# nirschl-lab/stain2stain

Measured on AMD Instinct MI355X. Metric: paired 256x256 stain tiles/sec (full CFM optimisation step), higher is better.
Workload: dtype bf16

## Files before the change

include/stain2stain_hip.h:

```cpp
#ifndef STAIN2STAIN_HIP_H
#define STAIN2STAIN_HIP_H

#ifdef __cplusplus
extern "C" {
#endif

#define S2S_OK 0
#define S2S_ERR_SHAPE (-1)
#define S2S_ERR_ALIGN (-2)
#define S2S_ERR_DTYPE (-3)
#define S2S_ERR_LAUNCH (-4)
#define S2S_ERR_NULL (-5)

#define S2S_BF16 0
#define S2S_F32 1

int s2s_conv3x3_stat_blocks(int dtype, int B, int H, int W, int Cout);
int s2s_conv3x3_nhwc(int dtype, const void* x0, int ld0, int c0, const void* x1, int ld1, int c1,
                     const void* w_packed, const float* bias, void* y, int ldy, float* stat_part,
                     const float* ep_scale, const float* ep_shift, int relu, int B, int H, int W, int Cout,
                     void* stream);

int s2s_conv3x3_ksplit(int dtype, int B, int H, int W, int Cout, int cin);
int s2s_conv3x3_nhwc_k(int dtype, const void* x0, int ld0, int c0, const void* x1, int ld1, int c1,
                       const void* w_packed, const float* bias, void* y, int ldy, float* stat_part,
                       const float* ep_scale, const float* ep_shift, int relu, float* kwork, int B, int H, int W,
                       int Cout, void* stream);
int s2s_conv3x3_stat_rows(int dtype, int B, int H, int W, int Cout, int c0, int c1, int ld0, int ld1, int has_bias);
int s2s_conv3x3_staged(int dtype, int B, int H, int W, int Cout, int c0, int c1, int ld0, int ld1, int ldy, int stats);
int s2s_conv3x3_family(int dtype, int B, int H, int W, int Cout, int c0, int c1, int ld0, int ld1, int ldy, int has_bias,
                       int has_affine, int stats, int stat_rows, int kwork);
int s2s_conv3x3_nhwc_s(int dtype, const void* x0, int ld0, int c0, const void* x1, int ld1, int c1, const void* w_packed,
                       const float* bias, void* y, int ldy, float* stat_part, int stat_rows, const float* ep_scale,
                       const float* ep_shift, int relu, float* kwork, int B, int H, int W, int Cout, void* stream);
int s2s_debug_conv_clock(long* out_host, int n);

int s2s_conv3x3_wgrad_splits(int dtype, int B, int H, int W, int Cin, int Cout);
int s2s_conv3x3_wgrad_nhwc(int dtype, const void* dy, int lddy, int Cout, const void* x0, int ld0, int c0,
                           const void* x1, int ld1, int c1, float* part, float* grad_oihw, int accumulate,
                           int B, int H, int W, void* stream);
int s2s_conv3x3_wgrad_phase(int dtype, const void* dy, int lddy, int Cout, const void* x0, int ld0, int c0,
                            const void* x1, int ld1, int c1, float* part, float* grad_oihw, int accumulate,
                            int B, int H, int W, int phases, void* stream);

int s2s_stem_stat_blocks(int B, int H, int W);
int s2s_stem_conv3x3_fwd(int dtype, const float* x_nchw, const float* w_oihw, const float* bias, void* y, int ldy,
                         float* stat_part, int B, int H, int W, int Cin, int Cout, void* stream);
int s2s_stem_wgrad_blocks(int B, int H, int W);
int s2s_stem_conv3x3_wgrad(int dtype, const void* dy, int lddy, const float* x_nchw, float* part, float* dw_oihw,
                           float* dbias, int accumulate, int B, int H, int W, int Cin, int Cout, void* stream);
int s2s_head_conv1x1_fwd(int dtype, const void* x, int ldx, const float* w, const float* bias, float* y_nchw, int B,
                         int H, int W, int C, int Cout, void* stream);
int s2s_head_wgrad_blocks(int B, int H, int W);
int s2s_head_conv1x1_bwd(int dtype, const float* dy_nchw, const void* x, int ldx, const float* w, void* dx, int lddx,
                         float* part, float* dw, float* dbias, int accumulate, int B, int H, int W, int C, int Cout,
                         void* stream);

int s2s_head_loss_blocks(int B, int H, int W);
int s2s_head_loss_fused(int dtype, const void* x, int ldx, const float* w, const float* bias, const float* u_nchw,
                        float* v_nchw, void* dx, int lddx, float grad_scale, float* part, double* lpart, float* dw,
                        float* dbias, float* loss, int accumulate, int B, int H, int W, int C, int Cout, void* stream);

int s2s_tail_blocks(int B, int H, int W);
int s2s_tail_fwd_loss(int dtype, const void* raw, int ldx, const float* scale, const float* shift, const float* mean,
                      const float* invstd, const float* w, const float* bias, const float* u_nchw, float* v_nchw,
                      float* g_nchw, float grad_scale, float* part, double* lpart, float* bnwork, float* dw,
                      float* dbias, float* loss, float* dgamma, float* dbeta, float* conv_dbias, int accumulate, int B,
                      int H, int W, int C, int Cout, void* stream);
int s2s_tail_bwd_apply(int dtype, const void* raw, int ldx, const float* g_nchw, const float* w, const float* scale,
                       const float* shift, const float* mean, const float* invstd, const float* gamma,
                       const float* bnwork, void* dx, int lddx, int B, int H, int W, int C, int Cout, void* stream);

int s2s_bn_finalize(const float* part, int nblk, int C, long count, const float* gamma, const float* beta,
                    float* running_mean, float* running_var, long* num_batches_tracked, float momentum, float eps,
                    float* mean, float* invstd, float* scale, float* shift, void* stream);
int s2s_bn_finalize_b(const float* part, int nblk, int C, long count, const float* gamma, const float* beta,
                      float* running_mean, float* running_var, long* num_batches_tracked, float momentum, float eps,
                      float* mean, float* invstd, float* scale, float* shift, const float* conv_bias, void* stream);
int s2s_bn_eval_prepare(int C, const float* gamma, const float* beta, const float* running_mean,
                        const float* running_var, float eps, float* scale, float* shift, void* stream);
int s2s_bn_relu_apply(int dtype, const void* x, int ldx, const float* scale, const float* shift, void* y, int ldy,
                      void* pool, int ldp, int B, int H, int W, int C, void* stream);
int s2s_maxpool2(int dtype, const void* x, int ldx, void* pool, int ldp, int B, int H, int W, int C, void* stream);
int s2s_bn_bwd_blocks(int B, int H, int W, int C);
int s2s_bn_relu_bwd(int dtype, const void* g1, int ldg1, const void* gp, int ldgp, const float* scale,
                    const float* shift, const void* x, int ldx, const float* mean, const float* invstd, const float* gamma, float* dgamma,
                    float* dbeta, float* dbias_conv, int accumulate, void* dx, int lddx, float* work, int B, int H,
                    int W, int C, void* stream);
int s2s_bn_partial_sums(const float* part, int nblk, int C, float* sums, void* stream);
int s2s_bn_relu_bwd_phase(int dtype, const void* g1, int ldg1, const void* gp, int ldgp, const float* scale,
                          const float* shift, const void* x, int ldx, const float* mean, const float* invstd,
                          const float* gamma, float* dgamma, float* dbeta, float* dbias_conv, int accumulate, void* dx,
                          int lddx, float* work, int B, int H, int W, int C, long count_total, int phases, void* stream);

int s2s_upsample2x_bilinear_ac_fwd(int dtype, const void* x, int ldx, const float* bias_nc, void* y, int ldy, int B,
                                   int Hin, int Win, int Hout, int Wout, int C, void* stream);
int s2s_upsample2x_bilinear_ac_fwd_ref(int dtype, const void* x, int ldx, const float* bias_nc, void* y, int ldy, int B,
                                       int Hin, int Win, int Hout, int Wout, int C, void* stream);
int s2s_upsample2x_fwd_family(int ldx, int ldy, int B, int Hin, int Win, int Hout, int Wout, int C, int reference);
int s2s_upsample2x_bilinear_ac_bwd(int dtype, const void* dy, int lddy, void* dx, int lddx, int B, int Hin, int Win,
                                   int Hout, int Wout, int C, void* stream);
int s2s_upsample2x_bilinear_ac_bwd_ref(int dtype, const void* dy, int lddy, void* dx, int lddx, int B, int Hin,
                                       int Win, int Hout, int Wout, int C, void* stream);
int s2s_upsample2x_bwd_family(int lddy, int lddx, int B, int Hin, int Win, int Hout, int Wout, int C, int reference);
int s2s_pixel_sum(int dtype, const void* x, int ldx, float* out_nc, int B, int HW, int C, int accumulate,
                  void* stream);

int s2s_time_embedding(const float* t, float* out, int B, int dim, void* stream);
int s2s_linear_fwd(const float* x, const float* w, const float* bias, float* y, int B, int K, int N, void* stream);
int s2s_linear_bwd(const float* dy, const float* x, const float* w, float* dx, float* dw, float* db, int accumulate,
                   int B, int K, int N, void* stream);
int s2s_silu_fwd(const float* h, float* a, int n, void* stream);
int s2s_silu_bwd(const float* h, const float* da, float* dh, int n, void* stream);
int s2s_cfm_sample(const float* x0, const float* x1, const float* t, const float* eps, float sigma, float* xt,
                   float* ut, int B, long per_sample, void* stream);
int s2s_mse_loss(const float* v, const float* u, float* dv, float grad_scale, float* loss, double* work, long count,
                 void* stream);
int s2s_ode_error_norm(const float* e, const float* y0, const float* y1, float atol, float rtol, float* out,
                       double* work, long n, void* stream);
int s2s_axpy(float* x, const float* y, float a, long n, void* stream);
int s2s_dp_partials(long n);
int s2s_dp_init(int phase, const float* y, const float* k1, const float* fa, double* state, double* part, float* out,
                float* t_out, int* status, float atol, float rtol, int B, long n, void* stream);
int s2s_dp_stage(int i, const float* y, const float* k1, const float* k2, const float* k3, const float* k4,
                 const float* k5, const float* k6, const double* state, float* out, float* t_out, int B, long n,
                 void* stream);
int s2s_dp_error(const float* k1, const float* k2, const float* k3, const float* k4, const float* k5, const float* k6,
                 const float* k7, const float* y, const float* y_new, const double* state, double* part, float atol,
                 float rtol, int B, long n, void* stream);
int s2s_dp_control(double* state, const double* part, int* status, int max_steps, int B, long n, void* stream);
int s2s_dp_commit(float* y, const float* y_new, float* k1, const float* k7, const double* state, int B, long n,
                  void* stream);
int s2s_rk_stage(const float* x, const float* k1, const float* k2, const float* k3, float c1, float c2, float c3, int nk,
                 float* out, float* t_out, const float* table, const int* counter, int stages, int stage, int table_len,
                 int B, long n, void* stream);
int s2s_rk_combine(float* x, const float* k1, const float* k2, const float* k3, const float* k4, float c1, float c2,
                   float c3, float c4, int nk, int* counter, int B, long n, void* stream);
int s2s_fill_f32(float* x, float v, long n, void* stream);
int s2s_euler_tick(float* t, int n, const float* table, int* counter, void* stream);

int s2s_adam_step(float* p, const float* g, float* m, float* v, long n, int step, float lr, float beta1, float beta2,
                  float eps, float weight_decay, float grad_scale, void* stream);
int s2s_adam_step_dev(float* p, const float* g, float* m, float* v, long n, const float* hyper, void* stream);
long s2s_adam_multi_blocks(long n);
int s2s_adam_multi(const void* desc, int ntensors, long total, int step, float lr, float beta1, float beta2, float eps,
                   float weight_decay, float grad_scale, void* stream);
int s2s_adam_ema_step(float* p, const float* g, float* m, float* v, float* ema, long n, int step, float lr, float beta1,
                      float beta2, float eps, float weight_decay, float grad_scale, float ema_weight, void* stream);
int s2s_adam_ema_step_dev(float* p, const float* g, float* m, float* v, float* ema, long n, const float* hyper,
                          const float* ema_weight, void* stream);
long s2s_ema_multi_blocks(long n);
int s2s_ema_multi(const void* desc, int ntensors, long total, const float* weight, void* stream);
long s2s_pack_conv3x3_fwd_elems(int Cout, int Cin);
long s2s_pack_conv3x3_dgrad_elems(int Cout, int Cin);
int s2s_pack_conv3x3(int dtype, const float* w_oihw, void* w_fwd, void* w_dgrad, int Cout, int Cin, void* stream);
int s2s_pack_conv3x3_batched(int dtype, const void* desc, int nlayers, long total, void* stream);
int s2s_nchw_to_nhwc(int dtype, const float* x_nchw, void* y, int ldy, int B, int C, int H, int W, void* stream);
int s2s_nhwc_to_nchw(int dtype, const void* x, int ldx, float* y_nchw, int accumulate, int B, int C, int H, int W,
                     void* stream);

int s2s_paired_crop_flip_normalize(const void* src_u8, const void* tgt_u8, const int* params, float* out_src,
                                   float* out_tgt, int B, int Hs, int Ws, int S, void* stream);
int s2s_pil_resize_bilinear_normalize(const void* src_u8, void* tmp_u8, const int* bounds_h, const int* kk_h,
                                      int ksize_h, const int* bounds_v, const int* kk_v, int ksize_v, void* out_u8,
                                      float* out_f, int B, int Hs, int Ws, int Ho, int Wo, void* stream);

int s2s_region_gather(const void* img_u8, long pitch, int H, int W, int band_top, int band_h, const int* origins,
                      float* out, int B, int T, void* stream);
int s2s_region_blend(const float* tiles, int c0, const float* tiles1, int c1, const int* origins, int n, int T,
                     int overlap, float* acc, int band_rows, int H, int W, int r0, int r1, void* stream);
int s2s_region_finalize(float* acc, int band_rows, int W, int C, int r0, int r1, void* out_u8, long pitch_u8,
                        float* out_f, long pitch_f, int out_top, void* stream);

int s2s_region_tissue_count(const void* img_u8, long pitch, int H, int W, int band_top, int band_h, const int* origins,
                            int n, int T, int white, int black, int* counts, void* stream);
int s2s_region_skip_weight(const int* origins, int n, int T, int overlap, float* ws, int band_rows, int H, int W,
                           int r0, int r1, void* stream);
int s2s_region_finalize_mixed(float* acc, float* ws, int band_rows, int W, int C, int r0, int r1, const void* src_u8,
                              long src_pitch, int src_top, void* out_u8, long pitch_u8, float* out_f, long pitch_f,
                              int out_top, void* stream);

int s2s_seg_loss(const float* z, const float* g, float* dz, float* out, double* work, long n, float smooth,
                 float dice_weight, float grad_scale, void* stream);
int s2s_seg_loss_multiclass(const float* z, const long* target, float* dz, float* out, double* work, long B, long HW,
                            int C, int ignore_index, float smooth, float dice_weight, float grad_scale, void* stream);

int s2s_seg_eval_binary(const float* z, const float* g, float* out, long* counts, double* work, long n, float smooth,
                        float dice_weight, void* stream);
int s2s_seg_eval_multiclass(const float* z, const long* target, float* out, long* counts, double* work, long B,
                            long HW, int C, int ignore_index, float smooth, float dice_weight, void* stream);
int s2s_head_mse_eval_blocks(int B, int H, int W, int C);
int s2s_head_mse_eval(int dtype, const void* x, int ldx, const float* w, const float* bias, const float* u_nchw,
                      float* loss, double* lpart, int B, int H, int W, int C, int Cout, void* stream);

int s2s_image_quality_blocks(int H, int W, int win);
int s2s_image_quality_f32(const float* a, const float* b, int B, int C, int H, int W, int quantize, int win,
                          const float* taps, float k1, float k2, double* part, void* stream);
int s2s_image_quality_u8(const void* a, long pitch_a, long img_a, const void* b, long pitch_b, long img_b, int B,
                         int band_top, int band_h, int H, int W, int by0, int nby, int win, const float* taps, float k1,
                         float k2, double* part, void* stream);
int s2s_image_quality_finalize(const double* part, int B, int C, int H, int W, int win, float range, float* out,
                               void* stream);

int s2s_stain_quant_chunks(int cell_h, int cell_w);
int s2s_stain_quant_u8(const void* a, long pitch_a, long img_a, const void* b, long pitch_b, long img_b, int paired,
                       int B, int band_top, int band_h, int H, int W, int cell_h, int cell_w, int g0, int ng,
                       const float* od_table, const float* unmix, int white, int black, int stain, double* part,
                       void* stream);
int s2s_stain_quant_f32(const float* a, const float* b, int paired, int B, int H, int W, const float* od_table,
                        const float* unmix, int white, int black, int stain, double* part, void* stream);
int s2s_stain_quant_finalize(const double* part, long owners, int nchunk, int paired, long* counts, double* sums,
                             float* out, void* stream);
int s2s_stain_separate(const void* img, int is_f32, long pitch, long img_stride, int B, int H, int W,
                       const float* od_table, const float* unmix, float* out, void* stream);
int s2s_stain_mask_u8(const void* img, long pitch, long img_stride, int B, int band_top, int band_h, int H, int W,
                      const float* od_table, const float* unmix, int white, int black, int stain, void* mask,
                      long mask_pitch, long mask_stride, long* tissue, void* stream);
int s2s_stain_mask_f32(const float* img, int B, int H, int W, const float* od_table, const float* unmix, int white,
                       int black, int stain, void* mask, long mask_pitch, long mask_stride, long* tissue, void* stream);

long s2s_stain_moments_slots(int B, int H, int W);
int s2s_stain_moments_u8(const void* img, long pitch, long img_stride, int B, int band_top, int band_h, int H, int W,
                         const int* q_table, int u_beta, int black, long* part, void* stream);
int s2s_stain_moments_finalize(const long* part, long nslots, long* out, void* stream);
int s2s_stain_angle_hist_u8(const void* img, long pitch, long img_stride, int B, int band_top, int band_h, int H, int W,
                            const float* od_table, const float* plane, int u_beta, int black, int reset, long* hist,
                            void* stream);
int s2s_stain_conc_hist_u8(const void* img, long pitch, long img_stride, int B, int band_top, int band_h, int H, int W,
                           const float* od_table, const float* unmix, int u_beta, int black, int reset, long* hist,
                           void* stream);
int s2s_stain_normalize_u8(const void* img, long pitch, long img_stride, int B, int H, int W, const float* od_table,
                           const float* coef, void* out, long out_pitch, long out_img, int out_f32, void* stream);

long s2s_objects_words(int B, int H, int W);
long s2s_objects_hit_words(int B, int H, int W);
int s2s_objects_label(const void* mask, long pitch, long img_stride, int fg_bits, int B, int H, int W, int connectivity,
                      int min_area, int max_objects, int* scratch, int* labels, int* count, long* kept_pixels,
                      int* largest, long* size_hist, int* tab_area, int* tab_bbox, long* tab_sums, void* stream);
int s2s_objects_centroid(const int* count, const int* tab_area, const long* tab_sums, int B, int max_objects,
                         float* centroid, void* stream);
int s2s_objects_hits(const int* labels_pred, const int* labels_target, int B, int H, int W, int* scratch, int* hits,
                     void* stream);
int s2s_objects_scores(const int* count_pred, const int* count_target, const int* hits, int B, float* out,
                       int* abs_err, void* stream);
int s2s_objects_density(const long* kept_pixels, const long* tissue, const int* count, int B,
                        const double* mm2_per_pixel, float* burden, double* per_mm2, void* stream);

int s2s_paired_augment(const void* src_u8, long src_pitch, long src_img, const void* tgt_u8, long tgt_pitch,
                       long tgt_img, const void* mask_u8, long mask_pitch, long mask_img, int B, int Hs, int Ws, int S,
                       const int* params, int param_cols, const float* src_map, const float* tgt_map,
                       const float* od_table, int white, float* out_src, float* out_tgt, void* out_mask, int mask_kind,
                       void* out_src_u8, void* out_tgt_u8, void* stream);
int s2s_stain_augment_u8(const void* img, long pitch, long img_stride, int B, int H, int W, const float* maps,
                         const float* od_table, int white, void* out, long out_pitch, long out_img, int out_f32,
                         void* stream);

int s2s_structure_map_u8(const void* img, long pitch, long img_stride, int B, int H, int W, const int* q_table,
                         const int* w, int ds, void* out, void* stream);
int s2s_register_sums(const void* a, const void* b, int B, int h, int w, int R, const int* center, long* tsum,
                      long* sums, void* stream);
int s2s_register_pick(const long* tsum, const long* sums, const int* center, int B, int R, int ds, int* shift,
                      double* score, int* valid, void* stream);
int s2s_shift_tiles_u8(const void* img, long pitch, long img_stride, int B, int H, int W, int C, const int* shift,
                       int fill, void* out, long out_pitch, long out_img, void* stream);

int s2s_weighted_mse(const float* v, const float* u, const float* mask, float* dv, float* out, double* work, long B,
                     int C, long HW, float roi_lambda, float grad_scale, void* stream);
int s2s_charbonnier_roi(const float* pred, const float* truth, const float* mask, float* out, double* work, long B,
                        int C, long HW, float eps_charb, float eps_area, void* stream);
int s2s_class_embed_add(const float* temb, const float* table, const long* y, float* out, int B, int dim,
                        void* stream);
int s2s_class_embed_bwd(const float* dout, const long* y, float* dtable, int accumulate, int B, int dim,
                        int num_classes, void* stream);

int s2s_instnorm_blocks(int B, int H, int W, int C);
int s2s_instnorm_lrelu_fwd(int dtype, const void* x, int ldx, const float* gamma, const float* beta, void* y, int ldy,
                           float* work, float* stats, int B, int H, int W, int C, float eps, float slope,
                           void* stream);
int s2s_instnorm_lrelu_bwd(int dtype, const void* g, int ldg, const void* x, int ldx, const float* stats, void* dx,
                           int lddx, float* dgamma, float* dbeta, int accumulate, float* work, int B, int H, int W,
                           int C, float eps, float slope, void* stream);

int s2s_conv2x2_stat_blocks(int B, int H, int W, int Cout);
int s2s_conv2x2_nhwc(int dtype, const void* x, int ldx, int cin, const void* w_packed, const float* bias, void* y,
                     int ldy, float* stat_part, int B, int H, int W, int Cout, int pad, void* stream);
int s2s_space_to_depth_pad1(int dtype, const void* x, int ldx, void* xs, int ldxs, int inverse, int B, int H, int W,
                            int C, void* stream);
int s2s_channel_sum_blocks(long npix, int C);
int s2s_channel_sum(int dtype, const void* x, int ldx, float* work, float* out, long npix, int C, int accumulate,
                    void* stream);
int s2s_pack_conv4x4(const float* w_oihw, void* wf, void* wd, int Cout, int Cin, int stride, void* stream);
int s2s_conv4x4s1_nhwc(int dtype, const void* x, int ldx, int cin, const void* w_packed, const float* bias, void* y,
                       int ldy, float* stat_part, int B, int H, int W, int Cout, int pad, void* stream);
int s2s_conv4x4s1_wgrad_splits(int B, int H, int W, int Cin, int Cout);
int s2s_conv4x4s1_wgrad_nhwc(int dtype, const void* dy, int lddy, int Cout, const void* x, int ldx, int cin,
                             float* part, float* grad16, int accumulate, int B, int H, int W, void* stream);
int s2s_conv2x2_wgrad_splits(int B, int H, int W, int Cin, int Cout);
int s2s_conv2x2_wgrad_nhwc(int dtype, const void* dy, int lddy, int Cout, const void* x, int ldx, int cin, float* part,
                           float* grad2, int accumulate, int B, int H, int W, void* stream);

int s2s_convkxk_stat_blocks(int dtype, int B, int H, int W, int Cout, int ks);
int s2s_convkxk_nhwc(int dtype, const void* x, int ldx, int cin, const void* w_packed, const float* bias, int bias_mod,
                     void* y, int ldy, void* y2, int ldy2, int act, float act_slope, float* stat_part, float* kwork, int B,
                     int H, int W, int Cout, int ks, int pad, void* stream);
int s2s_convkxk_ksplit(int dtype, int B, int H, int W, int Cout, int cin, int ks);
int s2s_convkxk_wgrad_splits(int dtype, int B, int H, int W, int Cin, int Cout, int ks);
int s2s_convkxk_wgrad_nhwc(int dtype, const void* dy, int lddy, int Cout, const void* x, int ldx, int cin, float* part,
                           float* grad, int layout, int accumulate, int B, int H, int W, int ks, int x_plain, void* stream);
int s2s_conv4x4s2_ksplit(int B, int H, int W, int Cout, int Cin);
int s2s_conv4x4s2_plan(int B, int H, int W, int Cout, int Cin);
int s2s_conv4x4s2_nhwc(int dtype, const void* x, int ldx, int Cin, const void* wf, const float* bias, void* y, int ldy,
                       void* y2, int ldy2, int act, float act_slope, float* kwork, int B, int H, int W, int Cout,
                       void* stream);
int s2s_convt4x4s2_ksplit(int B, int h, int w, int C, int Cin);
int s2s_convt4x4s2_plan(int B, int h, int w, int C, int Cin);
int s2s_convt4x4s2_nhwc(int dtype, const void* x, int ldx, int Cin, const void* wd, const float* bias, void* y, int ldy,
                        float* kwork, int B, int h, int w, int C, void* stream);
int s2s_convsm_ok(int dtype, int mode, int B, int h, int w, int Cin, int Cout);
int s2s_convsm_nhwc(int dtype, int mode, const void* x, int ldx, int Cin, const void* w_packed, const float* bias, int epi,
                    int act, float slope, float eps, void* raw, int ldraw, void* y, int ldy, void* y2, int ldy2,
                    float* stats, const float* stats_in, const void* z, int ldz, const void* g2, int ldg2, int bwd_c0,
                    int B, int h, int w, int Cout, void* stream);
int s2s_instnorm_lrelu_fwd2(int dtype, const void* x, int ldx, const float* gamma, const float* beta, void* y, int ldy,
                            void* y2, int ldy2, float* work, float* stats, int B, int H, int W, int C, float eps,
                            float slope, void* stream);
int s2s_instnorm_lrelu_bwd2(int dtype, const void* g, int ldg, const void* g2, int ldg2, const void* x, int ldx,
                            const float* stats, void* dx, int lddx, float* dgamma, float* dbeta, int accumulate,
                            float* work, int B, int H, int W, int C, float eps, float slope, void* stream);
int s2s_instnorm_split_ok(int dtype, int H, int W, int C);
int s2s_instnorm_lrelu_fwd_split(int dtype, const float* slabs, int S, const float* bias, void* raw, int ldraw, void* y,
                                 int ldy, void* y2, int ldy2, float* stats, int B, int H, int W, int C, float eps,
                                 float slope, void* stream);
int s2s_instnorm_lrelu_bwd_split(int dtype, const float* gslabs, int S, const void* g2, int ldg2, const void* x, int ldx,
                                 const float* stats, void* dx, int lddx, int B, int H, int W, int C, float slope,
                                 void* stream);
int s2s_pack_conv4x4_t(int dtype, const float* w_oihw, void* wf, void* wd, int Cout, int Cin, int stride, void* stream);
long s2s_pack_conv4x4_blocks(int Cout, int Cin, int stride);
int s2s_pack_conv4x4_batched(int dtype, const void* desc, int nlayers, long total, void* stream);
int s2s_p2p_pack_input(int dtype, const float* a_nchw, int ca, const float* b_nchw, int cb, void* out, int ldo, int B,
                       int H, int W, void* stream);
int s2s_p2p_unpack(int dtype, const void* in, int ldi, int c0, int C, float* out_nchw, int B, int H, int W, void* stream);
int s2s_p2p_tanh_l1_blocks(int B, int H, int W);
int s2s_p2p_tanh_l1_fwd(int dtype, const void* h, int ldh, const float* src_nchw, const float* tgt_nchw, void* d_in,
                        int ldd, float* fake_nchw, float* l1_out, void* work, int B, int H, int W, int C, void* stream);
int s2s_p2p_tanh_l1_bwd(int dtype, const void* h, int ldh, const float* tgt_nchw, const void* gd, int ldg, float l1_scale,
                        void* dh, int lddh, int B, int H, int W, int C, void* stream);
int s2s_p2p_bce_logits(int dtype, const void* z, int ldz, int n_real, float w_real, float w_fake, void* dz, int lddz,
                       float* out2, int N, int HW, void* stream);
int s2s_p2p_bce_blocks(int N, int HW);
int s2s_p2p_bce_logits_w(int dtype, const void* z, int ldz, int n_real, float w_real, float w_fake, void* dz, int lddz,
                         float* out2, double* work, int N, int HW, void* stream);
int s2s_p2p_act_bwd_blocks(long npix, int C);
int s2s_p2p_act_bwd(int dtype, const void* g, int ldg, const void* g2, int ldg2, const void* a, int lda, float slope,
// ... 15 lines not shown
```

stain2stain_amd/csrc/conv_edge.hip:

```cpp
#include "common.h"

namespace {

constexpr int STEM_MAX_CIN = 8;

typedef __attribute__((address_space(3))) s16x4 lds_s16x4;

__device__ __forceinline__ bf16x8 tr_frag8(const char* p) {
  s16x4 lo = __builtin_amdgcn_ds_read_tr16_b64_v4i16((lds_s16x4*)(p));
  s16x4 hi = __builtin_amdgcn_ds_read_tr16_b64_v4i16((lds_s16x4*)(p + 4 * 64));
  bf16x4 l4 = __builtin_bit_cast(bf16x4, lo), h4 = __builtin_bit_cast(bf16x4, hi);
  bf16x8 r;
#pragma unroll
  for (int i = 0; i < 4; ++i) { r[i] = l4[i]; r[4 + i] = h4[i]; }
  return r;
}

template <int NIMG>
__device__ __forceinline__ void split_store(char* base, int img_stride, int off, const float* v8) {
  bf16x8 h, m, l;
#pragma unroll
  for (int i = 0; i < 8; ++i) {
    h[i] = (bf16_t)v8[i];
    const float r1 = v8[i] - (float)h[i];
    m[i] = (bf16_t)r1;
    l[i] = (bf16_t)(r1 - (float)m[i]);
  }
  *reinterpret_cast<bf16x8*>(base + off) = h;
  if (NIMG == 3) {
    *reinterpret_cast<bf16x8*>(base + img_stride + off) = m;
    *reinterpret_cast<bf16x8*>(base + 2 * img_stride + off) = l;
  }
}

template <typename T>
__global__ __launch_bounds__(256) void stem_wgrad_kernel(const T* __restrict__ dy, int lddy,
                                                         const float* __restrict__ x, float* __restrict__ part,
                                                         int B, int H, int W, int Cin, int Cout, int tilesY,
                                                         int tilesX) {
  constexpr int NIMG = sizeof(T) == 4 ? 3 : 1;
  constexpr int NPX = 256;
  constexpr int DY_IMG = 2 * NPX * 64;
  constexpr int P_IMG = NPX * 64;
  extern __shared__ __attribute__((aligned(16))) char smem[];
  char* const ldsDY = smem;
  char* const ldsP = smem + NIMG * DY_IMG;
  float* const xl = reinterpret_cast<float*>(ldsP + NIMG * P_IMG);
  const int tid = threadIdx.x, lane = tid & 63, wave = tid >> 6;
  const int wco = wave & 1, whalf = wave >> 1;
  const int co0 = blockIdx.y * 64;
  const int c0 = blockIdx.z * 3;
  const int nc = (Cin - c0) < 3 ? (Cin - c0) : 3, K = nc * 9;
  const int g = lane >> 4, q = (lane & 15) >> 2, pq = lane & 3;
  const int frag_off = ((g >> 1) * 8 + q) * 64 + ((g & 1) * 16 + pq * 4) * 2;
  const int ntiles = B * tilesY * tilesX;
  f32x16 acc;
#pragma unroll
  for (int j = 0; j < 16; ++j) acc[j] = 0.f;
  for (int tile = blockIdx.x; tile < ntiles; tile += gridDim.x) {
    int bt = tile;
    const int tx = bt % tilesX; bt /= tilesX;
    const int ty = bt % tilesY;
    const int n = bt / tilesY;
    const int y0 = ty * 16, x0 = tx * 16;
    __syncthreads();
    for (int i = tid; i < nc * 324; i += 256) {
      const int ci = i / 324, r = i - ci * 324, hy = r / 18, hx = r - hy * 18;
      const int gy = y0 - 1 + hy, gx = x0 - 1 + hx;
      xl[i] = (gy >= 0 && gy < H && gx >= 0 && gx < W) ? x[(((long)n * Cin + c0 + ci) * H + gy) * W + gx] : 0.f;
    }
#pragma unroll
    for (int it = 0; it < 8; ++it) {
      const int idx = tid + it * 256;
      const int px = idx >> 3, pc = idx & 7;
      const int gy = y0 + (px >> 4), gx = x0 + (px & 15), co = co0 + pc * 8;
      float v8[8];
#pragma unroll
      for (int k = 0; k < 8; ++k) v8[k] = 0.f;
      if (gy < H && gx < W && co < Cout) {
        const f32x8 v = load8(dy + (((long)n * H + gy) * W + gx) * lddy + co);
#pragma unroll
        for (int k = 0; k < 8; ++k) v8[k] = v.v[k];
      }
      split_store<NIMG>(ldsDY, DY_IMG, (pc >> 2) * (NPX * 64) + px * 64 + (pc & 3) * 16, v8);
    }
    __syncthreads();
    {
      const int py = tid >> 4, px = tid & 15;
      const bool inside = (y0 + py < H) && (x0 + px < W);
#pragma unroll
      for (int c4 = 0; c4 < 4; ++c4) {
        float v8[8];
#pragma unroll
        for (int k = 0; k < 8; ++k) {
          const int kk = c4 * 8 + k;
          float v = 0.f;
          if (kk < K) {
            const int ci = kk / 9, t = kk - ci * 9;
            v = xl[ci * 324 + (py + t / 3) * 18 + px + t % 3];
          } else if (kk == K && c0 == 0) {
            v = inside ? 1.f : 0.f;
          }
          v8[k] = v;
        }
        split_store<NIMG>(ldsP, P_IMG, tid * 64 + c4 * 16, v8);
      }
    }
    __syncthreads();
    const char* A0 = ldsDY + wco * (NPX * 64) + frag_off;
    const char* B0 = ldsP + frag_off;
#pragma unroll
    for (int ks = 0; ks < 8; ++ks) {
      const int m0 = (whalf * 8 + ks) * 16;
      const bf16x8 ah = tr_frag8(A0 + m0 * 64);
      const bf16x8 bh = tr_frag8(B0 + m0 * 64);
      if constexpr (NIMG == 3) {
        const bf16x8 am = tr_frag8(A0 + DY_IMG + m0 * 64), al = tr_frag8(A0 + 2 * DY_IMG + m0 * 64);
        const bf16x8 bm = tr_frag8(B0 + P_IMG + m0 * 64), bl = tr_frag8(B0 + 2 * P_IMG + m0 * 64);
        acc = __builtin_amdgcn_mfma_f32_32x32x16_bf16(am, bm, acc, 0, 0, 0);
        acc = __builtin_amdgcn_mfma_f32_32x32x16_bf16(al, bh, acc, 0, 0, 0);
        acc = __builtin_amdgcn_mfma_f32_32x32x16_bf16(ah, bl, acc, 0, 0, 0);
        acc = __builtin_amdgcn_mfma_f32_32x32x16_bf16(am, bh, acc, 0, 0, 0);
        acc = __builtin_amdgcn_mfma_f32_32x32x16_bf16(ah, bm, acc, 0, 0, 0);
      }
      acc = __builtin_amdgcn_mfma_f32_32x32x16_bf16(ah, bh, acc, 0, 0, 0);
    }
  }
  const int kcol = lane & 31, h = lane >> 5;
#pragma unroll
  for (int j = 0; j < 16; ++j) {
    const int co = co0 + wco * 32 + (j & 3) + 8 * (j >> 2) + 4 * h;
    if (co < Cout)
      part[((((long)blockIdx.z * gridDim.x + blockIdx.x) * 2 + whalf) * Cout + co) * 32 + kcol] = acc[j];
  }
}

__global__ __launch_bounds__(1024) void stem_wgrad_reduce_kernel(const float* part, int nslab, int Cout, int Cin, float* dw, float* db,
                                         int accumulate) {
  __shared__ double red[32][33];
  const int c0 = blockIdx.y * 3;
  const int K = ((Cin - c0) < 3 ? (Cin - c0) : 3) * 9;
  const int co = blockIdx.x, k = threadIdx.x & 31, sg = threadIdx.x >> 5;
  part += (long)blockIdx.y * nslab * Cout * 32;
  double s = 0.0, s1 = 0.0;
  int b = sg;
  for (; b + 32 < nslab; b += 64) {
    s += (double)part[((long)b * Cout + co) * 32 + k];
    s1 += (double)part[((long)(b + 32) * Cout + co) * 32 + k];
  }
  for (; b < nslab; b += 32) s += (double)part[((long)b * Cout + co) * 32 + k];
  s += s1;
  red[sg][k] = s;
  __syncthreads();
  if (sg == 0) {
    for (int j = 1; j < 32; ++j) s += red[j][k];
    if (k < K) {
      float* dst = dw + co * Cin * 9 + c0 * 9 + k;
      *dst = accumulate ? *dst + (float)s : (float)s;
    } else if (k == K && c0 == 0 && db) {
      db[co] = accumulate ? db[co] + (float)s : (float)s;
    }
  }
}

constexpr int HEAD_MAX_COUT = 4;
constexpr int HEAD_WIDE_COUT = 8;

template <typename T, int MO>
__global__ void head_fwd_kernel(const T* __restrict__ x, int ldx, const float* __restrict__ w,
                                const float* __restrict__ bias, float* __restrict__ y, long npix, int HW, int C,
                                int Cout) {
  extern __shared__ __attribute__((aligned(16))) char smem[];
  float* wl = reinterpret_cast<float*>(smem);
  for (int i = threadIdx.x; i < Cout * C; i += blockDim.x) wl[i] = w[i];
  __syncthreads();
  for (long p = (long)blockIdx.x * blockDim.x + threadIdx.x; p < npix; p += (long)gridDim.x * blockDim.x) {
    float acc[MO];
#pragma unroll
    for (int o = 0; o < MO; ++o) acc[o] = 0.f;
    for (int c8 = 0; c8 < C; c8 += 8) {
      const f32x8 v = load8(x + p * ldx + c8);
#pragma unroll
      for (int o = 0; o < MO; ++o)
        if (o < Cout)
#pragma unroll
          for (int k = 0; k < 8; ++k) acc[o] = fmaf(v.v[k], wl[o * C + c8 + k], acc[o]);
    }
    const long n = p / HW, q = p - n * HW;
#pragma unroll
    for (int o = 0; o < MO; ++o)
      if (o < Cout) y[(n * Cout + o) * HW + q] = acc[o] + (bias ? bias[o] : 0.f);
  }
}

template <typename T, int MO>
__global__ void head_bwd_data_kernel(const float* __restrict__ dy, const float* __restrict__ w, T* __restrict__ dx,
                                     int lddx, long npix, int HW, int C, int Cout) {
  extern __shared__ __attribute__((aligned(16))) char smem[];
  float* wl = reinterpret_cast<float*>(smem);
  for (int i = threadIdx.x; i < Cout * C; i += blockDim.x) wl[i] = w[i];
  __syncthreads();
  for (long p = (long)blockIdx.x * blockDim.x + threadIdx.x; p < npix; p += (long)gridDim.x * blockDim.x) {
    const long n = p / HW, q = p - n * HW;
    float g[MO];
#pragma unroll
    for (int o = 0; o < MO; ++o) g[o] = o < Cout ? dy[(n * Cout + o) * HW + q] : 0.f;
    for (int c8 = 0; c8 < C; c8 += 8) {
      f32x8 v;
#pragma unroll
      for (int k = 0; k < 8; ++k) {
        float a = 0.f;
#pragma unroll
        for (int o = 0; o < MO; ++o)
          if (o < Cout) a = fmaf(g[o], wl[o * C + c8 + k], a);
        v.v[k] = a;
      }
      store8(dx + p * lddx + c8, v);
    }
  }
}

template <typename T, int MO>
__global__ __launch_bounds__(256) void head_wgrad_kernel(const float* __restrict__ dy, const T* __restrict__ x,
                                                         int ldx, float* __restrict__ part, long npix, int HW, int C,
                                                         int Cout) {
  extern __shared__ __attribute__((aligned(16))) char smem[];
  float* xl = reinterpret_cast<float*>(smem);
  float* gl = xl + 64 * (C + 1);
  const int nout = Cout * (C + 1);
  float acc[8];
#pragma unroll
  for (int i = 0; i < 8; ++i) acc[i] = 0.f;
  for (long p0 = (long)blockIdx.x * 64; p0 < npix; p0 += (long)gridDim.x * 64) {
    __syncthreads();
    for (int i = threadIdx.x; i < 64 * C; i += 256) {
      const int pp = i / C, c = i - pp * C;
      xl[pp * (C + 1) + c] = (p0 + pp < npix) ? to_f32(x[(p0 + pp) * ldx + c]) : 0.f;
    }
    for (int i = threadIdx.x; i < 64 * MO; i += 256) {
      const int pp = i / MO, o = i - pp * MO;
      float v = 0.f;
      if (o < Cout && p0 + pp < npix) {
        const long p = p0 + pp, n = p / HW, q = p - n * HW;
        v = dy[(n * Cout + o) * HW + q];
      }
      gl[i] = v;
    }
    __syncthreads();
#pragma unroll
    for (int i = 0; i < 8; ++i) {
      const int id = threadIdx.x + i * 256;
      if (id < nout) {
        const int o = id / (C + 1), c = id - o * (C + 1);
        float a = acc[i];
        if (c < C) for (int pp = 0; pp < 64; ++pp) a = fmaf(gl[pp * MO + o], xl[pp * (C + 1) + c], a);
        else for (int pp = 0; pp < 64; ++pp) a += gl[pp * MO + o];
        acc[i] = a;
      }
    }
  }
#pragma unroll
  for (int i = 0; i < 8; ++i) {
    const int id = threadIdx.x + i * 256;
    if (id < nout) part[(long)blockIdx.x * nout + id] = acc[i];
  }
}

__global__ __launch_bounds__(256) void head_wgrad_reduce_kernel(const float* part, int nblk, int Cout, int C, float* dw, float* db,
                                         int accumulate) {
  __shared__ double red[32][9];
  const int nout = Cout * (C + 1);
  const int ol = threadIdx.x & 7, sg = threadIdx.x >> 3;
  const int i = blockIdx.x * 8 + ol;
  double s = 0.0;
  if (i < nout) {
    double s1 = 0.0;
    int b = sg;
    for (; b + 32 < nblk; b += 64) { s += (double)part[(long)b * nout + i]; s1 += (double)part[(long)(b + 32) * nout + i]; }
    for (; b < nblk; b += 32) s += (double)part[(long)b * nout + i];
    s += s1;
  }
  red[sg][ol] = s;
  __syncthreads();
  if (sg == 0 && i < nout) {
    for (int j = 1; j < 32; ++j) s += red[j][ol];
    const int o = i / (C + 1), c = i - o * (C + 1);
    if (c == C && !db) return;
    float* dst = (c < C) ? dw + o * C + c : db + o;
    *dst = accumulate ? *dst + (float)s : (float)s;
  }
}

template <typename T>
__global__ __launch_bounds__(256) void head_loss_fused_kernel(const T* __restrict__ x, int ldx,
                                                              const float* __restrict__ w, const float* __restrict__ bias,
                                                              const float* __restrict__ u, float* __restrict__ v_out,
                                                              T* __restrict__ dx, int lddx, float coef,
                                                              float* __restrict__ part, double* __restrict__ lpart,
                                                              long npix, int HW, int C, int Cout) {
  extern __shared__ __attribute__((aligned(16))) char smem[];
  float* wl = reinterpret_cast<float*>(smem);
  float* gl = wl + HEAD_MAX_COUT * C;
  bf16_t* al = reinterpret_cast<bf16_t*>(gl + 256 * HEAD_MAX_COUT);
  __shared__ double lred[256];
  const int AS = C + 8;
  for (int i = threadIdx.x; i < Cout * C; i += 256) wl[i] = w[i];
  const int nout = Cout * (C + 1);
  float acc[4];
#pragma unroll
  for (int i = 0; i < 4; ++i) acc[i] = 0.f;
  double lsum = 0.0;
  __syncthreads();
  for (long p0 = (long)blockIdx.x * 256; p0 < npix; p0 += (long)gridDim.x * 256) {
    const long p = p0 + threadIdx.x;
    const bool ok = p < npix;
    float g[HEAD_MAX_COUT];
#pragma unroll
    for (int o = 0; o < HEAD_MAX_COUT; ++o) g[o] = 0.f;
    if (ok) {
      float vv[HEAD_MAX_COUT];
#pragma unroll
      for (int o = 0; o < HEAD_MAX_COUT; ++o) vv[o] = 0.f;
      for (int c8 = 0; c8 < C; c8 += 8) {
        const f32x8 a = load8(x + p * ldx + c8);
        bf16x8 ab;
#pragma unroll
        for (int k = 0; k < 8; ++k) ab[k] = (bf16_t)a.v[k];
        *reinterpret_cast<bf16x8*>(al + threadIdx.x * AS + c8) = ab;
#pragma unroll
        for (int o = 0; o < HEAD_MAX_COUT; ++o)
          if (o < Cout)
#pragma unroll
            for (int k = 0; k < 8; ++k) vv[o] = fmaf(a.v[k], wl[o * C + c8 + k], vv[o]);
      }
      const long n = p / HW, q = p - n * HW;
#pragma unroll
      for (int o = 0; o < HEAD_MAX_COUT; ++o)
        if (o < Cout) {
          const float vo = vv[o] + (bias ? bias[o] : 0.f);
          const long idx = (n * Cout + o) * HW + q;
          if (v_out) v_out[idx] = vo;
          const float d = vo - u[idx];
          lsum += (double)(d * d);
          g[o] = coef * d;
        }
      for (int c8 = 0; c8 < C; c8 += 8) {
        f32x8 da;
#pragma unroll
        for (int k = 0; k < 8; ++k) {
          float s = 0.f;
#pragma unroll
          for (int o = 0; o < HEAD_MAX_COUT; ++o)
            if (o < Cout) s = fmaf(g[o], wl[o * C + c8 + k], s);
          da.v[k] = s;
        }
        store8(dx + p * lddx + c8, da);
      }
    } else {
      for (int c8 = 0; c8 < C; c8 += 8) {
        bf16x8 z;
#pragma unroll
        for (int k = 0; k < 8; ++k) z[k] = (bf16_t)0.f;
        *reinterpret_cast<bf16x8*>(al + threadIdx.x * AS + c8) = z;
      }
    }
#pragma unroll
    for (int o = 0; o < HEAD_MAX_COUT; ++o) gl[threadIdx.x * HEAD_MAX_COUT + o] = g[o];
    __syncthreads();
#pragma unroll
    for (int i = 0; i < 4; ++i) {
      const int id = threadIdx.x + i * 256;
      if (id < nout) {
        const int o = id / (C + 1), c = id - o * (C + 1);
        float a = acc[i];
        if (c < C) for (int pp = 0; pp < 256; ++pp) a = fmaf(gl[pp * HEAD_MAX_COUT + o], (float)al[pp * AS + c], a);
        else for (int pp = 0; pp < 256; ++pp) a += gl[pp * HEAD_MAX_COUT + o];
        acc[i] = a;
      }
    }
    __syncthreads();
  }
#pragma unroll
  for (int i = 0; i < 4; ++i) {
    const int id = threadIdx.x + i * 256;
    if (id < nout) part[(long)blockIdx.x * nout + id] = acc[i];
  }
  lred[threadIdx.x] = lsum;
  __syncthreads();
  for (int o = 128; o > 0; o >>= 1) {
    if (threadIdx.x < o) lred[threadIdx.x] += lred[threadIdx.x + o];
    __syncthreads();
  }
  if (threadIdx.x == 0) lpart[blockIdx.x] = lred[0];
}

template <typename T, int PCB>
__global__ __launch_bounds__(256) void head_loss_lanes_kernel(const T* __restrict__ x, int ldx,
                                                              const float* __restrict__ w,
                                                              const float* __restrict__ bias,
                                                              const float* __restrict__ u, float* __restrict__ v_out,
                                                              T* __restrict__ dx, int lddx, float coef,
                                                              float* __restrict__ part, double* __restrict__ lpart,
                                                              long npix, int HW, int Cout) {
  constexpr int C = PCB * 8, PPB = 256 / PCB, MO = HEAD_MAX_COUT;
  __shared__ float fold[256][MO * 8 + 1];
  __shared__ float dbf[PPB][MO];
  __shared__ double lred[256];
  const int tid = threadIdx.x, pc = tid & (PCB - 1), slot = tid / PCB;
  const int lane = tid & 63, grp0 = lane & ~(PCB - 1);
  float wr[MO][8], bo[MO];
#pragma unroll
  for (int o = 0; o < MO; ++o) {
    bo[o] = (o < Cout && bias) ? bias[o] : 0.f;
#pragma unroll
    for (int k = 0; k < 8; ++k) wr[o][k] = o < Cout ? w[o * C + pc * 8 + k] : 0.f;
  }
  float dwacc[MO][8], dbacc[MO];
#pragma unroll
  for (int o = 0; o < MO; ++o) {
    dbacc[o] = 0.f;
#pragma unroll
    for (int k = 0; k < 8; ++k) dwacc[o][k] = 0.f;
  }
  double lsum = 0.0;
  const int np = (int)npix, stride = (int)gridDim.x * PPB;
  f32x8 a_next;
  {
    const int pf = (int)blockIdx.x * PPB + slot;
#pragma unroll
    for (int k = 0; k < 8; ++k) a_next.v[k] = 0.f;
    if (pf < np) a_next = load8(x + (long)pf * ldx + pc * 8);
  }
  for (int p0 = (int)blockIdx.x * PPB; p0 < np; p0 += stride) {
    const int p = p0 + slot;
    const bool ok = p < np;
    const f32x8 a = a_next;
    {
// ... 104 lines not shown
#pragma unroll
    for (int k = 0; k < 8; ++k) a_next.v[k] = 0.f;
    if (pf < np) a_next = load8(x + (long)pf * ldx + pc * 8);
  }
  for (int p0 = (int)blockIdx.x * PPB; p0 < np; p0 += stride) {
    const int p = p0 + slot;
    const bool ok = p < np;
    const f32x8 a = a_next;
    {
      const int pn = p + stride;
#pragma unroll
      for (int k = 0; k < 8; ++k) a_next.v[k] = 0.f;
      if (p0 + stride < np && pn < np) a_next = load8(x + (long)pn * ldx + pc * 8);
    }
    const int n = p / HW, q = p - n * HW;
    if (FWD) {
#pragma unroll
      for (int o = 0; o < MO; ++o) {
        float t = 0.f;
#pragma unroll
        for (int k = 0; k < 8; ++k) t = fmaf(a.v[k], wr[o][k], t);
#pragma unroll
        for (int m = 1; m < PCB; m <<= 1) t += __shfl_xor(t, m, 64);
        if (ok && o < Cout && (o & (PCB - 1)) == pc) v_out[((long)n * Cout + o) * HW + q] = t + bo[o];
      }
    } else {
      float gm[MO], g[MO];
#pragma unroll
      for (int o = 0; o < MO; ++o) {
        gm[o] = 0.f;
        if (ok && o < Cout && (o & (PCB - 1)) == pc) gm[o] = dy[((long)n * Cout + o) * HW + q];
      }
#pragma unroll
      for (int o = 0; o < MO; ++o) g[o] = __shfl(gm[o], grp0 + (o & (PCB - 1)), 64);
      if (ok) {
        f32x8 da;
#pragma unroll
        for (int k = 0; k < 8; ++k) {
          float t = 0.f;
#pragma unroll
          for (int o = 0; o < MO; ++o) t = fmaf(g[o], wr[o][k], t);
          da.v[k] = t;
        }
        store8(dx + (long)p * lddx + pc * 8, da);
      }
#pragma unroll
      for (int o = 0; o < MO; ++o) {
        if (pc == 0) dbacc[o] += g[o];
#pragma unroll
        for (int k = 0; k < 8; ++k) dwacc[o][k] = fmaf(g[o], a.v[k], dwacc[o][k]);
      }
    }
  }
  if (FWD) return;
#pragma unroll
  for (int o = 0; o < MO; ++o) {
#pragma unroll
    for (int k = 0; k < 8; ++k) fold[tid][o * 8 + k] = dwacc[o][k];
    if (pc == 0) dbf[slot][o] = dbacc[o];
  }
  __syncthreads();
  const int nout = Cout * (C + 1);
  for (int id = tid; id < nout; id += 256) {
    const int o = id / (C + 1), c = id - o * (C + 1);
    float t = 0.f;
    if (c < C) {
      const int cp = c >> 3, k = c & 7;
      for (int sl = 0; sl < PPB; ++sl) t += fold[sl * PCB + cp][o * 8 + k];
    } else {
      for (int sl = 0; sl < PPB; ++sl) t += dbf[sl][o];
    }
    part[(long)blockIdx.x * nout + id] = t;
  }
}

template <typename T, bool FWD>
bool launch_head_lanes(const void* x, int ldx, const float* w, const float* bias, const float* dy, float* v, void* dx,
                       int lddx, float* part, int nb, long npix, int HW, int C, int Cout, hipStream_t s) {
  if (Cout > HEAD_MAX_COUT || (C % 8) || npix >= (1L << 31) - (1L << 20)) return false;
#define S2S_HLN(PP)                                                                                                  \
  hipLaunchKernelGGL((head_lanes_kernel<T, PP, FWD>), dim3(nb), dim3(256), 0, s, (const T*)x, ldx, w, bias, dy, v,   \
                     (T*)dx, lddx, part, npix, HW, Cout);                                                            \
  return true;
  switch (C / 8) {
    case 1: S2S_HLN(1) case 2: S2S_HLN(2) case 4: S2S_HLN(4) case 8: S2S_HLN(8) case 16: S2S_HLN(16) case 32: S2S_HLN(32)
    case 64: S2S_HLN(64) default: return false;
  }
#undef S2S_HLN
}

template <int CTRL>
__device__ __forceinline__ float dpp_f32(float v) {
  return __builtin_bit_cast(float, __builtin_amdgcn_update_dpp(0, __builtin_bit_cast(int, v), CTRL, 0xf, 0xf, true));
}
template <int PCB>
__device__ __forceinline__ float group_sum(float t) {
  if (PCB >= 2) t += dpp_f32<0xB1>(t);
  if (PCB >= 4) t += dpp_f32<0x4E>(t);
  if (PCB >= 8) t += dpp_f32<0x141>(t);
  if (PCB >= 16) t += dpp_f32<0x140>(t);
#pragma unroll
  for (int m = 16; m < PCB; m <<= 1) t += __shfl_xor(t, m, 64);
  return t;
}

__device__ __forceinline__ bf16x8 tail_ld(const bf16_t* p) { return *reinterpret_cast<const bf16x8*>(p); }
__device__ __forceinline__ f32x8 tail_ld(const float* p) { return load8(p); }
__device__ __forceinline__ float tail_at(const bf16x8& v, int k) { return (float)v[k]; }
__device__ __forceinline__ float tail_at(const f32x8& v, int k) { return v.v[k]; }

template <typename T, int PCB, int MO>
__global__ __launch_bounds__(256) void tail_fwd_loss_kernel(const T* __restrict__ raw, int ldx,
                                                            const float* __restrict__ scale, const float* __restrict__ shift,
                                                            const float* __restrict__ w, const float* __restrict__ bias,
                                                            const float* __restrict__ u, float* __restrict__ v_out,
                                                            float* __restrict__ g_out, float coef,
                                                            float* __restrict__ part, double* __restrict__ lpart,
                                                            long npix, int HW, int Cout) {
  constexpr int C = PCB * 8, PPB = 256 / PCB;
  __shared__ float fold[256][MO * 8 + 1];
  __shared__ float dbf[PPB][MO];
  __shared__ double lred[256];
  const int tid = threadIdx.x, pc = tid & (PCB - 1), slot = tid / PCB;
  float wr[MO][8], bo[MO];
#pragma unroll
  for (int o = 0; o < MO; ++o) {
    bo[o] = (o < Cout && bias) ? bias[o] : 0.f;
#pragma unroll
    for (int k = 0; k < 8; ++k) wr[o][k] = o < Cout ? w[o * C + pc * 8 + k] : 0.f;
  }
  float sc[8], sh[8];
#pragma unroll
  for (int k = 0; k < 8; ++k) { sc[k] = scale[pc * 8 + k]; sh[k] = shift[pc * 8 + k]; }
  float dwacc[MO][8], dbacc[MO];
#pragma unroll
  for (int o = 0; o < MO; ++o) {
    dbacc[o] = 0.f;
#pragma unroll
    for (int k = 0; k < 8; ++k) dwacc[o][k] = 0.f;
  }
  double lsum = 0.0;
  const int np = (int)npix, stride = (int)gridDim.x * PPB;
  struct Stage {
    decltype(tail_ld((const T*)nullptr)) r;
    float u[MO];
    long i;
  };
  auto fetch = [&](Stage& st, int pf) {
    pf = pf < np ? pf : np - 1;
    st.r = tail_ld(raw + (long)pf * ldx + pc * 8);
    const int n = pf / HW, q = pf - n * HW;
    st.i = (long)n * Cout * HW + q;
#pragma unroll
    for (int o = 0; o < MO; ++o) st.u[o] = u[st.i + (long)(o < Cout ? o : Cout - 1) * HW];
  };
  Stage sa, sb;
  fetch(sa, (int)blockIdx.x * PPB + slot);
  fetch(sb, (int)blockIdx.x * PPB + slot + stride);
  auto step = [&](Stage& st, int p0) {
    const int p = p0 + slot;
    const bool ok = p < np;
    f32x8 r;
#pragma unroll
    for (int k = 0; k < 8; ++k) r.v[k] = tail_at(st.r, k);
    float cu[MO];
#pragma unroll
    for (int o = 0; o < MO; ++o) cu[o] = st.u[o];
    const long i0 = st.i;
    fetch(st, p + 2 * stride);
    float a[8];
#pragma unroll
    for (int k = 0; k < 8; ++k)
      a[k] = to_f32(from_f32<T>(fmaxf(fmaf(r.v[k], sc[k], sh[k]), 0.f)));
    float vv[MO];
#pragma unroll
    for (int o = 0; o < MO; ++o) {
      float t = 0.f;
#pragma unroll
      for (int k = 0; k < 8; ++k) t = fmaf(a[k], wr[o][k], t);
      vv[o] = group_sum<PCB>(t) + bo[o];
    }
    float g[MO];
#pragma unroll
    for (int o = 0; o < MO; ++o) {
      const float d = vv[o] - cu[o];
      g[o] = (ok && o < Cout) ? coef * d : 0.f;
      if (ok && o < Cout && (o & (PCB - 1)) == pc) {
        const long idx = i0 + (long)o * HW;
        if (v_out) v_out[idx] = vv[o];
        lsum += (double)(d * d);
        g_out[idx] = g[o];
      }
    }
#pragma unroll
    for (int o = 0; o < MO; ++o) {
      if (pc == 0) dbacc[o] += g[o];
#pragma unroll
      for (int k = 0; k < 8; ++k) dwacc[o][k] = fmaf(g[o], a[k], dwacc[o][k]);
    }
  };
  for (int p0 = (int)blockIdx.x * PPB; p0 < np; p0 += 2 * stride) {
    step(sa, p0);
    if (p0 + stride < np) step(sb, p0 + stride);
  }
#pragma unroll
  for (int o = 0; o < MO; ++o) {
#pragma unroll
    for (int k = 0; k < 8; ++k) fold[tid][o * 8 + k] = dwacc[o][k];
    if (pc == 0) dbf[slot][o] = dbacc[o];
  }
  lred[tid] = lsum;
  __syncthreads();
  const int nout = Cout * (C + 1);
  for (int id = tid; id < nout; id += 256) {
    const int o = id / (C + 1), c = id - o * (C + 1);
    float t = 0.f;
    if (c < C) {
      const int cp = c >> 3, k = c & 7;
      for (int sl = 0; sl < PPB; ++sl) t += fold[sl * PCB + cp][o * 8 + k];
    } else {
      for (int sl = 0; sl < PPB; ++sl) t += dbf[sl][o];
    }
    part[(long)blockIdx.x * nout + id] = t;
  }
  for (int o = 128; o > 0; o >>= 1) {
    if (tid < o) lred[tid] += lred[tid + o];
    __syncthreads();
  }
  if (tid == 0) lpart[blockIdx.x] = lred[0];
}

template <typename T, int PCB, int MO>
__global__ __launch_bounds__(256) void tail_bwd_apply_kernel(const T* __restrict__ raw, int ldx,
                                                             const float* __restrict__ g_nchw, const float* __restrict__ w,
                                                             const float* __restrict__ scale, const float* __restrict__ shift,
                                                             const float* __restrict__ mean, const float* __restrict__ invstd,
                                                             const float* __restrict__ gamma, const float* __restrict__ c1,
                                                             const float* __restrict__ c2, T* __restrict__ dx, int lddx,
                                                             long npix, int HW, int Cout) {
  constexpr int C = PCB * 8, PPB = 256 / PCB;
  const int tid = threadIdx.x, pc = tid & (PCB - 1), slot = tid / PCB;
  float wr[MO][8];
#pragma unroll
  for (int o = 0; o < MO; ++o)
#pragma unroll
    for (int k = 0; k < 8; ++k) wr[o][k] = o < Cout ? w[o * C + pc * 8 + k] : 0.f;
  float ga[8], k1[8], k2[8], mu[8], is[8], sc[8], sh[8];
#pragma unroll
  for (int k = 0; k < 8; ++k) {
    const int c = pc * 8 + k;
    mu[k] = mean[c]; is[k] = invstd[c]; sc[k] = scale[c]; sh[k] = shift[c];
    ga[k] = gamma[c] * is[k]; k1[k] = c1[c]; k2[k] = c2[c];
  }
  const int np = (int)npix, stride = (int)gridDim.x * PPB;
  const int first = (int)blockIdx.x * PPB + slot;
  const int nit = first < np ? (np - first + stride - 1) / stride : 0;
  f32x8 r_next;
  float g_next[MO];
  auto fetch = [&](int p) {
    r_next = load8(raw + (long)p * ldx + pc * 8);
    const int n = p / HW, q = p - n * HW;
#pragma unroll
    for (int o = 0; o < MO; ++o) g_next[o] = o < Cout ? g_nchw[((long)n * Cout + o) * HW + q] : 0.f;
  };
  if (nit > 0) fetch(first + (nit - 1) * stride);
  for (int it = nit - 1; it >= 0; --it) {
    const int p = first + it * stride;
    const f32x8 r = r_next;
    float g[MO];
#pragma unroll
    for (int o = 0; o < MO; ++o) g[o] = g_next[o];
    if (it > 0) fetch(p - stride);
    f32x8 out;
#pragma unroll
    for (int k = 0; k < 8; ++k) {
      float t = 0.f;
#pragma unroll
      for (int o = 0; o < MO; ++o) t = fmaf(g[o], wr[o][k], t);
      const float da = to_f32(from_f32<T>(t));
      const float dz = fmaf(r.v[k], sc[k], sh[k]) > 0.f ? da : 0.f;
      out.v[k] = ga[k] * (dz - k1[k] - ((r.v[k] - mu[k]) * is[k]) * k2[k]);
    }
    store8(dx + (long)p * lddx + pc * 8, out);
  }
}

__global__ __launch_bounds__(256) void loss_finalize_kernel(const double* part, int n, double inv_count, float* loss) {
  __shared__ double red[256];
  double s = 0.0;
  for (int i = threadIdx.x; i < n; i += 256) s += part[i];
  red[threadIdx.x] = s;
  __syncthreads();
  for (int o = 128; o > 0; o >>= 1) {
    if (threadIdx.x < o) red[threadIdx.x] += red[threadIdx.x + o];
    __syncthreads();
  }
  if (threadIdx.x == 0) *loss = (float)(red[0] * inv_count);
}

}

int s2s_internal_stem_fwd(int dtype, const float* x_nchw, const float* w_oihw, const float* bias, void* y, int ldy,
                          float* stat_part, int B, int H, int W, int Cin, int Cout, hipStream_t s);

extern "C" int s2s_stem_stat_blocks(int B, int H, int W) {
  if (B <= 0 || H <= 0 || W <= 0) return S2S_ERR_SHAPE;
  return B * cdiv(H, 16) * cdiv(W, 16);
}

extern "C" int s2s_stem_conv3x3_fwd(int dtype, const float* x_nchw, const float* w_oihw, const float* bias, void* y,
                                    int ldy, float* stat_part, int B, int H, int W, int Cin, int Cout, void* stream) {
  if (!x_nchw || !w_oihw || !y) return S2S_ERR_NULL;
  if (B <= 0 || H <= 0 || W <= 0 || Cin <= 0 || Cin > 6 || Cout <= 0 || (Cout % 8) || (ldy % 8))
    return S2S_ERR_SHAPE;
  return s2s_internal_stem_fwd(dtype, x_nchw, w_oihw, bias, y, ldy, stat_part, B, H, W, Cin, Cout,
                               (hipStream_t)stream);
}

extern "C" int s2s_stem_wgrad_blocks(int B, int H, int W) {
  if (B <= 0 || H <= 0 || W <= 0) return S2S_ERR_SHAPE;
  const int nt = B * cdiv(H, 16) * cdiv(W, 16);
  constexpr int cap = 512;
  return nt < cap ? nt : cap;
}

extern "C" int s2s_stem_conv3x3_wgrad(int dtype, const void* dy, int lddy, const float* x_nchw, float* part,
                                      float* dw_oihw, float* dbias, int accumulate, int B, int H, int W, int Cin,
                                      int Cout, void* stream) {
  if (!dy || !x_nchw || !part || !dw_oihw) return S2S_ERR_NULL;
  if (B <= 0 || H <= 0 || W <= 0 || Cin <= 0 || Cin > 6 || Cout <= 0 || (Cout % 8) || (lddy % 8))
    return S2S_ERR_SHAPE;
  const int nb = s2s_stem_wgrad_blocks(B, H, W);
  hipStream_t s = (hipStream_t)stream;
  dim3 grid(nb, cdiv(Cout, 64), cdiv(Cin, 3));
  if (dtype == S2S_BF16) {
    const int lds = 1 * (2 * 256 * 64 + 256 * 64) + 3 * 324 * 4;
    hipLaunchKernelGGL(stem_wgrad_kernel<bf16_t>, grid, dim3(256), lds, s, (const bf16_t*)dy, lddy, x_nchw, part, B,
                       H, W, Cin, Cout, cdiv(H, 16), cdiv(W, 16));
  } else if (dtype == S2S_F32) {
    const int lds = 3 * (2 * 256 * 64 + 256 * 64) + 3 * 324 * 4;
    static unsigned long long attr_devs = 0;
    if (int rc = s2s_allow_dyn_lds(reinterpret_cast<const void*>(stem_wgrad_kernel<float>), lds, &attr_devs)) return rc;
    hipLaunchKernelGGL(stem_wgrad_kernel<float>, grid, dim3(256), lds, s, (const float*)dy, lddy, x_nchw, part, B, H,
                       W, Cin, Cout, cdiv(H, 16), cdiv(W, 16));
  } else return S2S_ERR_DTYPE;
  hipLaunchKernelGGL(stem_wgrad_reduce_kernel, dim3(Cout, cdiv(Cin, 3)), dim3(1024), 0, s, part, 2 * nb, Cout, Cin, dw_oihw, dbias,
                     accumulate);
  S2S_LAUNCH_CHECK();
  return S2S_OK;
}

extern "C" int s2s_head_conv1x1_fwd(int dtype, const void* x, int ldx, const float* w, const float* bias,
                                    float* y_nchw, int B, int H, int W, int C, int Cout, void* stream) {
  if (!x || !w || !y_nchw) return S2S_ERR_NULL;
  if (B <= 0 || H <= 0 || W <= 0 || C <= 0 || (C % 8) || (ldx % 8) || Cout <= 0 || Cout > HEAD_WIDE_COUT)
    return S2S_ERR_SHAPE;
  const long npix = (long)B * H * W;
  long grid = (npix + 255) / 256;
  if (grid > 4096) grid = 4096;
  hipStream_t s = (hipStream_t)stream;
  if (dtype != S2S_BF16 && dtype != S2S_F32) return S2S_ERR_DTYPE;
  {
    const int nbl = (int)(((npix + 255) / 256) < 2048 ? ((npix + 255) / 256) : 2048);
    const bool done = dtype == S2S_BF16
        ? launch_head_lanes<bf16_t, true>(x, ldx, w, bias, nullptr, y_nchw, nullptr, 8, nullptr, nbl, npix, H * W, C, Cout, s)
        : launch_head_lanes<float, true>(x, ldx, w, bias, nullptr, y_nchw, nullptr, 8, nullptr, nbl, npix, H * W, C, Cout, s);
    if (done) { S2S_LAUNCH_CHECK(); return S2S_OK; }
  }
#define S2S_HEAD_FWD(TT, MO)                                                                                        \
  hipLaunchKernelGGL((head_fwd_kernel<TT, MO>), dim3((int)grid), dim3(256), Cout * C * 4, s, (const TT*)x, ldx, w, \
                     bias, y_nchw, npix, H * W, C, Cout)
  if (dtype == S2S_BF16) { if (Cout <= 4) S2S_HEAD_FWD(bf16_t, 4); else S2S_HEAD_FWD(bf16_t, 8); }
  else if (dtype == S2S_F32) { if (Cout <= 4) S2S_HEAD_FWD(float, 4); else S2S_HEAD_FWD(float, 8); }
  else return S2S_ERR_DTYPE;
#undef S2S_HEAD_FWD
  S2S_LAUNCH_CHECK();
  return S2S_OK;
}

extern "C" int s2s_head_wgrad_blocks(int B, int H, int W) {
  if (B <= 0 || H <= 0 || W <= 0) return S2S_ERR_SHAPE;
  const long nb = ((long)B * H * W + 63) / 64;
  return (int)(nb < 512 ? nb : 512);
}

extern "C" int s2s_head_conv1x1_bwd(int dtype, const float* dy_nchw, const void* x, int ldx, const float* w, void* dx,
                                    int lddx, float* part, float* dw, float* dbias, int accumulate, int B, int H, int W,
                                    int C, int Cout, void* stream) {
  if (!dy_nchw || !x || !w || !dx || !part || !dw) return S2S_ERR_NULL;
  if (B <= 0 || H <= 0 || W <= 0 || C <= 0 || (C % 8) || (ldx % 8) || (lddx % 8) || Cout <= 0 || Cout > HEAD_WIDE_COUT)
    return S2S_ERR_SHAPE;
  if (Cout * (C + 1) > 2048) return S2S_ERR_SHAPE;
  const long npix = (long)B * H * W;
  long grid = (npix + 255) / 256;
  if (grid > 4096) grid = 4096;
  const int nb = s2s_head_wgrad_blocks(B, H, W);
  const int mo = Cout <= 4 ? 4 : 8;
  const int lds = (64 * (C + 1) + 64 * mo) * 4;
  hipStream_t s = (hipStream_t)stream;
  if (dtype != S2S_BF16 && dtype != S2S_F32) return S2S_ERR_DTYPE;
  {
    const bool done = dtype == S2S_BF16
        ? launch_head_lanes<bf16_t, false>(x, ldx, w, nullptr, dy_nchw, nullptr, dx, lddx, part, nb, npix, H * W, C, Cout, s)
        : launch_head_lanes<float, false>(x, ldx, w, nullptr, dy_nchw, nullptr, dx, lddx, part, nb, npix, H * W, C, Cout, s);
    if (done) {
      hipLaunchKernelGGL(head_wgrad_reduce_kernel, dim3(cdiv(Cout * (C + 1), 8)), dim3(256), 0, s, part, nb, Cout, C,
                         dw, dbias, accumulate);
      S2S_LAUNCH_CHECK();
      return S2S_OK;
    }
  }
#define S2S_HEAD_BWD(TT, MO)                                                                                       \
  hipLaunchKernelGGL((head_bwd_data_kernel<TT, MO>), dim3((int)grid), dim3(256), Cout * C * 4, s, dy_nchw, w,      \
                     (TT*)dx, lddx, npix, H * W, C, Cout);                                                         \
  hipLaunchKernelGGL((head_wgrad_kernel<TT, MO>), dim3(nb), dim3(256), lds, s, dy_nchw, (const TT*)x, ldx, part,   \
                     npix, H * W, C, Cout);
  if (dtype == S2S_BF16) { if (mo == 4) { S2S_HEAD_BWD(bf16_t, 4) } else { S2S_HEAD_BWD(bf16_t, 8) } }
  else if (dtype == S2S_F32) { if (mo == 4) { S2S_HEAD_BWD(float, 4) } else { S2S_HEAD_BWD(float, 8) } }
  else return S2S_ERR_DTYPE;
#undef S2S_HEAD_BWD
  hipLaunchKernelGGL(head_wgrad_reduce_kernel, dim3(cdiv(Cout * (C + 1), 8)), dim3(256), 0, s, part, nb, Cout, C,
                     dw, dbias, accumulate);
  S2S_LAUNCH_CHECK();
  return S2S_OK;
}

extern "C" int s2s_head_loss_blocks(int B, int H, int W) {
  if (B <= 0 || H <= 0 || W <= 0) return S2S_ERR_SHAPE;
  const long nb = ((long)B * H * W + 255) / 256;
  return (int)(nb < 1024 ? nb : 1024);
}

extern "C" int s2s_head_loss_fused(int dtype, const void* x, int ldx, const float* w, const float* bias,
                                   const float* u_nchw, float* v_nchw, void* dx, int lddx, float grad_scale,
                                   float* part, double* lpart, float* dw, float* dbias, float* loss, int accumulate,
                                   int B, int H, int W, int C, int Cout, void* stream) {
  if (!x || !w || !u_nchw || !dx || !part || !lpart || !dw || !loss) return S2S_ERR_NULL;
  if (B <= 0 || H <= 0 || W <= 0 || C <= 0 || (C % 8) || (ldx % 8) || (lddx % 8) || Cout <= 0 || Cout > HEAD_MAX_COUT)
    return S2S_ERR_SHAPE;
  if (Cout * (C + 1) > 1024) return S2S_ERR_SHAPE;
  const long npix = (long)B * H * W;
  if (npix >= (1L << 31) - (1L << 20)) return S2S_ERR_SHAPE;
  const double count = (double)npix * Cout;
  const int nb = s2s_head_loss_blocks(B, H, W);
  const int lds = (HEAD_MAX_COUT * C + 256 * HEAD_MAX_COUT) * 4 + 256 * (C + 8) * 2;
  if (lds > 60 * 1024) return S2S_ERR_SHAPE;
  hipStream_t s = (hipStream_t)stream;
  const float coef = (float)(2.0 * (double)grad_scale / count);
  if (dtype != S2S_BF16 && dtype != S2S_F32) return S2S_ERR_DTYPE;
  const int pcb = C / 8;
  bool done = false;
#define S2S_HL(TT, PP)                                                                                              \
  hipLaunchKernelGGL((head_loss_lanes_kernel<TT, PP>), dim3(nb), dim3(256), 0, s, (const TT*)x, ldx, w, bias, u_nchw, \
                     v_nchw, (TT*)dx, lddx, coef, part, lpart, npix, H * W, Cout);                                 \
  done = true;
#define S2S_HL_T(TT)                                                                                    \
  switch (pcb) {                                                                                        \
    case 1: { S2S_HL(TT, 1) } break;  case 2: { S2S_HL(TT, 2) } break;  case 4: { S2S_HL(TT, 4) } break;    \
    case 8: { S2S_HL(TT, 8) } break;  case 16: { S2S_HL(TT, 16) } break; case 32: { S2S_HL(TT, 32) } break;  \
    case 64: { S2S_HL(TT, 64) } break; default: break;                                                  \
  }
  if (dtype == S2S_BF16) { S2S_HL_T(bf16_t) } else { S2S_HL_T(float) }
#undef S2S_HL_T
#undef S2S_HL
  if (!done) {
    if (dtype == S2S_BF16)
      hipLaunchKernelGGL(head_loss_fused_kernel<bf16_t>, dim3(nb), dim3(256), lds, s, (const bf16_t*)x, ldx, w, bias,
                         u_nchw, v_nchw, (bf16_t*)dx, lddx, coef, part, lpart, npix, H * W, C, Cout);
    else
      hipLaunchKernelGGL(head_loss_fused_kernel<float>, dim3(nb), dim3(256), lds, s, (const float*)x, ldx, w, bias,
                         u_nchw, v_nchw, (float*)dx, lddx, coef, part, lpart, npix, H * W, C, Cout);
  }
  hipLaunchKernelGGL(head_wgrad_reduce_kernel, dim3(cdiv(Cout * (C + 1), 8)), dim3(256), 0, s, part, nb, Cout, C,
                     dw, dbias, accumulate);
  hipLaunchKernelGGL(loss_finalize_kernel, dim3(1), dim3(256), 0, s, lpart, nb, 1.0 / count, loss);
  S2S_LAUNCH_CHECK();
  return S2S_OK;
}

int s2s_internal_tail_bn_sums(int dtype, const void* raw, int ldx, const float* g_nchw, const float* w, const float* scale,
                              const float* shift, const float* mean, const float* invstd, float* work, float* dgamma,
                              float* dbeta, float* zero_out, int accumulate, int B, int H, int W, int C, int Cout,
                              hipStream_t s);
extern "C" int s2s_bn_bwd_blocks(int B, int H, int W, int C);

namespace {
inline bool tail_shape_ok(int B, int H, int W, int C, int Cout, int ldx) {
  if (B <= 0 || H <= 0 || W <= 0 || C < 8 || (C % 8) || (ldx % 8) || Cout <= 0 || Cout > HEAD_MAX_COUT) return false;
  const int pcb = C / 8;
  if (pcb > 64 || (pcb & (pcb - 1))) return false;
  return (long)B * H * W < (1L << 31) - (1L << 20);
}
}

extern "C" int s2s_tail_blocks(int B, int H, int W) { return s2s_head_loss_blocks(B, H, W); }

extern "C" int s2s_tail_fwd_loss(int dtype, const void* raw, int ldx, const float* scale, const float* shift,
                                 const float* mean, const float* invstd, const float* w, const float* bias,
                                 const float* u_nchw, float* v_nchw, float* g_nchw, float grad_scale, float* part,
                                 double* lpart, float* bnwork, float* dw, float* dbias, float* loss, float* dgamma,
                                 float* dbeta, float* conv_dbias, int accumulate, int B, int H, int W, int C, int Cout,
                                 void* stream) {
  if (!raw || !scale || !shift || !mean || !invstd || !w || !u_nchw || !g_nchw || !part || !lpart || !bnwork || !dw ||
      !loss || !dgamma || !dbeta)
    return S2S_ERR_NULL;
  if (!tail_shape_ok(B, H, W, C, Cout, ldx)) return S2S_ERR_SHAPE;
  if (dtype != S2S_BF16 && dtype != S2S_F32) return S2S_ERR_DTYPE;
  const long npix = (long)B * H * W;
  const double count = (double)npix * Cout;
  const int nb = s2s_tail_blocks(B, H, W);
  hipStream_t s = (hipStream_t)stream;
  const float coef = (float)(2.0 * (double)grad_scale / count);
#define S2S_TA(TT, PP)                                                                                               \
  if (Cout <= 3)                                                                                                     \
    hipLaunchKernelGGL((tail_fwd_loss_kernel<TT, PP, 3>), dim3(nb), dim3(256), 0, s, (const TT*)raw, ldx, scale,     \
                       shift, w, bias, u_nchw, v_nchw, g_nchw, coef, part, lpart, npix, H * W, Cout);                \
  else                                                                                                               \
  hipLaunchKernelGGL((tail_fwd_loss_kernel<TT, PP, HEAD_MAX_COUT>), dim3(nb), dim3(256), 0, s, (const TT*)raw, ldx, scale, shift,   \
                     w, bias, u_nchw, v_nchw, g_nchw, coef, part, lpart, npix, H * W, Cout);
#define S2S_TA_T(TT)                                                                                    \
  switch (C / 8) {                                                                                      \
    case 1: { S2S_TA(TT, 1) } break;  case 2: { S2S_TA(TT, 2) } break;  case 4: { S2S_TA(TT, 4) } break;    \
    case 8: { S2S_TA(TT, 8) } break;  case 16: { S2S_TA(TT, 16) } break; case 32: { S2S_TA(TT, 32) } break;  \
    default: { S2S_TA(TT, 64) } break;                                                                  \
  }
  if (dtype == S2S_BF16) { S2S_TA_T(bf16_t) } else { S2S_TA_T(float) }
#undef S2S_TA_T
#undef S2S_TA
  hipLaunchKernelGGL(head_wgrad_reduce_kernel, dim3(cdiv(Cout * (C + 1), 8)), dim3(256), 0, s, part, nb, Cout, C,
                     dw, dbias, accumulate);
  hipLaunchKernelGGL(loss_finalize_kernel, dim3(1), dim3(256), 0, s, lpart, nb, 1.0 / count, loss);
  if (int rc = s2s_internal_tail_bn_sums(dtype, raw, ldx, g_nchw, w, scale, shift, mean, invstd, bnwork, dgamma, dbeta,
                                         (conv_dbias && !accumulate) ? conv_dbias : nullptr, accumulate, B, H, W, C,
                                         Cout, s))
    return rc;
  S2S_LAUNCH_CHECK();
  return S2S_OK;
}

extern "C" int s2s_tail_bwd_apply(int dtype, const void* raw, int ldx, const float* g_nchw, const float* w,
                                  const float* scale, const float* shift, const float* mean, const float* invstd,
                                  const float* gamma, const float* bnwork, void* dx, int lddx, int B, int H, int W,
                                  int C, int Cout, void* stream) {
  if (!raw || !g_nchw || !w || !scale || !shift || !mean || !invstd || !gamma || !bnwork || !dx) return S2S_ERR_NULL;
  if (!tail_shape_ok(B, H, W, C, Cout, ldx) || (lddx % 8) || lddx < C) return S2S_ERR_SHAPE;
  if (dtype != S2S_BF16 && dtype != S2S_F32) return S2S_ERR_DTYPE;
  const long npix = (long)B * H * W;
  const int nb = s2s_tail_blocks(B, H, W);
  const float* const c1 = bnwork + (long)2 * C * s2s_bn_bwd_blocks(B, H, W, C);
  hipStream_t s = (hipStream_t)stream;
#define S2S_TB(TT, PP)                                                                                              \
  if (Cout <= 3)                                                                                                    \
    hipLaunchKernelGGL((tail_bwd_apply_kernel<TT, PP, 3>), dim3(nb), dim3(256), 0, s, (const TT*)raw, ldx, g_nchw,  \
                       w, scale, shift, mean, invstd, gamma, c1, c1 + C, (TT*)dx, lddx, npix, H * W, Cout);         \
  else                                                                                                              \
  hipLaunchKernelGGL((tail_bwd_apply_kernel<TT, PP, HEAD_MAX_COUT>), dim3(nb), dim3(256), 0, s, (const TT*)raw, ldx, g_nchw, w,    \
                     scale, shift, mean, invstd, gamma, c1, c1 + C, (TT*)dx, lddx, npix, H * W, Cout);
#define S2S_TB_T(TT)                                                                                    \
  switch (C / 8) {                                                                                      \
    case 1: { S2S_TB(TT, 1) } break;  case 2: { S2S_TB(TT, 2) } break;  case 4: { S2S_TB(TT, 4) } break;    \
    case 8: { S2S_TB(TT, 8) } break;  case 16: { S2S_TB(TT, 16) } break; case 32: { S2S_TB(TT, 32) } break;  \
    default: { S2S_TB(TT, 64) } break;                                                                  \
  }
  if (dtype == S2S_BF16) { S2S_TB_T(bf16_t) } else { S2S_TB_T(float) }
#undef S2S_TB_T
#undef S2S_TB
  S2S_LAUNCH_CHECK();
  return S2S_OK;
}
```

stain2stain_amd/csrc/norm_act.hip:

```cpp
#include "common.h"
#include <type_traits>

namespace {

constexpr int RED_ROWS = 8;

constexpr int PRE_R = 16;
__global__ __launch_bounds__(1024) void prereduce_rows_kernel(float* __restrict__ part, int nrows, int ncols) {
  __shared__ double s1[32][33];
  const int cl = threadIdx.x & 31, rg = threadIdx.x >> 5;
  const int c = blockIdx.x * 32 + cl, r = blockIdx.y;
  double a = 0.0;
  if (c < ncols)
    for (int i = r + PRE_R * rg; i < nrows; i += PRE_R * 32) a += (double)part[(long)i * ncols + c];
  s1[rg][cl] = a;
  __syncthreads();
  if (rg == 0 && c < ncols) {
    for (int k = 1; k < 32; ++k) a += s1[k][cl];
    part[(long)r * ncols + c] = (float)a;
  }
}

inline int prereduce(float* part, int nrows, int ncols, hipStream_t s) {
  if (nrows <= 4 * PRE_R) return nrows;
// ... 342 lines not shown
        }
        o0[k] = from_f32<T>(v[0]); o1[k] = from_f32<T>(v[1]); o2[k] = from_f32<T>(v[2]); o3[k] = from_f32<T>(v[3]);
        __builtin_amdgcn_sched_barrier(0);
      }
      T* const d00 = dx + (((long)n * H + wy * 2) * W + wx * 2) * lddx + c8;
      vstore8(d00, o0);
      if (wg.ok(1)) vstore8(d00 + lddx, o1);
      if (wg.ok(2)) vstore8(d00 + (long)W * lddx, o2);
      if (wg.ok(3)) vstore8(d00 + (long)(W + 1) * lddx, o3);
    }
  }
  if (dxsum_part) {
    __shared__ float red[2304];
    const int rowlen = PCB * 8 + 1;
#pragma unroll
    for (int k = 0; k < 8; ++k) red[wl * rowlen + pc * 8 + k] = s[k];
    __syncthreads();
    for (int cl = threadIdx.x; cl < PCB * 8; cl += 256) {
      float t = 0.f;
      for (int r = 0; r < WL; ++r) t += red[r * rowlen + cl];
      const int c = blockIdx.x * PCB * 8 + cl;
      if (c < C) dxsum_part[(long)blockIdx.y * C + c] = t;
    }
  }
}

template <typename T>
__global__ __launch_bounds__(256) void bn_relu_bwd_reduce_flat_kernel(const T* __restrict__ g1, int ldg1, const float* __restrict__ scale, const float* __restrict__ shift,
                                               const T* __restrict__ x, int ldx, const float* mean, const float* invstd,
                                               float* part, long npix, int C) {
  const int PCB = pcb_of(C), WL = 256 / PCB;
  const int pc = threadIdx.x & (PCB - 1), wl = threadIdx.x / PCB;
  const int c8 = (blockIdx.x * PCB + pc) * 8;
  using Acc = typename std::conditional<std::is_same<T, float>::value, double, float>::type;
  Acc s1[8], s2[8];
#pragma unroll
  for (int k = 0; k < 8; ++k) { s1[k] = 0; s2[k] = 0; }
  if (c8 < C) {
    float mu[8], is[8], sc[8], sh[8];
#pragma unroll
    for (int k = 0; k < 8; ++k) { mu[k] = mean[c8 + k]; is[k] = invstd[c8 + k]; sc[k] = scale[c8 + k]; sh[k] = shift[c8 + k]; }
    for (long p = (long)blockIdx.y * WL + wl; p < npix; p += (long)gridDim.y * WL) {
      const f32x8 g = load8(g1 + p * ldg1 + c8);
      const f32x8 b = load8(x + p * ldx + c8);
#pragma unroll
      for (int k = 0; k < 8; ++k) {
        const float dz = fmaf(b.v[k], sc[k], sh[k]) > 0.f ? g.v[k] : 0.f;
        s1[k] += (Acc)dz;
        s2[k] += (Acc)(dz * ((b.v[k] - mu[k]) * is[k]));
      }
    }
  }
  __shared__ Acc red[2][2304];
  const int rowlen = PCB * 8 + 1;
#pragma unroll
  for (int k = 0; k < 8; ++k) { red[0][wl * rowlen + pc * 8 + k] = s1[k]; red[1][wl * rowlen + pc * 8 + k] = s2[k]; }
  __syncthreads();
  for (int i = threadIdx.x; i < 2 * PCB * 8; i += 256) {
    const int which = i / (PCB * 8), cl = i - which * (PCB * 8);
    Acc s = 0;
    for (int r = 0; r < WL; ++r) s += red[which][r * rowlen + cl];
    const int c = blockIdx.x * PCB * 8 + cl;
    if (c < C) part[((long)which * C + c) * gridDim.y + blockIdx.y] = (float)s;
  }
}

template <typename T>
__global__ __launch_bounds__(256) void bn_relu_bwd_reduce_tail_kernel(const float* __restrict__ g_nchw, const float* __restrict__ w, int Cout, int HW,
                                               const float* __restrict__ scale, const float* __restrict__ shift,
                                               const T* __restrict__ x, int ldx, const float* mean, const float* invstd,
                                               float* part, long npix, int C) {
  const int PCB = pcb_of(C), WL = 256 / PCB;
  const int pc = threadIdx.x & (PCB - 1), wl = threadIdx.x / PCB;
  const int c8 = (blockIdx.x * PCB + pc) * 8;
  using Acc = typename std::conditional<std::is_same<T, float>::value, double, float>::type;
  Acc s1[8], s2[8];
#pragma unroll
  for (int k = 0; k < 8; ++k) { s1[k] = 0; s2[k] = 0; }
  if (c8 < C) {
    float mu[8], is[8], sc[8], sh[8], wr[4][8];
#pragma unroll
    for (int k = 0; k < 8; ++k) { mu[k] = mean[c8 + k]; is[k] = invstd[c8 + k]; sc[k] = scale[c8 + k]; sh[k] = shift[c8 + k]; }
#pragma unroll
    for (int o = 0; o < 4; ++o)
#pragma unroll
      for (int k = 0; k < 8; ++k) wr[o][k] = o < Cout ? w[o * C + c8 + k] : 0.f;
    for (long p = (long)blockIdx.y * WL + wl; p < npix; p += (long)gridDim.y * WL) {
      const int pi = (int)p, n = pi / HW, q = pi - n * HW;
      float gv[4];
#pragma unroll
      for (int o = 0; o < 4; ++o) {
        const float t = g_nchw[((long)n * Cout + (o < Cout ? o : Cout - 1)) * HW + q];
        gv[o] = o < Cout ? t : 0.f;
      }
      const f32x8 b = load8(x + p * ldx + c8);
#pragma unroll
      for (int k = 0; k < 8; ++k) {
        float t = 0.f;
#pragma unroll
        for (int o = 0; o < 4; ++o) t = fmaf(gv[o], wr[o][k], t);
        const float gk = to_f32(from_f32<T>(t));
        const float dz = fmaf(b.v[k], sc[k], sh[k]) > 0.f ? gk : 0.f;
        s1[k] += (Acc)dz;
        s2[k] += (Acc)(dz * ((b.v[k] - mu[k]) * is[k]));
      }
    }
  }
  __shared__ Acc red[2][2304];
  const int rowlen = PCB * 8 + 1;
#pragma unroll
  for (int k = 0; k < 8; ++k) { red[0][wl * rowlen + pc * 8 + k] = s1[k]; red[1][wl * rowlen + pc * 8 + k] = s2[k]; }
  __syncthreads();
  for (int i = threadIdx.x; i < 2 * PCB * 8; i += 256) {
    const int which = i / (PCB * 8), cl = i - which * (PCB * 8);
    Acc s = 0;
    for (int r = 0; r < WL; ++r) s += red[which][r * rowlen + cl];
    const int c = blockIdx.x * PCB * 8 + cl;
    if (c < C) part[((long)which * C + c) * gridDim.y + blockIdx.y] = (float)s;
  }
}

template <typename T>
__global__ __launch_bounds__(256) void bn_relu_bwd_apply_flat_kernel(const T* __restrict__ g1, int ldg1, const float* __restrict__ scale, const float* __restrict__ shift,
                                              const T* __restrict__ x, int ldx, const float* mean, const float* invstd,
                                              const float* gamma, const float* c1, const float* c2, T* __restrict__ dx,
                                              int lddx, float* dxsum_part, long npix, int C, int rev) {
  const int PCB = pcb_of(C), WL = 256 / PCB;
  const int pc = threadIdx.x & (PCB - 1), wl = threadIdx.x / PCB;
  const int c8 = (blockIdx.x * PCB + pc) * 8;
  float s[8];
#pragma unroll
  for (int k = 0; k < 8; ++k) s[k] = 0.f;
  if (c8 < C) {
    float ga[8], k1[8], k2[8], mu[8], is[8], sc[8], sh[8];
#pragma unroll
    for (int k = 0; k < 8; ++k) {
      mu[k] = mean[c8 + k]; is[k] = invstd[c8 + k]; sc[k] = scale[c8 + k]; sh[k] = shift[c8 + k];
      ga[k] = gamma[c8 + k] * is[k]; k1[k] = c1[c8 + k]; k2[k] = c2[c8 + k];
    }
    const long p0 = (long)blockIdx.y * WL + wl, pstep = (long)gridDim.y * WL;
    const long nit = p0 < npix ? (npix - p0 + pstep - 1) / pstep : 0;
    for (long it = 0; it < nit; ++it) {
      const long p = p0 + (rev ? nit - 1 - it : it) * pstep;
      const f32x8 g = load8(g1 + p * ldg1 + c8);
      const f32x8 b = load8(x + p * ldx + c8);
      f32x8 o;
#pragma unroll
      for (int k = 0; k < 8; ++k) {
        const float dz = fmaf(b.v[k], sc[k], sh[k]) > 0.f ? g.v[k] : 0.f;
        o.v[k] = ga[k] * (dz - k1[k] - ((b.v[k] - mu[k]) * is[k]) * k2[k]);
        s[k] += o.v[k];
      }
      store8(dx + p * lddx + c8, o);
    }
  }
  if (dxsum_part) {
    __shared__ float red[2304];
    const int rowlen = PCB * 8 + 1;
#pragma unroll
    for (int k = 0; k < 8; ++k) red[wl * rowlen + pc * 8 + k] = s[k];
    __syncthreads();
    for (int cl = threadIdx.x; cl < PCB * 8; cl += 256) {
      float t = 0.f;
      for (int r = 0; r < WL; ++r) t += red[r * rowlen + cl];
      const int c = blockIdx.x * PCB * 8 + cl;
      if (c < C) dxsum_part[(long)blockIdx.y * C + c] = t;
    }
  }
}

__global__ __launch_bounds__(1024) void colsum_finalize_kernel(const float* part, int nblk, int C, float* out, int accumulate) {
  __shared__ double s1[32][33];
  const int cl = threadIdx.x & 31, rg = threadIdx.x >> 5;
  const int c = blockIdx.x * 32 + cl;
  double a = 0.0;
  if (c < C)
    for (int i = rg; i < nblk; i += 32) a += (double)part[(long)i * C + c];
  s1[rg][cl] = a;
  __syncthreads();
  if (rg == 0 && c < C) {
    for (int k = 1; k < 32; ++k) a += s1[k][cl];
    out[c] = accumulate ? out[c] + (float)a : (float)a;
  }
}

inline int ew_grid(long total) {
  long b = (total + 255) / 256;
  if (b > 2048 * 4) b = 2048 * 4;
  if (b < 1) b = 1;
  return (int)b;
}

inline int host_pcb(int C) {
  int p = 1;
  while (p < 32 && p * 8 < C) p <<= 1;
  return p;
}

inline int red_blocks(int B, int H, int W, int C) {
  const long nwin = (long)B * ((H + 1) / 2) * ((W + 1) / 2);
  const int pcb = host_pcb(C), wl = 256 / pcb;
  long want = 1536 / cdiv(C / 8, pcb);
  if (want < 1) want = 1;
  long nb = (nwin + wl - 1) / wl;
  if (nb > want) nb = want;
  if (nb < 1) nb = 1;
  return (int)nb;
}

}

extern "C" int s2s_bn_finalize_b(const float* part, int nblk, int C, long count, const float* gamma,
                                 const float* beta, float* running_mean, float* running_var, long* num_batches,
                                 float momentum, float eps, float* mean, float* invstd, float* scale, float* shift,
                                 const float* conv_bias, void* stream) {
  if (!part || !gamma || !beta || !mean || !invstd || !scale || !shift) return S2S_ERR_NULL;
  if (nblk <= 0 || C <= 0 || count <= 0) return S2S_ERR_SHAPE;
  if (finalize_tpc(nblk) == 256)
    hipLaunchKernelGGL(bn_finalize_kernel<256>, dim3(C), dim3(256), 0, (hipStream_t)stream, part, nblk, C,
                       (double)count, gamma, beta, running_mean, running_var, num_batches, momentum, eps, mean,
                       invstd, scale, shift, conv_bias);
  else
    hipLaunchKernelGGL(bn_finalize_kernel<64>, dim3(cdiv(C, 4)), dim3(256), 0, (hipStream_t)stream, part, nblk, C,
                       (double)count, gamma, beta, running_mean, running_var, num_batches, momentum, eps, mean,
                       invstd, scale, shift, conv_bias);
  S2S_LAUNCH_CHECK();
  return S2S_OK;
}

extern "C" int s2s_bn_finalize(const float* part, int nblk, int C, long count, const float* gamma,
                               const float* beta, float* running_mean, float* running_var, long* num_batches,
                               float momentum, float eps, float* mean, float* invstd, float* scale, float* shift,
                               void* stream) {
  return s2s_bn_finalize_b(part, nblk, C, count, gamma, beta, running_mean, running_var, num_batches, momentum, eps, mean,
                           invstd, scale, shift, nullptr, stream);
}

extern "C" int s2s_bn_partial_sums(const float* part, int nblk, int C, float* sums, void* stream) {
  if (!part || !sums) return S2S_ERR_NULL;
  if (nblk <= 0 || C <= 0) return S2S_ERR_SHAPE;
  if (finalize_tpc(nblk) == 256)
    hipLaunchKernelGGL(bn_partial_sums_kernel<256>, dim3(C), dim3(256), 0, (hipStream_t)stream, part, nblk, C, sums);
  else
    hipLaunchKernelGGL(bn_partial_sums_kernel<64>, dim3(cdiv(C, 4)), dim3(256), 0, (hipStream_t)stream, part, nblk, C, sums);
  S2S_LAUNCH_CHECK();
  return S2S_OK;
}

extern "C" int s2s_bn_eval_prepare(int C, const float* gamma, const float* beta, const float* rmean,
                                   const float* rvar, float eps, float* scale, float* shift, void* stream) {
  if (!gamma || !beta || !rmean || !rvar || !scale || !shift) return S2S_ERR_NULL;
  if (C <= 0) return S2S_ERR_SHAPE;
  hipLaunchKernelGGL(bn_eval_prepare_kernel, dim3(cdiv(C, 256)), dim3(256), 0, (hipStream_t)stream, C, gamma, beta,
                     rmean, rvar, eps, scale, shift);
  S2S_LAUNCH_CHECK();
  return S2S_OK;
}

extern "C" int s2s_bn_relu_apply(int dtype, const void* x, int ldx, const float* scale, const float* shift, void* y,
                                 int ldy, void* pool, int ldp, int B, int H, int W, int C, void* stream) {
  if (!x || !scale || !shift || !y) return S2S_ERR_NULL;
  if (B <= 0 || H <= 0 || W <= 0 || C <= 0 || (C % 8) || (ldx % 8) || (ldy % 8) || (pool && (ldp % 8)))
    return S2S_ERR_SHAPE;
  const long total = (long)B * ((H + 1) / 2) * ((W + 1) / 2) * (C / 8);
  hipStream_t s = (hipStream_t)stream;
  if (dtype == S2S_BF16)
    hipLaunchKernelGGL(bn_relu_apply_kernel<bf16_t>, dim3(ew_grid(total)), dim3(256), 0, s, (const bf16_t*)x, ldx,
                       scale, shift, (bf16_t*)y, ldy, (bf16_t*)pool, ldp, B, H, W, C);
  else if (dtype == S2S_F32)
    hipLaunchKernelGGL(bn_relu_apply_kernel<float>, dim3(ew_grid(total)), dim3(256), 0, s, (const float*)x, ldx,
                       scale, shift, (float*)y, ldy, (float*)pool, ldp, B, H, W, C);
  else return S2S_ERR_DTYPE;
  S2S_LAUNCH_CHECK();
  return S2S_OK;
}

extern "C" int s2s_maxpool2(int dtype, const void* x, int ldx, void* pool, int ldp, int B, int H, int W, int C,
                            void* stream) {
  if (!x || !pool) return S2S_ERR_NULL;
  if (B <= 0 || H < 2 || W < 2 || C <= 0 || (C % 8) || (ldx % 8) || (ldp % 8)) return S2S_ERR_SHAPE;
  const long total = (long)B * (H / 2) * (W / 2) * (C / 8);
  hipStream_t s = (hipStream_t)stream;
  if (dtype == S2S_BF16)
    hipLaunchKernelGGL(maxpool2_kernel<bf16_t>, dim3(ew_grid(total)), dim3(256), 0, s, (const bf16_t*)x, ldx,
                       (bf16_t*)pool, ldp, B, H, W, C);
  else if (dtype == S2S_F32)
    hipLaunchKernelGGL(maxpool2_kernel<float>, dim3(ew_grid(total)), dim3(256), 0, s, (const float*)x, ldx,
                       (float*)pool, ldp, B, H, W, C);
  else return S2S_ERR_DTYPE;
  S2S_LAUNCH_CHECK();
  return S2S_OK;
}

extern "C" int s2s_bn_bwd_blocks(int B, int H, int W, int C) {
  if (B <= 0 || H <= 0 || W <= 0 || C <= 0) return S2S_ERR_SHAPE;
  return red_blocks(B, H, W, C);
}

extern "C" int s2s_bn_relu_bwd_phase(int dtype, const void* g1, int ldg1, const void* gp, int ldgp, const float* scale,
                               const float* shift, const void* x, int ldx, const float* mean, const float* invstd, const float* gamma,
                               float* dgamma, float* dbeta, float* dbias_conv, int accumulate, void* dx, int lddx,
                               float* work, int B, int H, int W, int C, long count_total, int phases, void* stream) {
  if (phases < 1 || phases > 3 || count_total < (long)B * H * W) return S2S_ERR_SHAPE;
  if ((!g1 && !gp) || !scale || !shift || !x || !mean || !invstd || !gamma || !dgamma || !dbeta || !dx || !work) return S2S_ERR_NULL;
  if (B <= 0 || H <= 0 || W <= 0 || C <= 0 || (C % 8) || (ldx % 8) || (lddx % 8) ||
      (g1 && (ldg1 % 8)) || (gp && (ldgp % 8)))
    return S2S_ERR_SHAPE;
  if ((long)B * ((H + 1) / 2) * ((W + 1) / 2) >= (1L << 31) - (1 << 20)) return S2S_ERR_SHAPE;
  const int nb = red_blocks(B, H, W, C);
  float* part = work;
  float* part2 = work + (long)nb * 2 * C;
  float* c1 = part2 + (long)nb * 2 * C;
  float* c2 = c1 + C;
  const double count = (double)count_total;
  hipStream_t s = (hipStream_t)stream;
  float* const dbias_zero = (dbias_conv && !accumulate) ? dbias_conv : nullptr;
  dbias_conv = nullptr;
  dim3 grid(cdiv(C / 8, host_pcb(C)), nb);
  constexpr int bn_rev = 1;
#define S2S_BN_BWD(TT)                                                                                             \
  if (!(phases & 1)) {                                                                                             \
  } else if (gp) {                                                                                                 \
    hipLaunchKernelGGL(bn_relu_bwd_reduce_kernel<TT>, grid, dim3(256), 0, s, (const TT*)g1, ldg1, (const TT*)gp,   \
                       ldgp, scale, shift, (const TT*)x, ldx, mean, invstd, part, B, H, W, C);                \
  } else {                                                                                                         \
    hipLaunchKernelGGL(bn_relu_bwd_reduce_flat_kernel<TT>, grid, dim3(256), 0, s, (const TT*)g1, ldg1,             \
                       scale, shift, (const TT*)x, ldx, mean, invstd, part, (long)B * H * W, C);              \
  }                                                                                                                \
  if (!(phases & 1)) {                                                                                             \
  } else if (finalize_tpc(nb) == 256)                                                                              \
    hipLaunchKernelGGL(bn_bwd_finalize_kernel<256>, dim3(C), dim3(256), 0, s, part, nb, C, count, dgamma, dbeta,   \
                       accumulate, c1, c2, dbias_zero);                                                            \
  else                                                                                                             \
    hipLaunchKernelGGL(bn_bwd_finalize_kernel<64>, dim3(cdiv(C, 4)), dim3(256), 0, s, part, nb, C, count, dgamma,  \
                       dbeta, accumulate, c1, c2, dbias_zero);                                                     \
  if (!(phases & 2)) {                                                                                             \
  } else if (gp) {                                                                                                 \
    hipLaunchKernelGGL(bn_relu_bwd_apply_kernel<TT>, grid, dim3(256), 0, s, (const TT*)g1, ldg1, (const TT*)gp,    \
                       ldgp, scale, shift, (const TT*)x, ldx, mean, invstd, gamma, c1, c2, (TT*)dx, lddx,     \
                       dbias_conv ? part2 : nullptr, B, H, W, C);                                                  \
  } else {                                                                                                         \
    hipLaunchKernelGGL(bn_relu_bwd_apply_flat_kernel<TT>, grid, dim3(256), 0, s, (const TT*)g1, ldg1,              \
                       scale, shift, (const TT*)x, ldx, mean, invstd, gamma, c1, c2, (TT*)dx, lddx,           \
                       dbias_conv ? part2 : nullptr, (long)B * H * W, C, bn_rev);                                  \
  }
  if (dtype == S2S_BF16) { S2S_BN_BWD(bf16_t) }
  else if (dtype == S2S_F32) { S2S_BN_BWD(float) }
  else return S2S_ERR_DTYPE;
#undef S2S_BN_BWD
  if (dbias_conv && (phases & 2))
    hipLaunchKernelGGL(colsum_finalize_kernel, dim3(cdiv(C, 32)), dim3(1024), 0, s, part2, prereduce(part2, nb, C, s),
                       C, dbias_conv, accumulate);
  S2S_LAUNCH_CHECK();
  return S2S_OK;
}

int s2s_internal_tail_bn_sums(int dtype, const void* raw, int ldx, const float* g_nchw, const float* w, const float* scale,
                              const float* shift, const float* mean, const float* invstd, float* work, float* dgamma,
                              float* dbeta, float* zero_out, int accumulate, int B, int H, int W, int C, int Cout,
                              hipStream_t s) {
  const int nb = red_blocks(B, H, W, C);
  float* const c1 = work + (long)2 * C * nb;
  const long npix = (long)B * H * W;
  dim3 grid(cdiv(C / 8, host_pcb(C)), nb);
  if (dtype == S2S_BF16)
    hipLaunchKernelGGL(bn_relu_bwd_reduce_tail_kernel<bf16_t>, grid, dim3(256), 0, s, g_nchw, w, Cout, H * W, scale, shift,
                       (const bf16_t*)raw, ldx, mean, invstd, work, npix, C);
  else if (dtype == S2S_F32)
    hipLaunchKernelGGL(bn_relu_bwd_reduce_tail_kernel<float>, grid, dim3(256), 0, s, g_nchw, w, Cout, H * W, scale, shift,
                       (const float*)raw, ldx, mean, invstd, work, npix, C);
  else return S2S_ERR_DTYPE;
  if (finalize_tpc(nb) == 256)
    hipLaunchKernelGGL(bn_bwd_finalize_kernel<256>, dim3(C), dim3(256), 0, s, work, nb, C, (double)npix, dgamma, dbeta,
                       accumulate, c1, c1 + C, zero_out);
  else
    hipLaunchKernelGGL(bn_bwd_finalize_kernel<64>, dim3(cdiv(C, 4)), dim3(256), 0, s, work, nb, C, (double)npix, dgamma,
                       dbeta, accumulate, c1, c1 + C, zero_out);
  return S2S_OK;
}

extern "C" int s2s_bn_relu_bwd(int dtype, const void* g1, int ldg1, const void* gp, int ldgp, const float* scale,
                               const float* shift, const void* x, int ldx, const float* mean, const float* invstd, const float* gamma,
                               float* dgamma, float* dbeta, float* dbias_conv, int accumulate, void* dx, int lddx,
                               float* work, int B, int H, int W, int C, void* stream) {
  return s2s_bn_relu_bwd_phase(dtype, g1, ldg1, gp, ldgp, scale, shift, x, ldx, mean, invstd, gamma, dgamma, dbeta,
                               dbias_conv, accumulate, dx, lddx, work, B, H, W, C, (long)B * H * W, 3, stream);
}
```

stain2stain_amd/engine.py:

```python
from __future__ import annotations

from dataclasses import dataclass, field
from typing import Dict, List, Optional, Sequence, Tuple

import contextlib
import threading

import torch
import torch.distributed as dist

from . import ops

BN_EPS = 1e-5
BN_MOMENTUM = 0.1


class SyncBNExchange:

    def __init__(self, process_group=None):
        if not (dist.is_available() and dist.is_initialized()):
            raise RuntimeError("stain2stain_amd: SyncBatchNorm needs an initialised torch.distributed process group")
        self.pg = process_group
        self.world = dist.get_world_size(process_group)
        self._host = dist.get_backend(process_group) != "nccl"

    def __call__(self, t: torch.Tensor) -> None:
        if self._host and t.is_cuda:
            h = t.cpu()
            dist.all_reduce(h, op=dist.ReduceOp.SUM, group=self.pg)
            t.copy_(h)
        else:
            dist.all_reduce(t, op=dist.ReduceOp.SUM, group=self.pg)


sync_bn: Optional[SyncBNExchange] = None
_module_exchanges: Dict[int, SyncBNExchange] = {}


def _module_exchange(bn: torch.nn.Module) -> Optional[SyncBNExchange]:
    if not isinstance(bn, torch.nn.SyncBatchNorm) or not (dist.is_available() and dist.is_initialized()):
        return None
    pg = bn.process_group
    import os
    if dist.get_world_size(pg) < 2 and os.environ.get("S2S_FORCE_DDP") != "1":
        return None
    key = id(pg) if pg is not None else 0
    ex = _module_exchanges.get(key)
    if ex is None or ex.pg is not pg:
        ex = _module_exchanges[key] = SyncBNExchange(pg)
    return ex


@contextlib.contextmanager
def sync_batchnorm(exchange: Optional[SyncBNExchange]):
    global sync_bn
    prev, sync_bn = sync_bn, exchange
    try:
        yield
    finally:
        sync_bn = prev


mutation_epoch = [0]


class ConvBN:

    def __init__(self, prefix: str, i_conv: str, i_bn: str, seq: torch.nn.Sequential):
        self.prefix = prefix
        self.idx = (i_conv, i_bn)
        self._seq = seq
        self._pack: Dict[torch.dtype, Tuple] = {}
        self._pack_key: Dict[torch.dtype, Tuple] = {}
        self._eval_key, self._eval_ss = None, None

    @property
    def conv(self) -> torch.nn.Conv2d:
        return self._seq._modules[self.idx[0]]

    @property
    def bn(self) -> torch.nn.BatchNorm2d:
        return self._seq._modules[self.idx[1]]

    @property
    def cout(self) -> int:
        return self.conv.weight.shape[0]

    @property
    def cin(self) -> int:
        return self.conv.weight.shape[1]

    def packed(self, dtype: torch.dtype):
        w = self.conv.weight
        key = (w.data_ptr(), w._version, w.device)
        if self._pack_key.get(dtype) != key:
            old = self._pack.get(dtype)
            reuse = old if (old is not None and old[0].device == w.device) else None
            self._pack[dtype] = ops.pack_conv3x3(w.detach(), dtype, want_dgrad=True, out=reuse)
            self._pack_key[dtype] = key
        return self._pack[dtype]

    def invalidate(self) -> None:
        self._pack_key.clear()

    def eval_affine(self):
        bn = self.bn
        ts = (bn.weight, bn.bias, bn.running_mean, bn.running_var)
        key = (mutation_epoch[0],) + tuple((t.data_ptr(), t._version) for t in ts)
        if self._eval_key != key:
            self._eval_ss = ops.bn_eval_prepare(bn.weight.detach(), bn.bias.detach(), bn.running_mean,
                                                bn.running_var, bn.eps)
            self._eval_key = key
        return self._eval_ss

    def ensure_buffers(self, dtype: torch.dtype):
        old = self._pack.get(dtype)
        w = self.conv.weight
        if old is None or old[0].device != w.device:
            L = ops._L()
            wf = torch.empty((L.s2s_pack_conv3x3_fwd_elems(self.cout, self.cin),), dtype=dtype, device=w.device)
            wd = torch.empty((L.s2s_pack_conv3x3_dgrad_elems(self.cout, self.cin),), dtype=dtype, device=w.device)
            self._pack[dtype] = (wf, wd)
            self._pack_key.pop(dtype, None)
        return self._pack[dtype]

    def mark_packed(self, dtype: torch.dtype) -> None:
        w = self.conv.weight
        self._pack_key[dtype] = (w.data_ptr(), w._version, w.device)


def _pack_table(cbs: Sequence[ConvBN], dtype: torch.dtype) -> Tuple[torch.Tensor, int]:
    rows, start = [], 0
    for cb in cbs:
        wf, wd = cb.ensure_buffers(dtype)
        rows.append([cb.conv.weight.data_ptr(), wf.data_ptr(), wd.data_ptr(), cb.cout, cb.cin, start])
        start += ((cb.cout + 31) // 32) * ((cb.cin + 31) // 32)
    return torch.tensor(rows, dtype=torch.int64, device=cbs[0].conv.weight.device), start


class Conv3x3Packer:

    def __init__(self, blocks: Sequence[Tuple[ConvBN, ConvBN]], dtype: torch.dtype):
        stem = blocks[0][0]
        self.convs = [cb for pair in blocks for cb in pair
                      if cb is not stem or (dtype == torch.bfloat16 and cb.cin <= 8)]
        self.dtype = dtype
        self.desc, self.total = _pack_table(self.convs, dtype)
        self.repack()

    def repack(self) -> None:
        ops.pack_conv3x3_batched(self.desc, self.total, self.dtype)
        for cb in self.convs:
            cb.mark_packed(self.dtype)


_REPACK_DESC: Dict[tuple, Tuple[torch.Tensor, int]] = {}


def repack_stale(cbs: Sequence[ConvBN], dtype: torch.dtype) -> None:
    stale = []
    for cb in cbs:
        w = cb.conv.weight
        if not w.is_cuda:
            return
        if cb._pack_key.get(dtype) != (w.data_ptr(), w._version, w.device):
            stale.append(cb)
    if len(stale) < 2:
        return
    bufs = [cb.ensure_buffers(dtype) for cb in stale]
    key = (dtype,) + tuple((cb.conv.weight.data_ptr(), b[0].data_ptr(), b[1].data_ptr(), cb.cout, cb.cin)
                           for cb, b in zip(stale, bufs))
    hit = _REPACK_DESC.get(key)
    if hit is None:
        if len(_REPACK_DESC) > 64:
            _REPACK_DESC.clear()
        hit = _REPACK_DESC[key] = _pack_table(stale, dtype)
    ops.pack_conv3x3_batched(hit[0], hit[1], dtype)
    for cb in stale:
        cb.mark_packed(dtype)


@dataclass
class LayerCtx:
    x0: Optional[torch.Tensor]
    x1: Optional[torch.Tensor]
    raw: torch.Tensor
    act: Optional[torch.Tensor]
    stats: torch.Tensor
    count: Optional[int] = None
    sync: Optional["SyncBNExchange"] = None


@dataclass
class EncCtx:
    dtype: torch.dtype
    x_nchw: torch.Tensor
    layers: List[Tuple[LayerCtx, LayerCtx]] = field(default_factory=list)
    feats: List[torch.Tensor] = field(default_factory=list)


@dataclass
class DecCtx:
    dtype: torch.dtype
    t_emb: torch.Tensor
    h1: torch.Tensor = None
    a1: torch.Tensor = None
    h2: torch.Tensor = None
    lows: List[torch.Tensor] = field(default_factory=list)
    ups: List[torch.Tensor] = field(default_factory=list)
    skips: List[torch.Tensor] = field(default_factory=list)
    layers: List[Tuple[LayerCtx, LayerCtx]] = field(default_factory=list)
    v: torch.Tensor = None
    tail: Optional[Tuple[torch.Tensor, torch.Tensor]] = None


def _stem_as_conv(x_nchw: torch.Tensor, dtype: torch.dtype) -> bool:
    return dtype == torch.bfloat16 and x_nchw.shape[1] <= 8


def _stem_image(x_nchw: torch.Tensor, dtype: torch.dtype) -> torch.Tensor:
    B, _, H, W = x_nchw.shape
    return ops.p2p_pack_input(x_nchw, None, torch.empty((B, H, W, 8), dtype=dtype, device=x_nchw.device))


def _conv_bn_stats(cb: ConvBN, x0, x1, dtype, stem: bool = False):
    bn = cb.bn
    bias = cb.conv.bias.detach() if cb.conv.bias is not None else None
    late_bias = None
    if stem and _stem_as_conv(x0, dtype):
        raw, stat = ops.conv3x3(_stem_image(x0, dtype), None, cb.packed(dtype)[0], None, cb.cout, want_stats=True)
        late_bias = bias
    elif stem:
        raw, stat = ops.stem_fwd(x0, cb.conv.weight.detach(), bias, dtype, want_stats=True)
    elif dtype == torch.bfloat16 and bias is not None:
        raw, stat = ops.conv3x3(x0, x1, cb.packed(dtype)[0], None, cb.cout, want_stats=True)
        late_bias = bias
    else:
        raw, stat = ops.conv3x3(x0, x1, cb.packed(dtype)[0], bias, cb.cout, want_stats=True)
    count = raw.shape[0] * raw.shape[1] * raw.shape[2]
    sx = sync_bn if sync_bn is not None else _module_exchange(bn)
    if sx is not None:
        sums = ops.bn_partial_sums(stat)
        sx(sums)
        stat = sums.view(2, -1, 1)
        count *= sx.world
    if count <= 1:
        raise ValueError(f"Expected more than 1 value per channel when training, got input size "
                         f"{[raw.shape[0], raw.shape[3], raw.shape[1], raw.shape[2]]}")
    track = bn.track_running_stats and bn.running_mean is not None
    mutation_epoch[0] += 1
    st = ops.bn_finalize(stat, count, bn.weight.detach(), bn.bias.detach(),
                         bn.running_mean if track else None, bn.running_var if track else None,
                         bn.num_batches_tracked if track else None,
                         BN_MOMENTUM if bn.momentum is None else bn.momentum, bn.eps, conv_bias=late_bias)
    return raw, st, count, sx


def _conv_bn_relu(cb: ConvBN, x0, x1, dtype, training: bool, want_pool: bool = False, stem: bool = False):
    bias = cb.conv.bias.detach() if cb.conv.bias is not None else None
    if training:
        raw, st, count, sx = _conv_bn_stats(cb, x0, x1, dtype, stem)
        act, pooled = ops.bn_relu_apply(raw, st[2], st[3], want_pool=want_pool)
        return LayerCtx(x0, x1, raw, act, st, count if sx is not None else None, sx), act, pooled
    ss = cb.eval_affine()
    if stem and _stem_as_conv(x0, dtype):
        act, _ = ops.conv3x3(_stem_image(x0, dtype), None, cb.packed(dtype)[0], bias, cb.cout, scale=ss[0], shift=ss[1], relu=True)
        pooled = ops.maxpool2(act) if want_pool else None
    elif stem:
        raw, _ = ops.stem_fwd(x0, cb.conv.weight.detach(), bias, dtype, want_stats=False)
        act, pooled = ops.bn_relu_apply(raw, ss[0], ss[1], want_pool=want_pool)
    else:
        act, _ = ops.conv3x3(x0, x1, cb.packed(dtype)[0], bias, cb.cout, scale=ss[0], shift=ss[1], relu=True)
        pooled = ops.maxpool2(act) if want_pool else None
    return None, act, pooled


class _SideState(threading.local):
    stream: Optional[torch.cuda.Stream] = None
    keep: Optional[List[torch.Tensor]] = None


_side = _SideState()


@contextlib.contextmanager
def side_scope(stream: Optional[torch.cuda.Stream]):
    prev = _side.stream, _side.keep
    _side.stream, _side.keep = stream, []
    try:
        yield
    finally:
        try:
            join_side(stream)
        finally:
            _side.stream, _side.keep = prev


def current_side() -> Optional[torch.cuda.Stream]:
    return _side.stream


def run_on_side(fn, keep=()) -> None:
    side = _side.stream
    if side is None:
        fn()
        return
    ev = torch.cuda.Event()
    ev.record()
    with torch.cuda.stream(side):
        side.wait_event(ev)
        fn()
    _side.keep.extend(t for t in keep if t is not None)


def join_side(side: Optional[torch.cuda.Stream]) -> None:
    if side is not None:
        torch.cuda.current_stream().wait_stream(side)


def _g(grads: Dict[str, torch.Tensor], name: str) -> torch.Tensor:
    try:
        return grads[name]
    except KeyError as e:
        raise RuntimeError(f"stain2stain_amd: no gradient buffer for parameter {name!r}") from e


def _conv_bn_relu_bwd(cb: ConvBN, lc: LayerCtx, g1, gp, grads, accumulate: bool, need_dx: bool, stem: bool = False):
    p = cb.prefix
    i_conv, i_bn = cb.idx
    dgamma = _g(grads, f"{p}.{i_bn}.weight")
    dbeta = _g(grads, f"{p}.{i_bn}.bias")
    dbias = _g(grads, f"{p}.{i_conv}.bias") if cb.conv.bias is not None else None
    draw = ops.bn_relu_bwd(g1, gp, lc.raw, lc.stats, cb.bn.weight.detach(), dgamma, dbeta, dbias, accumulate,
                           exchange=lc.sync, count_total=lc.count)
    dw = _g(grads, f"{p}.{i_conv}.weight")
    if stem:
        run_on_side(lambda: ops.stem_wgrad(draw, lc.x0, dw, None, accumulate), (draw,))
        return None
    run_on_side(lambda: ops.conv3x3_wgrad(draw, lc.x0, lc.x1, dw, accumulate), (draw,))
    if not need_dx:
        return None
    dx, _ = ops.conv3x3(draw, None, cb.packed(draw.dtype)[1], None, cb.cin)
    return dx


def _conv_bn_tail(cb: ConvBN, x0, dtype):
    raw, st, count, sx = _conv_bn_stats(cb, x0, None, dtype)
    if sx is not None:
        act, _ = ops.bn_relu_apply(raw, st[2], st[3])
        return LayerCtx(x0, None, raw, act, st, count, sx), act
    return LayerCtx(x0, None, raw, None, st), None


def decoder_tail_loss(dec, ctx: DecCtx, u_nchw: torch.Tensor, grads: Dict[str, torch.Tensor], want_v: bool = False,
                      accumulate: bool = False):
    cb = dec.up_blocks[-1][1]
    lc = ctx.layers[-1][1]
    p = cb.prefix
    i_conv, i_bn = cb.idx
    loss, g, v, work = ops.tail_fwd_loss(
        lc.raw, lc.stats, dec.outc.weight.detach(), dec.outc.bias.detach() if dec.outc.bias is not None else None,
        u_nchw, _g(grads, "outc.weight"), _g(grads, "outc.bias") if dec.outc.bias is not None else None,
        _g(grads, f"{p}.{i_bn}.weight"), _g(grads, f"{p}.{i_bn}.bias"),
        _g(grads, f"{p}.{i_conv}.bias") if cb.conv.bias is not None else None, want_v=want_v, accumulate=accumulate)
    ctx.tail = (g, work)
    ctx.v = v
    return loss, v


def _conv_bn_tail_bwd(dec, cb: ConvBN, lc: LayerCtx, tail, grads, accumulate: bool):
    g, work = tail
    draw = ops.tail_bwd_apply(lc.raw, lc.stats, dec.outc.weight.detach(), g, cb.bn.weight.detach(), work)
    dw = _g(grads, f"{cb.prefix}.{cb.idx[0]}.weight")
    run_on_side(lambda: ops.conv3x3_wgrad(draw, lc.x0, lc.x1, dw, accumulate), (draw,))
    dx, _ = ops.conv3x3(draw, None, cb.packed(draw.dtype)[1], None, cb.cin)
    return dx


def encoder_forward(blocks: Sequence[Tuple[ConvBN, ConvBN]], x_nchw: torch.Tensor, dtype: torch.dtype,
                    training: bool) -> EncCtx:
    ctx = EncCtx(dtype, x_nchw)
    nlev = len(blocks)
    repack_stale([cb for l, pair in enumerate(blocks) for j, cb in enumerate(pair)
                  if (l, j) != (0, 0) or _stem_as_conv(x_nchw, dtype)], dtype)
    inp = x_nchw
    for l, (c1, c2) in enumerate(blocks):
        lc1, a1, _ = _conv_bn_relu(c1, inp, None, dtype, training, stem=(l == 0))
        lc2, a2, pooled = _conv_bn_relu(c2, a1, None, dtype, training, want_pool=(l + 1 < nlev))
        ctx.layers.append((lc1, lc2))
        ctx.feats.append(a2)
        inp = pooled
    return ctx


def encoder_backward(blocks: Sequence[Tuple[ConvBN, ConvBN]], ctx: EncCtx, dfeats: Sequence[Optional[torch.Tensor]],
                     grads: Dict[str, torch.Tensor], accumulate: bool = False, on_group_done=None) -> None:
    gpool = None
    nlev = len(blocks)
    for l in range(len(blocks) - 1, -1, -1):
        c1, c2 = blocks[l]
        lc1, lc2 = ctx.layers[l]
        g1 = dfeats[l]
        if g1 is None and gpool is None:
            raise RuntimeError("stain2stain_amd: encoder level without any incoming gradient")
        ga1 = _conv_bn_relu_bwd(c2, lc2, g1, gpool, grads, accumulate, need_dx=True)
        if on_group_done is not None:
            on_group_done()
        gpool = _conv_bn_relu_bwd(c1, lc1, ga1, None, grads, accumulate, need_dx=(l > 0), stem=(l == 0))
        if on_group_done is not None:
            on_group_done()


def decoder_forward(dec, bottleneck: torch.Tensor, skips: Sequence[torch.Tensor], t_emb: torch.Tensor,
                    dtype: torch.dtype, training: bool, with_head: bool = True, fuse_tail: bool = False) -> DecCtx:
    fuse_tail = (fuse_tail and training and not with_head and len(dec.up_blocks) > 0
                 and ops.tail_fusable(dec.up_blocks[-1][1].cout, dec.outc.weight.shape[0]))
    ctx = DecCtx(dtype, t_emb)
    repack_stale([cb for pair in dec.up_blocks for cb in pair], dtype)
    tbias = None
    if getattr(dec, "time_mlp", None) is not None:
        l0, l2 = dec.time_mlp[0], dec.time_mlp[2]
        ctx.h1 = ops.linear_fwd(t_emb, l0.weight.detach(), l0.bias.detach())
        ctx.a1 = ops.silu_fwd(ctx.h1)
        ctx.h2 = ops.linear_fwd(ctx.a1, l2.weight.detach(), l2.bias.detach())
        tbias = ops.linear_fwd(ctx.h2, dec.time_proj.weight.detach(), dec.time_proj.bias.detach())
    x = bottleneck
    for i, ((c1, c2), skip) in enumerate(zip(dec.up_blocks, skips)):
        B, Hs, Ws, _ = skip.shape
        up = torch.empty((B, Hs, Ws, x.shape[3]), dtype=dtype, device=x.device)
        ops.upsample2x_fwd(x, up, tbias if i == 0 else None)
        lc1, a1, _ = _conv_bn_relu(c1, skip, up, dtype, training)
        if fuse_tail and i == len(dec.up_blocks) - 1:
            lc2, a2 = _conv_bn_tail(c2, a1, dtype)
        else:
            lc2, a2, _ = _conv_bn_relu(c2, a1, None, dtype, training)
        ctx.lows.append(x); ctx.ups.append(up); ctx.skips.append(skip); ctx.layers.append((lc1, lc2))
        x = a2
    ctx.lows.append(x)
    if not with_head:
        return ctx
    ctx.v = ops.head_fwd(x, dec.outc.weight.detach(), dec.outc.bias.detach() if dec.outc.bias is not None else None)
    return ctx


def decoder_backward(dec, ctx: DecCtx, dv: Optional[torch.Tensor], grads: Dict[str, torch.Tensor],
                     accumulate: bool = False, need_dt_emb: bool = False, on_group_done=None,
                     g_head: Optional[torch.Tensor] = None):
    if ctx.tail is not None:
        g = None
    elif g_head is not None:
        g = g_head
    else:
        g = ops.head_bwd(dv, ctx.lows[-1], dec.outc.weight.detach(), _g(grads, "outc.weight"),
                         _g(grads, "outc.bias") if dec.outc.bias is not None else None, accumulate)
    if on_group_done is not None:
        on_group_done()
    nup = len(ctx.layers)
    dskips: List[torch.Tensor] = [None] * len(ctx.layers)
    for i in range(len(ctx.layers) - 1, -1, -1):
        c1, c2 = dec.up_blocks[i]
        lc1, lc2 = ctx.layers[i]
        if ctx.tail is not None and i == nup - 1:
            ga1 = _conv_bn_tail_bwd(dec, c2, lc2, ctx.tail, grads, accumulate)
        else:
            ga1 = _conv_bn_relu_bwd(c2, lc2, g, None, grads, accumulate, need_dx=True)
        if on_group_done is not None:
            on_group_done()
        dcat = _conv_bn_relu_bwd(c1, lc1, ga1, None, grads, accumulate, need_dx=True)
        cs = ctx.skips[i].shape[3]
        dskips[i] = dcat[..., :cs]
        low = ctx.lows[i]
        g = ops.upsample2x_bwd(dcat[..., cs:], low.shape[1], low.shape[2])
        if on_group_done is not None:
            on_group_done()
    dbott = g
    if getattr(dec, "time_mlp", None) is None:
        return dbott, dskips, None
    dtb = ops.pixel_sum(g)
    l0, l2 = dec.time_mlp[0], dec.time_mlp[2]
    dh2 = ops.linear_bwd(dtb, ctx.h2, dec.time_proj.weight.detach(), _g(grads, "time_proj.weight"),
                         _g(grads, "time_proj.bias"), True, accumulate)
    da1 = ops.linear_bwd(dh2, ctx.a1, l2.weight.detach(), _g(grads, "time_mlp.2.weight"),
                         _g(grads, "time_mlp.2.bias"), True, accumulate)
    dh1 = ops.silu_bwd(ctx.h1, da1)
    dt_emb = ops.linear_bwd(dh1, ctx.t_emb, l0.weight.detach(), _g(grads, "time_mlp.0.weight"),
                            _g(grads, "time_mlp.0.bias"), need_dt_emb, accumulate)
    if on_group_done is not None:
        on_group_done()
    return dbott, dskips, dt_emb
```

stain2stain_amd/multitask_trainer.py:

```python
from __future__ import annotations

from typing import Dict, List, Optional, Tuple

import torch
import torch.distributed as dist

from . import engine, evaluation, ops
from .components import FlowMatchingDecoder, SegmentationDecoder, SharedEncoder
from .ddp import all_reduce_mean_scalar
from .ema import TrainerEMA
from .fused_step import FlatParams


def _layer_groups(named: Dict[str, torch.nn.Parameter], prefix: str, owner: str) -> List[List[Tuple[str, torch.nn.Parameter]]]:
    out = []
    for idx in (("3.", "4."), ("0.", "1.")):
        out.append([(f"{owner}.{n}", p) for n, p in named.items() if any(n.startswith(prefix + i) for i in idx)])
    return out


def _decoder_groups(dec, owner: str) -> List[List[Tuple[str, torch.nn.Parameter]]]:
    named = dict(dec.named_parameters())
    groups = [[(f"{owner}.{n}", p) for n, p in named.items() if n.startswith("outc.")]]
    for i in range(len(dec.ups) - 1, -1, -1):
        groups += _layer_groups(named, f"ups.{i}.conv.double_conv.", owner)
    if getattr(dec, "time_mlp", None) is not None:
        groups.append([(f"{owner}.{n}", p) for n, p in named.items() if n.startswith("time_")])
    return groups


def _encoder_groups(enc, owner: str) -> List[List[Tuple[str, torch.nn.Parameter]]]:
    named = dict(enc.named_parameters())
    groups = []
    for i in range(len(enc.downs) - 1, -1, -1):
        groups += _layer_groups(named, f"downs.{i}.maxpool_conv.1.double_conv.", owner)
    return groups + _layer_groups(named, "inc.double_conv.", owner)


class MultiTaskTrainer:

    def __init__(self, encoder: SharedEncoder, flow_decoder: FlowMatchingDecoder, seg_decoder: SegmentationDecoder,
                 time_emb_dim: int = 256, lr: float = 1e-4, weight_decay: float = 1e-5,
                 betas: Tuple[float, float] = (0.9, 0.999), eps: float = 1e-8, seg_loss_weight: float = 1.0,
                 dice_weight: float = 0.5, dice_smooth: float = 1.0, num_classes: Optional[int] = None,
                 ignore_index: int = -100, sigma: float = 0.0, bucket_mb: float = 4.0, process_group=None,
                 sync_loss: bool = True, max_bucket_mb: float = 16.0, sharded_optimizer: bool = False,
                 ema_decay: Optional[float] = None, ema_buffers: bool = True):
        dev = next(encoder.parameters()).device
        if dev.type != "cuda":
            raise RuntimeError("stain2stain_amd: MultiTaskTrainer needs the networks on a GPU (HIP-only implementation)")
        if not (encoder.compute_dtype == flow_decoder.compute_dtype == seg_decoder.compute_dtype):
            raise ValueError("encoder and decoders must share one precision")
        self.encoder, self.flow_decoder, self.seg_decoder = encoder, flow_decoder, seg_decoder
        self.time_emb_dim, self.sigma = time_emb_dim, sigma
        self.lr, self.wd, self.betas, self.eps = lr, weight_decay, tuple(betas), eps
        self.seg_loss_weight, self.dice_weight, self.dice_smooth = seg_loss_weight, dice_weight, dice_smooth
        self.num_classes, self.ignore_index = num_classes, ignore_index
        self.pg, self.sync_loss = process_group, sync_loss
        self._dtype = encoder.compute_dtype
        groups = _decoder_groups(seg_decoder, "seg_decoder") + _decoder_groups(flow_decoder, "flow_decoder") \
            + _encoder_groups(encoder, "encoder")
        n_named = sum(1 for m in (encoder, flow_decoder, seg_decoder) for _ in m.parameters())
        if sum(len(g) for g in groups) != n_named or any(not g for g in groups):
            raise RuntimeError("parameter grouping does not cover the networks")
        self.fp = FlatParams(groups, bucket_mb, process_group, max_bucket_mb, sharded_optimizer)
        gr = self.fp.grads
        self.grads_enc = {k[len("encoder."):]: v for k, v in gr.items() if k.startswith("encoder.")}
        self.grads_flow = {k[len("flow_decoder."):]: v for k, v in gr.items() if k.startswith("flow_decoder.")}
        self.grads_seg = {k[len("seg_decoder."):]: v for k, v in gr.items() if k.startswith("seg_decoder.")}
        from .ddp import broadcast_from_rank0
        broadcast_from_rank0([b for m in (encoder, flow_decoder, seg_decoder) for b in m.buffers()], process_group)
        self.packer = engine.Conv3x3Packer(list(encoder._blocks) + list(flow_decoder.up_blocks)
                                           + list(seg_decoder.up_blocks), self._dtype)
        self._side = ops.side_stream_for(dev)
        self.overlap_wgrad = True
        self.fuse_tail = True
        self._group = 0
        self._eval_owner = object()
        self._generation = evaluation.GenerationEval()
        self._ema = None
        if ema_decay is not None:
            self.fp.enable_ema(ema_decay)
            self._ema = TrainerEMA(self.fp, [encoder, flow_decoder, seg_decoder], ema_buffers)

    @property
    def step_count(self) -> int:
        return self.fp.step_count

    def _group_done(self) -> None:
        self.fp.bucketer.mark_ready_ordered(self._group, self._side if self.overlap_wgrad else None)
        self._group += 1

    def forward_backward(self, source: torch.Tensor, target: torch.Tensor, mask: torch.Tensor,
                         t: Optional[torch.Tensor] = None, want_outputs: bool = False):
        enc, fdec, sdec = self.encoder, self.flow_decoder, self.seg_decoder
        dt = self._dtype
        x0, x1 = source.float().contiguous(), target.float().contiguous()
        B = x0.shape[0]
        if t is None:
            t = torch.rand(B, device=x0.device, dtype=torch.float32)
        t = t.float().contiguous()
        eps_noise = torch.randn_like(x0) if self.sigma != 0.0 else None
        xt, ut = ops.cfm_sample(x0, x1, t, self.sigma, eps_noise)
        ectx1 = engine.encoder_forward(enc._blocks, xt, dt, True)
        temb = ops.time_embedding(t, self.time_emb_dim)
        f1 = ectx1.feats
        dctx_f = engine.decoder_forward(fdec, f1[-1], f1[:-1][::-1], temb, dt, True, with_head=False,
                                        fuse_tail=self.fuse_tail and not want_outputs)
        ectx2 = engine.encoder_forward(enc._blocks, x0, dt, True)
        f2 = ectx2.feats
        dctx_s = engine.decoder_forward(sdec, f2[-1], f2[:-1][::-1], None, dt, True)
        logits = dctx_s.v
        if dctx_f.lows[-1] is None:
            g_head = None
            flow, v = engine.decoder_tail_loss(fdec, dctx_f, ut, self.grads_flow, want_v=want_outputs)
        else:
            flow, g_head, v = ops.head_loss_fused(dctx_f.lows[-1], fdec.outc.weight.detach(),
                                                  fdec.outc.bias.detach() if fdec.outc.bias is not None else None, ut,
                                                  self.grads_flow["outc.weight"], self.grads_flow.get("outc.bias"),
                                                  want_v=want_outputs)
        w = float(self.seg_loss_weight)
        if self.num_classes is not None:
            tgt = mask[:, 0] if (mask.dim() == 4 and mask.shape[1] == 1) else mask
            seg3, dz = ops.seg_loss_multiclass(logits, tgt.long(), self.ignore_index, self.dice_smooth, self.dice_weight,
                                               want_grad=True, grad_scale=w, validate=False)
        else:
            seg3, dz = ops.seg_loss(logits, mask.float().reshape(logits.shape), self.dice_smooth, self.dice_weight,
                                    want_grad=True, grad_scale=w)
        total = flow + w * seg3[0]
        self.fp.bucketer.start_step()
        self._group = 0
        with engine.side_scope(self._side if self.overlap_wgrad else None):
            L = len(f1) - 1
            dbs, dss, _ = engine.decoder_backward(sdec, dctx_s, dz, self.grads_seg, on_group_done=self._group_done)
            dbf, dsf, _ = engine.decoder_backward(fdec, dctx_f, None, self.grads_flow, g_head=g_head,
                                                  on_group_done=self._group_done)
            engine.encoder_backward(enc._blocks, ectx2, [dss[L - 1 - l] for l in range(L)] + [dbs], self.grads_enc)
            engine.encoder_backward(enc._blocks, ectx1, [dsf[L - 1 - l] for l in range(L)] + [dbf], self.grads_enc,
                                    accumulate=True, on_group_done=self._group_done)
        second = "seg_ce" if self.num_classes is not None else "seg_bce"
        losses = {"total": total, "flow": flow, "seg": seg3[0], "seg_dice": seg3[1], second: seg3[2]}
        return losses, ({"v": v, "logits": logits} if want_outputs else None)

    def optimizer_step(self) -> None:
        engine.join_side(self._side)
        self.fp.adam(self.lr, self.betas, self.eps, self.wd)
        if self._ema is not None:
            self._ema.update_buffers()
        self.packer.repack()
        engine.mutation_epoch[0] += 1
        if self._ema is not None:
            self._ema.after_step()

    def _ema_on(self) -> TrainerEMA:
        if self._ema is None:
            raise RuntimeError("stain2stain_amd: this trainer keeps no EMA (construct it with ema_decay=...)")
        return self._ema

    def ema_model(self) -> Tuple[SharedEncoder, FlowMatchingDecoder, SegmentationDecoder]:
        return tuple(self._ema_on().modules())

    def _ema_container(self) -> torch.nn.ModuleDict:
        enc, fdec, sdec = self._ema_on().copies
        return torch.nn.ModuleDict(dict(encoder=enc, flow_decoder=fdec, seg_decoder=sdec))

    def ema_state_dict(self) -> Dict[str, torch.Tensor]:
        ema = self._ema_on()
        ema.modules()
        return ema.state_dict(self._ema_container().state_dict())

    def load_ema_state_dict(self, sd: Dict[str, torch.Tensor]) -> None:
        self._ema_on().load_state_dict(sd, self._ema_container())

    def step(self, source: torch.Tensor, target: torch.Tensor, mask: torch.Tensor,
             t: Optional[torch.Tensor] = None) -> torch.Tensor:
        losses, _ = self.forward_backward(source, target, mask, t)
        total = losses["total"]
        work = all_reduce_mean_scalar(total, self.pg) if self.sync_loss else None
        self.optimizer_step()
        if work is not None:
            work.wait()
            total = total / dist.get_world_size(self.pg)
        return total

    def evaluate(self, source: torch.Tensor, target: torch.Tensor, mask: torch.Tensor, t: Optional[torch.Tensor] = None,
                 accumulator: Optional[evaluation.EvalAccumulator] = None,
                 use_ema: bool = False) -> Dict[str, torch.Tensor]:
        with ops.workspace_owner(self._eval_owner), evaluation.eval_grad_mode():
            x0, x1 = source.float().contiguous(), target.float().contiguous()
            if t is None:
                t = torch.rand(x0.shape[0], device=x0.device, dtype=torch.float32)
            t = t.float().contiguous()
            eps_noise = torch.randn_like(x0) if self.sigma != 0.0 else None
            xt, ut = ops.cfm_sample(x0, x1, t, self.sigma, eps_noise)
            enc, fdec, sdec = self.ema_model() if use_ema else (self.encoder, self.flow_decoder, self.seg_decoder)
            flow = evaluation.flow_loss(enc, fdec, self.time_emb_dim, xt, t, ut)
            logits = evaluation.mask_logits(enc, sdec, x0)
            d = evaluation.segmentation_values(logits, mask, self.num_classes, self.ignore_index, self.dice_smooth,
                                               self.dice_weight)
            second = "seg_ce" if self.num_classes is not None else "seg_bce"
            out = {"loss": flow + float(self.seg_loss_weight) * d["seg"], "flow_loss": flow, "seg_loss": d["seg"],
                   "seg_dice": d["seg_dice"], second: d[second], "dice_coef": d["dice_coef"], "iou": d["iou"]}
        if accumulator is not None:
            accumulator.add(out, x0.shape[0])
        return out

    def evaluate_generation(self, source: torch.Tensor, target: torch.Tensor, num_steps: int = 50,
                            method: str = "euler", graph: bool = False, use_ema: bool = False,
                            accumulator: Optional[evaluation.EvalAccumulator] = None,
                            quantize: bool = True, stain: Optional[dict] = None) -> Dict[str, torch.Tensor]:
        enc, fdec, _ = self.ema_model() if use_ema else (self.encoder, self.flow_decoder, self.seg_decoder)
        with ops.workspace_owner(self._eval_owner), evaluation.eval_grad_mode():
            return evaluation.generation_values(self._generation, bool(use_ema), enc, fdec, self.time_emb_dim, source,
                                                target, num_steps, method, graph, quantize, accumulator, stain)

    def close(self) -> None:
        self._generation.close()
        ops.release_workspaces(self._eval_owner)

    def __del__(self):
        try:
            self.close()
        except Exception:
            pass
```

stain2stain_amd/ops.py:

```python
from __future__ import annotations

import contextlib
import ctypes
import os
import sys
from typing import Optional, Tuple

import torch

from . import _native

BF16, F32 = 0, 1


def _dt(t: torch.Tensor) -> int:
    if t.dtype == torch.bfloat16:
        return BF16
    if t.dtype == torch.float32:
        return F32
    raise RuntimeError(f"stain2stain_amd: unsupported activation dtype {t.dtype}")


_raw_stream = getattr(torch._C, "_cuda_getCurrentRawStream", None)
_raw_device = getattr(torch._C, "_cuda_getDevice", None)
# ... 20 lines not shown
    return torch.cuda.current_stream().cuda_stream


def _nhwc(t: torch.Tensor) -> Tuple[int, int]:
    if not t.is_cuda:
        raise RuntimeError("stain2stain_amd: tensor is not on the GPU (there is no CPU path)")
    if t.dim() != 4 or t.stride(3) != 1:
        raise RuntimeError("stain2stain_amd: expected an NHWC view with contiguous channels")
    b, h, w, _ = t.shape
    ld = t.stride(2) if w > 1 else (t.stride(1) if h > 1 else (t.stride(0) if b > 1 else t.shape[3]))
    if w > 1 and h > 1 and t.stride(1) != w * ld:
        raise RuntimeError("stain2stain_amd: NHWC view has a row pitch")
    if b > 1 and t.stride(0) != h * w * ld:
        raise RuntimeError("stain2stain_amd: NHWC view has an image pitch")
    return t.data_ptr(), ld


def _f32(t: Optional[torch.Tensor]) -> int:
    if t is None:
        return 0
    if t.dtype != torch.float32 or not t.is_cuda or not t.is_contiguous():
        raise RuntimeError("stain2stain_amd: expected a contiguous fp32 GPU tensor")
    return t.data_ptr()


def _ptr(t: Optional[torch.Tensor]) -> int:
    if t is None:
        return 0
    if not t.is_cuda or not t.is_contiguous():
        raise RuntimeError("stain2stain_amd: expected a contiguous GPU tensor")
    return t.data_ptr()


def _L():
    return _native.lib()


_WORKSPACE = {}
_WS_OWNER = 0


class workspace_owner:
    def __init__(self, owner):
        self.key = id(owner)

    def __enter__(self):
        global _WS_OWNER
        self.prev, _WS_OWNER = _WS_OWNER, self.key
        return self

    def __exit__(self, *exc):
        global _WS_OWNER
        _WS_OWNER = self.prev
        return False


def release_workspaces(owner) -> None:
    k = id(owner)
    for key in [key for key in _WORKSPACE if key[3] == k]:
        del _WORKSPACE[key]


def _workspace(device: torch.device, numel: int, tag: str) -> torch.Tensor:
    key = (device.index if device.index is not None else torch.cuda.current_device(), tag, _stream(), _WS_OWNER)
    buf = _WORKSPACE.get(key)
    if buf is None or buf.numel() < numel:
        buf = torch.empty((max(numel, 1 << 20),), dtype=torch.float32, device=device)
        _WORKSPACE[key] = buf
    return buf[:numel]


_PROFILE: Optional[list] = None
_PROFILE_ONLY: Optional[set] = None
PROFILE_TAG = ""


@contextlib.contextmanager
def profile_tag(tag: str):
    global PROFILE_TAG
    prev, PROFILE_TAG = PROFILE_TAG, tag
    try:
        yield
    finally:
        PROFILE_TAG = prev


def profile_start(only=None) -> None:
    global _PROFILE, _PROFILE_ONLY
    _PROFILE = []
    _PROFILE_ONLY = set(only) if only else None


def cu_masked_stream(device, spec: str) -> torch.cuda.Stream:
    k, m = (int(v) for v in spec.split(":"))
    if not 0 < k <= m:
        raise ValueError("CU mask spec K:M needs 0 < K <= M")
    dev = torch.device(device)
    key = (dev.index if dev.index is not None else torch.cuda.current_device(), k, m)
    if key in _MASKED_STREAMS:
        return _MASKED_STREAMS[key]
    n = torch.cuda.get_device_properties(dev).multi_processor_count
    words = (ctypes.c_uint32 * ((n + 31) // 32))()
    for i in range(n):
        if i % m < k:
            words[i // 32] |= 1 << (i % 32)
    out = ctypes.c_long(0)
    with torch.cuda.device(dev):
        _native.check(_L().s2s_stream_create_cu_mask(ctypes.addressof(words), len(words), ctypes.addressof(out)),
                      "stream_create_cu_mask")
    stream = torch.cuda.ExternalStream(out.value, device=dev)
    _MASKED_STREAMS[key] = stream
    return stream


_MASKED_STREAMS = {}


def side_stream_for(device) -> Optional[torch.cuda.Stream]:
    import os
    if os.environ.get("S2S_WGRAD_STREAM", "1") == "0":
        return None
    spec = os.environ.get("S2S_WGRAD_CUS", "")
    if spec and spec != "0":
        return cu_masked_stream(device, spec)
    return torch.cuda.Stream(device=device)


_SHARED_SIDE = {}


def shared_side_stream(device) -> Optional[torch.cuda.Stream]:
    dev = torch.device(device)
    key = dev.index if dev.index is not None else torch.cuda.current_device()
    if key not in _SHARED_SIDE:
        _SHARED_SIDE[key] = side_stream_for(dev)
    return _SHARED_SIDE[key]


class TimingEvent:

    def __init__(self):
        out = ctypes.c_long(0)
        _native.check(_L().s2s_event_create(1, ctypes.addressof(out)), "event_create")
        self._e = out.value

    def record(self) -> None:
        _native.check(_L().s2s_event_record(self._e, _stream()), "event_record")

    def elapsed_time(self, end: "TimingEvent") -> float:
        ms = ctypes.c_float(0.0)
        _native.check(_L().s2s_event_synchronize(end._e), "event_synchronize")
        _native.check(_L().s2s_event_elapsed_ms(self._e, end._e, ctypes.addressof(ms)), "event_elapsed")
        return float(ms.value)

    def __del__(self):
        try:
            if self._e and not sys.is_finalizing():
                _L().s2s_event_destroy(self._e)
        except Exception:
            pass


def _timing_event():
    if os.environ.get("S2S_TIMING_EVENTS", "1") == "0":
        return torch.cuda.Event(enable_timing=True)
    return TimingEvent()


def profile_stop() -> list:
    global _PROFILE
    out, _PROFILE = _PROFILE or [], None
    return out


def _timed(name: str, work_fn=None):
    def deco(fn):
        def wrapped(*args, **kwargs):
            if _PROFILE is None or (_PROFILE_ONLY is not None and name not in _PROFILE_ONLY):
                return fn(*args, **kwargs)
            e0 = _timing_event()
            e1 = _timing_event()
            e0.record()
            out = fn(*args, **kwargs)
            e1.record()
            _PROFILE.append((name + ("@" + PROFILE_TAG if PROFILE_TAG else ""), work_fn(*args, **kwargs) if work_fn else 0.0, e0, e1))
            return out
        wrapped.__name__ = fn.__name__
        wrapped.__doc__ = fn.__doc__
        return wrapped
    return deco


def _conv_flops(x0, x1, w_packed, bias, cout, **kw) -> float:
    B, H, W, c0 = x0.shape
    cin = c0 + (x1.shape[3] if x1 is not None else 0)
    return 2.0 * B * H * W * cout * 9 * cin


def _wgrad_flops(dy, x0, x1, grad_oihw, accumulate=False) -> float:
    B, H, W, cout = dy.shape
    cin = x0.shape[3] + (x1.shape[3] if x1 is not None else 0)
    return 2.0 * B * H * W * cout * 9 * cin


@_timed("conv3x3_mfma", _conv_flops)
def conv3x3(x0: torch.Tensor, x1: Optional[torch.Tensor], w_packed: torch.Tensor, bias: Optional[torch.Tensor],
            cout: int, *, want_stats: bool = False, scale: Optional[torch.Tensor] = None,
            shift: Optional[torch.Tensor] = None, relu: bool = False, out: Optional[torch.Tensor] = None):
    B, H, W, c0 = x0.shape
    dt = _dt(x0)
    p0, ld0 = _nhwc(x0)
    p1, ld1, c1 = 0, 8, 0
    if x1 is not None:
        if x1.shape[:3] != x0.shape[:3] or x1.dtype != x0.dtype:
            raise RuntimeError("stain2stain_amd: conv3x3 sources disagree in shape/dtype")
        p1, ld1 = _nhwc(x1)
        c1 = x1.shape[3]
    if w_packed.dtype != x0.dtype or w_packed.numel() != _L().s2s_pack_conv3x3_fwd_elems(cout, c0 + c1):
        raise RuntimeError("stain2stain_amd: packed weight does not match (cout, cin, dtype)")
    if out is None:
        out = torch.empty((B, H, W, cout), dtype=x0.dtype, device=x0.device)
    elif out.shape != (B, H, W, cout) or out.dtype != x0.dtype:
        raise RuntimeError("stain2stain_amd: conv3x3 output buffer mismatch")
    py, ldy = _nhwc(out)
    stat, nb = None, 0
    if want_stats:
        nb = _L().s2s_conv3x3_stat_rows(dt, B, H, W, cout, c0, c1, ld0, ld1, int(bias is not None))
        _native.check(min(nb, 0), "conv3x3_stat_rows")
        stat = torch.empty((2, cout, nb), dtype=torch.float32, device=x0.device)
    kwork = None
    if not want_stats:
        nsplit = _L().s2s_conv3x3_ksplit(dt, B, H, W, cout, c0 + c1)
        if nsplit > 1:
            kwork = torch.empty((nsplit, B * H * W, cout), dtype=torch.float32, device=x0.device)
    rc = _L().s2s_conv3x3_nhwc_s(dt, p0, ld0, c0, p1, ld1, c1, _ptr(w_packed), _f32(bias), py, ldy, _f32(stat), nb,
                                 _f32(scale), _f32(shift), int(relu), _f32(kwork), B, H, W, cout, _stream())
    _native.check(rc, "conv3x3")
    return out, stat


def conv3x3_wgrad(dy: torch.Tensor, x0: torch.Tensor, x1: Optional[torch.Tensor], grad_oihw: torch.Tensor,
                  accumulate: bool = False) -> None:
    B, H, W, cout = dy.shape
    c0 = x0.shape[3]
    dt = _dt(dy)
    if x0.dtype != dy.dtype or x0.shape[:3] != dy.shape[:3]:
        raise RuntimeError("stain2stain_amd: conv3x3_wgrad operand mismatch")
    pdy, lddy = _nhwc(dy)
    p0, ld0 = _nhwc(x0)
    p1, ld1, c1 = 0, 8, 0
    if x1 is not None:
        p1, ld1 = _nhwc(x1)
        c1 = x1.shape[3]
    if tuple(grad_oihw.shape) != (cout, c0 + c1, 3, 3):
        raise RuntimeError("stain2stain_amd: conv3x3_wgrad gradient buffer has the wrong shape")
    s = _L().s2s_conv3x3_wgrad_splits(dt, B, H, W, c0 + c1, cout)
    part = _workspace(dy.device, s * 9 * cout * (c0 + c1), "wgrad")
    if _PROFILE is not None and (_PROFILE_ONLY is None or "conv3x3_wgrad_mfma" in _PROFILE_ONLY):
        for name, phase, work in (("conv3x3_wgrad_mfma", 1, _wgrad_flops(dy, x0, x1, grad_oihw)), ("wgrad_fold", 2, 0.0)):
            e0 = _timing_event()
            e1 = _timing_event()
            e0.record()
            rc = _L().s2s_conv3x3_wgrad_phase(dt, pdy, lddy, cout, p0, ld0, c0, p1, ld1, c1, _f32(part), _f32(grad_oihw),
                                              int(accumulate), B, H, W, phase, _stream())
            e1.record()
            _native.check(rc, "conv3x3_wgrad")
            _PROFILE.append((name, work, e0, e1))
        return
    rc = _L().s2s_conv3x3_wgrad_nhwc(dt, pdy, lddy, cout, p0, ld0, c0, p1, ld1, c1, _f32(part), _f32(grad_oihw),
                                     int(accumulate), B, H, W, _stream())
    _native.check(rc, "conv3x3_wgrad")


@_timed("stem_fwd")
def stem_fwd(x_nchw: torch.Tensor, w: torch.Tensor, bias: Optional[torch.Tensor], dtype: torch.dtype,
             want_stats: bool = True):
    B, cin, H, W = x_nchw.shape
    cout = w.shape[0]
    if tuple(w.shape) != (cout, cin, 3, 3):
        raise RuntimeError("stain2stain_amd: stem weight shape")
    y = torch.empty((B, H, W, cout), dtype=dtype, device=x_nchw.device)
    stat = None
    if want_stats:
        stat = torch.empty((2, cout, _L().s2s_stem_stat_blocks(B, H, W)), dtype=torch.float32, device=y.device)
    rc = _L().s2s_stem_conv3x3_fwd(_dt(y), _f32(x_nchw), _f32(w), _f32(bias), y.data_ptr(), cout, _f32(stat), B, H, W,
                                   cin, cout, _stream())
    _native.check(rc, "stem_conv3x3_fwd")
    return y, stat


@_timed("stem_wgrad")
def stem_wgrad(dy: torch.Tensor, x_nchw: torch.Tensor, dw: torch.Tensor, dbias: Optional[torch.Tensor],
               accumulate: bool = False) -> None:
    B, H, W, cout = dy.shape
    cin = x_nchw.shape[1]
    pdy, lddy = _nhwc(dy)
    nb = _L().s2s_stem_wgrad_blocks(B, H, W)
    part = torch.empty(((cin + 2) // 3, 2 * nb, cout, 32), dtype=torch.float32, device=dy.device)
    rc = _L().s2s_stem_conv3x3_wgrad(_dt(dy), pdy, lddy, _f32(x_nchw), _f32(part), _f32(dw), _f32(dbias),
                                     int(accumulate), B, H, W, cin, cout, _stream())
    _native.check(rc, "stem_conv3x3_wgrad")


@_timed("head_fwd")
def head_fwd(x: torch.Tensor, w: torch.Tensor, bias: Optional[torch.Tensor]) -> torch.Tensor:
    B, H, W, C = x.shape
    cout = w.shape[0]
    px, ldx = _nhwc(x)
    y = torch.empty((B, cout, H, W), dtype=torch.float32, device=x.device)
    rc = _L().s2s_head_conv1x1_fwd(_dt(x), px, ldx, _f32(w.reshape(cout, C)), _f32(bias), _f32(y), B, H, W, C, cout,
                                   _stream())
    _native.check(rc, "head_conv1x1_fwd")
    return y


@_timed("head_bwd")
def head_bwd(dy_nchw: torch.Tensor, x: torch.Tensor, w: torch.Tensor, dw: torch.Tensor, dbias: Optional[torch.Tensor],
             accumulate: bool = False) -> torch.Tensor:
    B, H, W, C = x.shape
    cout = w.shape[0]
    px, ldx = _nhwc(x)
    dx = torch.empty((B, H, W, C), dtype=x.dtype, device=x.device)
    nb = _L().s2s_head_wgrad_blocks(B, H, W)
    part = torch.empty((nb, cout, C + 1), dtype=torch.float32, device=x.device)
    rc = _L().s2s_head_conv1x1_bwd(_dt(x), _f32(dy_nchw), px, ldx, _f32(w.reshape(cout, C)), dx.data_ptr(), C,
                                   _f32(part), _f32(dw.reshape(cout, C)), _f32(dbias), int(accumulate), B, H, W, C,
                                   cout, _stream())
    _native.check(rc, "head_conv1x1_bwd")
    return dx


@_timed("head_loss_fused")
def head_loss_fused(x: torch.Tensor, w: torch.Tensor, bias: Optional[torch.Tensor], u_nchw: torch.Tensor,
                    dw: torch.Tensor, dbias: Optional[torch.Tensor], want_v: bool = False, grad_scale: float = 1.0,
                    accumulate: bool = False):
    B, H, W, C = x.shape
    cout = w.shape[0]
    px, ldx = _nhwc(x)
    dx = torch.empty((B, H, W, C), dtype=x.dtype, device=x.device)
    v = torch.empty((B, cout, H, W), dtype=torch.float32, device=x.device) if want_v else None
    nb = _L().s2s_head_loss_blocks(B, H, W)
    part = torch.empty((nb, cout, C + 1), dtype=torch.float32, device=x.device)
    lpart = torch.empty((nb,), dtype=torch.float64, device=x.device)
    loss = torch.empty((), dtype=torch.float32, device=x.device)
    rc = _L().s2s_head_loss_fused(_dt(x), px, ldx, _f32(w.reshape(cout, C)), _f32(bias), _f32(u_nchw), _f32(v),
                                  dx.data_ptr(), C, float(grad_scale), _f32(part), lpart.data_ptr(),
                                  _f32(dw.reshape(cout, C)), _f32(dbias), loss.data_ptr(), int(accumulate), B, H, W, C,
                                  cout, _stream())
    _native.check(rc, "head_loss_fused")
    return loss, dx, v


def tail_fusable(C: int, cout: int) -> bool:
    pcb = C // 8
    return C % 8 == 0 and 1 <= pcb <= 64 and pcb & (pcb - 1) == 0 and 1 <= cout <= 4


@_timed("tail_fwd_loss")
def tail_fwd_loss(raw: torch.Tensor, stats: torch.Tensor, w: torch.Tensor, bias: Optional[torch.Tensor],
                  u_nchw: torch.Tensor, dw: torch.Tensor, dbias: Optional[torch.Tensor], dgamma: torch.Tensor,
                  dbeta: torch.Tensor, dbias_conv: Optional[torch.Tensor], want_v: bool = False,
                  grad_scale: float = 1.0, accumulate: bool = False):
    B, H, W, C = raw.shape
    cout = w.shape[0]
    if not tail_fusable(C, cout):
        raise RuntimeError(f"stain2stain_amd: the fused tail does not take C = {C}, cout = {cout}")
    px, ldx = _nhwc(raw)
    dev = raw.device
    g = torch.empty((B, cout, H, W), dtype=torch.float32, device=dev)
    v = torch.empty((B, cout, H, W), dtype=torch.float32, device=dev) if want_v else None
    nb = _L().s2s_tail_blocks(B, H, W)
    part = torch.empty((nb, cout, C + 1), dtype=torch.float32, device=dev)
    lpart = torch.empty((nb,), dtype=torch.float64, device=dev)
    work = torch.empty((2 * C * _L().s2s_bn_bwd_blocks(B, H, W, C) + 2 * C,), dtype=torch.float32, device=dev)
    loss = torch.empty((), dtype=torch.float32, device=dev)
    rc = _L().s2s_tail_fwd_loss(_dt(raw), px, ldx, stats[2].data_ptr(), stats[3].data_ptr(), stats[0].data_ptr(),
                                stats[1].data_ptr(), _f32(w.reshape(cout, C)), _f32(bias), _f32(u_nchw), _f32(v),
                                _f32(g), float(grad_scale), _f32(part), lpart.data_ptr(), _f32(work),
                                _f32(dw.reshape(cout, C)), _f32(dbias), loss.data_ptr(), _f32(dgamma), _f32(dbeta),
                                _f32(dbias_conv), int(accumulate), B, H, W, C, cout, _stream())
    _native.check(rc, "tail_fwd_loss")
    return loss, g, v, work


@_timed("tail_bwd_apply")
def tail_bwd_apply(raw: torch.Tensor, stats: torch.Tensor, w: torch.Tensor, g: torch.Tensor, gamma: torch.Tensor,
                   work: torch.Tensor) -> torch.Tensor:
    B, H, W, C = raw.shape
    cout = w.shape[0]
    px, ldx = _nhwc(raw)
    if tuple(g.shape) != (B, cout, H, W) or work.numel() != 2 * C * _L().s2s_bn_bwd_blocks(B, H, W, C) + 2 * C:
        raise RuntimeError("stain2stain_amd: tail_bwd_apply operands do not belong to this tail_fwd_loss")
    dx = torch.empty((B, H, W, C), dtype=raw.dtype, device=raw.device)
    rc = _L().s2s_tail_bwd_apply(_dt(raw), px, ldx, _f32(g), _f32(w.reshape(cout, C)), stats[2].data_ptr(),
                                 stats[3].data_ptr(), stats[0].data_ptr(), stats[1].data_ptr(), _f32(gamma),
                                 _f32(work), dx.data_ptr(), C, B, H, W, C, cout, _stream())
    _native.check(rc, "tail_bwd_apply")
    return dx


@_timed("bn_finalize")
def bn_finalize(stat: torch.Tensor, count: int, gamma, beta, running_mean, running_var, num_batches,
                momentum: float = 0.1, eps: float = 1e-5, conv_bias: Optional[torch.Tensor] = None):
    _, C, nblk = stat.shape
    dev = stat.device
    out = torch.empty((4, C), dtype=torch.float32, device=dev)
    rc = _L().s2s_bn_finalize_b(_f32(stat), nblk, C, count, _f32(gamma), _f32(beta), _f32(running_mean),
                                _f32(running_var), 0 if num_batches is None else num_batches.data_ptr(), momentum, eps,
                                out[0].data_ptr(), out[1].data_ptr(), out[2].data_ptr(), out[3].data_ptr(),
                                _f32(conv_bias), _stream())
    _native.check(rc, "bn_finalize")
    return out


def bn_partial_sums(stat: torch.Tensor) -> torch.Tensor:
    _, C, nblk = stat.shape
    sums = torch.empty((2, C), dtype=torch.float32, device=stat.device)
    _native.check(_L().s2s_bn_partial_sums(_f32(stat), nblk, C, _f32(sums), _stream()), "bn_partial_sums")
    return sums


def bn_eval_prepare(gamma, beta, rmean, rvar, eps: float = 1e-5):
    C = gamma.numel()
    out = torch.empty((2, C), dtype=torch.float32, device=gamma.device)
    rc = _L().s2s_bn_eval_prepare(C, _f32(gamma), _f32(beta), _f32(rmean), _f32(rvar), eps, out[0].data_ptr(),
                                  out[1].data_ptr(), _stream())
    _native.check(rc, "bn_eval_prepare")
    return out


@_timed("bn_relu_apply")
def bn_relu_apply(x: torch.Tensor, scale: torch.Tensor, shift: torch.Tensor, out: Optional[torch.Tensor] = None,
                  pool: Optional[torch.Tensor] = None, want_pool: bool = False):
    B, H, W, C = x.shape
    px, ldx = _nhwc(x)
    if out is None:
        out = torch.empty((B, H, W, C), dtype=x.dtype, device=x.device)
    py, ldy = _nhwc(out)
    pp, ldp = 0, 8
    if want_pool and pool is None:
        pool = torch.empty((B, H // 2, W // 2, C), dtype=x.dtype, device=x.device)
    if pool is not None:
        pp, ldp = _nhwc(pool)
    rc = _L().s2s_bn_relu_apply(_dt(x), px, ldx, _f32(scale), _f32(shift), py, ldy, pp, ldp, B, H, W, C, _stream())
    _native.check(rc, "bn_relu_apply")
    return out, pool


@_timed("maxpool2")
def maxpool2(x: torch.Tensor) -> torch.Tensor:
    B, H, W, C = x.shape
    px, ldx = _nhwc(x)
    pool = torch.empty((B, H // 2, W // 2, C), dtype=x.dtype, device=x.device)
    rc = _L().s2s_maxpool2(_dt(x), px, ldx, pool.data_ptr(), C, B, H, W, C, _stream())
    _native.check(rc, "maxpool2")
    return pool


@_timed("bn_relu_bwd")
def bn_relu_bwd(g1: Optional[torch.Tensor], gp: Optional[torch.Tensor], x: torch.Tensor,
                stats: torch.Tensor, gamma: torch.Tensor, dgamma: torch.Tensor, dbeta: torch.Tensor,
                dbias_conv: Optional[torch.Tensor], accumulate: bool = False, exchange=None,
                count_total: Optional[int] = None) -> torch.Tensor:
    B, H, W, C = x.shape
    px, ldx = _nhwc(x)
    p1, ld1 = (0, 8) if g1 is None else _nhwc(g1)
    p2, ld2 = (0, 8) if gp is None else _nhwc(gp)
    dx = torch.empty((B, H, W, C), dtype=x.dtype, device=x.device)
    nb = _L().s2s_bn_bwd_blocks(B, H, W, C)
    work = torch.empty((4 * nb * C + 2 * C,), dtype=torch.float32, device=x.device)
    if exchange is not None:
        for phase in (1, 2):
            rc = _L().s2s_bn_relu_bwd_phase(_dt(x), p1, ld1, p2, ld2, stats[2].data_ptr(), stats[3].data_ptr(), px, ldx,
                                            stats[0].data_ptr(), stats[1].data_ptr(),
                                            _f32(gamma), _f32(dgamma), _f32(dbeta), _f32(dbias_conv), int(accumulate),
                                            dx.data_ptr(), C, _f32(work), B, H, W, C,
                                            int(count_total if count_total is not None else B * H * W), phase, _stream())
            _native.check(rc, "bn_relu_bwd")
            if phase == 1:
                exchange(work[4 * nb * C:])
        return dx
    rc = _L().s2s_bn_relu_bwd(_dt(x), p1, ld1, p2, ld2, stats[2].data_ptr(), stats[3].data_ptr(), px, ldx,
                              stats[0].data_ptr(), stats[1].data_ptr(),
                              _f32(gamma), _f32(dgamma), _f32(dbeta), _f32(dbias_conv), int(accumulate),
                              dx.data_ptr(), C, _f32(work), B, H, W, C, _stream())
    _native.check(rc, "bn_relu_bwd")
    return dx


@_timed("upsample2x_fwd")
def upsample2x_fwd(x: torch.Tensor, out: torch.Tensor, bias_nc: Optional[torch.Tensor] = None,
                   _reference: bool = False) -> None:
    B, Hin, Win, C = x.shape
    _, Hout, Wout, Co = out.shape
    if Co != C or out.dtype != x.dtype:
        raise RuntimeError("stain2stain_amd: upsample output slice mismatch")
    px, ldx = _nhwc(x)
    py, ldy = _nhwc(out)
    fn = _L().s2s_upsample2x_bilinear_ac_fwd_ref if _reference else _L().s2s_upsample2x_bilinear_ac_fwd
    rc = fn(_dt(x), px, ldx, _f32(bias_nc), py, ldy, B, Hin, Win, Hout, Wout, C, _stream())
    _native.check(rc, "upsample2x_fwd")


def upsample2x_fwd_family(x: torch.Tensor, out: torch.Tensor, _reference: bool = False) -> int:
    B, Hin, Win, C = x.shape
    _, Hout, Wout, _ = out.shape
    rc = _L().s2s_upsample2x_fwd_family(_nhwc(x)[1], _nhwc(out)[1], B, Hin, Win, Hout, Wout, C, int(_reference))
    if rc < 0:
        _native.check(rc, "upsample2x_fwd_family")
    return rc


@_timed("upsample2x_bwd")
def upsample2x_bwd(dy: torch.Tensor, hin: int, win: int, _reference: bool = False) -> torch.Tensor:
    B, Hout, Wout, C = dy.shape
    pdy, lddy = _nhwc(dy)
    dx = torch.empty((B, hin, win, C), dtype=dy.dtype, device=dy.device)
    fn = _L().s2s_upsample2x_bilinear_ac_bwd_ref if _reference else _L().s2s_upsample2x_bilinear_ac_bwd
    rc = fn(_dt(dy), pdy, lddy, dx.data_ptr(), C, B, hin, win, Hout, Wout, C, _stream())
    _native.check(rc, "upsample2x_bwd")
    return dx


def upsample2x_bwd_family(dy: torch.Tensor, hin: int, win: int, _reference: bool = False) -> int:
    B, Hout, Wout, C = dy.shape
    rc = _L().s2s_upsample2x_bwd_family(dy.stride(2), C, B, hin, win, Hout, Wout, C, int(_reference))
    if rc < 0:
        _native.check(rc, "upsample2x_bwd_family")
    return rc


def pixel_sum(x: torch.Tensor) -> torch.Tensor:
    B, H, W, C = x.shape
    px, ldx = _nhwc(x)
    out = torch.empty((B, C), dtype=torch.float32, device=x.device)
    rc = _L().s2s_pixel_sum(_dt(x), px, ldx, _f32(out), B, H * W, C, 0, _stream())
    _native.check(rc, "pixel_sum")
    return out


def time_embedding(t: torch.Tensor, dim: int) -> torch.Tensor:
    t = t.reshape(-1).to(torch.float32).contiguous()
    out = torch.empty((t.numel(), dim), dtype=torch.float32, device=t.device)
    _native.check(_L().s2s_time_embedding(_f32(t), _f32(out), t.numel(), dim, _stream()), "time_embedding")
    return out


def linear_fwd(x: torch.Tensor, w: torch.Tensor, b: Optional[torch.Tensor]) -> torch.Tensor:
    B, K = x.shape
    N = w.shape[0]
    y = torch.empty((B, N), dtype=torch.float32, device=x.device)
    _native.check(_L().s2s_linear_fwd(_f32(x), _f32(w), _f32(b), _f32(y), B, K, N, _stream()), "linear_fwd")
    return y


def linear_bwd(dy: torch.Tensor, x: torch.Tensor, w: torch.Tensor, dw: torch.Tensor, db: Optional[torch.Tensor],
               need_dx: bool = True, accumulate: bool = False) -> Optional[torch.Tensor]:
    B, K = x.shape
    N = w.shape[0]
    dx = torch.empty((B, K), dtype=torch.float32, device=x.device) if need_dx else None
    _native.check(_L().s2s_linear_bwd(_f32(dy), _f32(x), _f32(w), _f32(dx), _f32(dw), _f32(db), int(accumulate), B, K,
                                      N, _stream()), "linear_bwd")
    return dx


def silu_fwd(h: torch.Tensor) -> torch.Tensor:
    a = torch.empty_like(h)
    _native.check(_L().s2s_silu_fwd(_f32(h), _f32(a), h.numel(), _stream()), "silu_fwd")
    return a


def silu_bwd(h: torch.Tensor, da: torch.Tensor) -> torch.Tensor:
    dh = torch.empty_like(h)
    _native.check(_L().s2s_silu_bwd(_f32(h), _f32(da), _f32(dh), h.numel(), _stream()), "silu_bwd")
    return dh


@_timed("cfm_sample")
def cfm_sample(x0: torch.Tensor, x1: torch.Tensor, t: torch.Tensor, sigma: float = 0.0,
               eps: Optional[torch.Tensor] = None):
    xt = torch.empty_like(x0)
    ut = torch.empty_like(x0)
    B = x0.shape[0]
    _native.check(_L().s2s_cfm_sample(_f32(x0), _f32(x1), _f32(t), _f32(eps), float(sigma), _f32(xt), _f32(ut), B,
                                      x0.numel() // B, _stream()), "cfm_sample")
    return xt, ut


@_timed("mse_loss")
def mse_loss(v: torch.Tensor, u: torch.Tensor, want_grad: bool = True, grad_scale: float = 1.0):
    loss = torch.empty((), dtype=torch.float32, device=v.device)
    dv = torch.empty_like(v) if want_grad else None
    work = torch.empty((1024,), dtype=torch.float64, device=v.device)
    _native.check(_L().s2s_mse_loss(_f32(v), _f32(u), _f32(dv), float(grad_scale), loss.data_ptr(), work.data_ptr(),
                                    v.numel(), _stream()), "mse_loss")
    return loss, dv


def seg_loss(z: torch.Tensor, g: torch.Tensor, smooth: float = 1.0, dice_weight: float = 0.5, want_grad: bool = True,
             grad_scale: float = 1.0):
    z = z.contiguous()
    g = g.to(torch.float32).contiguous()
    out = torch.empty((3,), dtype=torch.float32, device=z.device)
    dz = torch.empty_like(z) if want_grad else None
    work = torch.empty((512 * 4 + 4,), dtype=torch.float64, device=z.device)
    _native.check(_L().s2s_seg_loss(_f32(z), _f32(g), _f32(dz), _f32(out), work.data_ptr(), z.numel(), float(smooth),
                                    float(dice_weight), float(grad_scale), _stream()), "seg_loss")
    return out, dz


def seg_loss_multiclass(z: torch.Tensor, target: torch.Tensor, ignore_index: int = -100, smooth: float = 1.0,
                        dice_weight: float = 0.5, want_grad: bool = True, grad_scale: float = 1.0,
                        validate: bool = True):
    if z.dim() != 4 or target.dim() != 3 or target.shape != (z.shape[0], z.shape[2], z.shape[3]):
        raise RuntimeError("stain2stain_amd: seg_loss_multiclass wants logits [B,C,H,W] and target [B,H,W]")
    B, C, H, W = z.shape
    z = z.contiguous()
    target = target.to(torch.int64).contiguous()
    if validate:
        lo, hi = int(target.min()), int(target.max())
        if lo < 0 or hi >= C:
            raise RuntimeError(f"stain2stain_amd: class index out of range [0, {C}) in segmentation target "
                               f"(min {lo}, max {hi})")
    out = torch.empty((3,), dtype=torch.float32, device=z.device)
    dz = torch.empty_like(z) if want_grad else None
    work = torch.empty((513 * 26,), dtype=torch.float64, device=z.device)
    _native.check(_L().s2s_seg_loss_multiclass(_f32(z), target.data_ptr(), _f32(dz), _f32(out), work.data_ptr(), B,
                                               H * W, C, int(ignore_index), float(smooth), float(dice_weight),
                                               float(grad_scale), _stream()), "seg_loss_multiclass")
    return out, dz


EV_BLOCKS = 512


def _gpu_f32_operand(t: torch.Tensor, what: str) -> torch.Tensor:
    if not t.is_cuda:
        raise RuntimeError(f"stain2stain_amd: {what} is not on the GPU (there is no CPU path)")
    if t.dtype != torch.float32:
        raise RuntimeError(f"stain2stain_amd: {what} must be float32, got {t.dtype}")
    return t.contiguous()


def _binary_mask(g: torch.Tensor) -> torch.Tensor:
    if g.dtype in (torch.bool, torch.uint8):
        return g.to(torch.float32).contiguous()
    if g.dtype != torch.float32:
        raise RuntimeError(f"stain2stain_amd: mask must be float32 (0/1), uint8 or bool, got {g.dtype}")
    return g.contiguous()


@_timed("seg_eval_binary")
def seg_eval_binary(z: torch.Tensor, g: torch.Tensor, smooth: float = 1.0, dice_weight: float = 0.5):
    if z.dim() != 4 or z.shape[1] != 1:
        raise RuntimeError(f"stain2stain_amd: seg_eval_binary wants logits [B,1,H,W], got {tuple(z.shape)}")
    if g.dim() == 3:
        g = g.unsqueeze(1)
    if tuple(g.shape) != tuple(z.shape):
        raise RuntimeError(f"stain2stain_amd: mask shape {tuple(g.shape)} does not match logits {tuple(z.shape)}")
    if g.device != z.device:
        raise RuntimeError("stain2stain_amd: logits and mask are on different devices")
    z, g = _gpu_f32_operand(z, "logits"), _binary_mask(g)
    out = torch.empty((5,), dtype=torch.float32, device=z.device)
    counts = torch.empty((4,), dtype=torch.int64, device=z.device)
    work = _workspace(z.device, 2 * EV_BLOCKS * 8, "seg_eval").view(torch.float64)
    _native.check(_L().s2s_seg_eval_binary(_f32(z), _f32(g), _f32(out), counts.data_ptr(), work.data_ptr(), z.numel(),
                                           float(smooth), float(dice_weight), _stream()), "seg_eval_binary")
    return out, counts


@_timed("seg_eval_multiclass")
def seg_eval_multiclass(z: torch.Tensor, target: torch.Tensor, ignore_index: int = -100, smooth: float = 1.0,
                        dice_weight: float = 0.5):
    if z.dim() != 4:
        raise RuntimeError(f"stain2stain_amd: seg_eval_multiclass wants logits [B,C,H,W], got {tuple(z.shape)}")
    B, C, H, W = z.shape
    if not 2 <= C <= 8:
        raise RuntimeError(f"stain2stain_amd: seg_eval_multiclass supports 2 <= C <= 8 classes, got {C}")
    if target.dim() == 4 and target.shape[1] == 1:
        target = target[:, 0]
    if tuple(target.shape) != (B, H, W):
        raise RuntimeError(f"stain2stain_amd: target shape {tuple(target.shape)} does not match logits {tuple(z.shape)}")
    if target.dtype.is_floating_point or target.dtype == torch.bool or target.dtype.is_complex:
        raise RuntimeError(f"stain2stain_amd: target must hold integer class indices, got {target.dtype}")
    if target.device != z.device:
        raise RuntimeError("stain2stain_amd: logits and target are on different devices")
    z = _gpu_f32_operand(z, "logits")
    target = target.to(torch.int64).contiguous()
    out = torch.empty((5,), dtype=torch.float32, device=z.device)
    counts = torch.empty((32,), dtype=torch.int64, device=z.device)
    work = _workspace(z.device, 2 * EV_BLOCKS * 58, "seg_eval").view(torch.float64)
    _native.check(_L().s2s_seg_eval_multiclass(_f32(z), target.data_ptr(), _f32(out), counts.data_ptr(),
                                               work.data_ptr(), B, H * W, C, int(ignore_index), float(smooth),
                                               float(dice_weight), _stream()), "seg_eval_multiclass")
    return out, counts.view(4, 8)[:, :C]


@_timed("head_mse_eval")
def head_mse_eval(x: torch.Tensor, w: torch.Tensor, bias: Optional[torch.Tensor], u_nchw: torch.Tensor) -> torch.Tensor:
    if x.dim() != 4:
        raise RuntimeError("stain2stain_amd: head_mse_eval wants an NHWC activation [B,H,W,C]")
    B, H, W, C = x.shape
    cout = w.shape[0]
    if w.numel() != cout * C:
        raise RuntimeError(f"stain2stain_amd: head weight {tuple(w.shape)} does not match {C} input channels")
    if not 1 <= cout <= 8 or C % 8:
        raise RuntimeError(f"stain2stain_amd: head_mse_eval supports C % 8 == 0 and 1 <= Cout <= 8 (C={C}, Cout={cout})")
    if tuple(u_nchw.shape) != (B, cout, H, W):
        raise RuntimeError(f"stain2stain_amd: target shape {tuple(u_nchw.shape)} != {(B, cout, H, W)}")
    if bias is not None and bias.numel() != cout:
        raise RuntimeError("stain2stain_amd: head bias does not match its weight")
    px, ldx = _nhwc(x)
    u = _gpu_f32_operand(u_nchw, "flow target")
    nb = _L().s2s_head_mse_eval_blocks(B, H, W, C)
    _native.check(nb if nb < 0 else 0, "head_mse_eval_blocks")
    lpart = _workspace(x.device, 2 * nb, "head_mse_eval").view(torch.float64)
    loss = torch.empty((), dtype=torch.float32, device=x.device)
    _native.check(_L().s2s_head_mse_eval(_dt(x), px, ldx, _f32(w.detach().reshape(cout, C).contiguous()),
                                         _f32(None if bias is None else bias.detach().contiguous()), _f32(u),
                                         loss.data_ptr(), lpart.data_ptr(), B, H, W, C, cout, _stream()),
                  "head_mse_eval")
    return loss


def _mask_bhw(mask: torch.Tensor, like: torch.Tensor) -> torch.Tensor:
    B, C, H, W = like.shape
    if mask.dim() == 4 and mask.shape[1] == 1:
        mask = mask[:, 0]
    if tuple(mask.shape) != (B, H, W):
        raise RuntimeError(f"stain2stain_amd: mask shape {tuple(mask.shape)} does not match images {tuple(like.shape)}")
    return mask.to(torch.float32).contiguous()


def weighted_mse(v: torch.Tensor, u: torch.Tensor, mask: torch.Tensor, roi_lambda: float = 10.0,
                 want_grad: bool = True, grad_scale: float = 1.0):
    if v.dim() != 4 or v.shape != u.shape:
        raise RuntimeError("stain2stain_amd: weighted_mse wants v, u of equal shape [B,C,H,W]")
    B, C, H, W = v.shape
    v, u, m = v.contiguous(), u.contiguous(), _mask_bhw(mask, v)
    out = torch.empty((1,), dtype=torch.float32, device=v.device)
    dv = torch.empty_like(v) if want_grad else None
    work = torch.empty((512 * 2 + 2,), dtype=torch.float64, device=v.device)
    _native.check(_L().s2s_weighted_mse(_f32(v), _f32(u), _f32(m), _f32(dv), _f32(out), work.data_ptr(), B, C, H * W,
                                        float(roi_lambda), float(grad_scale), _stream()), "weighted_mse")
    return out, dv


def charbonnier_roi(pred: torch.Tensor, truth: torch.Tensor, mask: torch.Tensor, eps_charb: float = 1e-3,
                    eps_area: float = 1e-8) -> torch.Tensor:
    if pred.dim() != 4 or pred.shape != truth.shape:
        raise RuntimeError("stain2stain_amd: charbonnier_roi wants pred, truth of equal shape [B,C,H,W]")
    B, C, H, W = pred.shape
    pred, truth, m = pred.contiguous(), truth.contiguous(), _mask_bhw(mask, pred)
    out = torch.empty((1,), dtype=torch.float32, device=pred.device)
    work = torch.empty((512 * 2 + 2,), dtype=torch.float64, device=pred.device)
    _native.check(_L().s2s_charbonnier_roi(_f32(pred), _f32(truth), _f32(m), _f32(out), work.data_ptr(), B, C, H * W,
                                           float(eps_charb), float(eps_area), _stream()), "charbonnier_roi")
    return out


def class_embed_add(temb: torch.Tensor, table: torch.Tensor, y: torch.Tensor) -> torch.Tensor:
    B, dim = temb.shape
    if table.shape[1] != dim or y.shape != (B,):
        raise RuntimeError("stain2stain_amd: class_embed_add shape mismatch")
    out = torch.empty_like(temb)
    _native.check(_L().s2s_class_embed_add(_f32(temb.contiguous()), _f32(table), y.data_ptr(), _f32(out), B, dim,
                                           _stream()), "class_embed_add")
    return out


def class_embed_bwd(dout: torch.Tensor, y: torch.Tensor, num_classes: int) -> torch.Tensor:
    B, dim = dout.shape
    dtable = torch.empty((num_classes, dim), dtype=torch.float32, device=dout.device)
    _native.check(_L().s2s_class_embed_bwd(_f32(dout.contiguous()), y.data_ptr(), _f32(dtable), 0, B, dim,
                                           num_classes, _stream()), "class_embed_bwd")
    return dtable


def ode_error_norm(e: torch.Tensor, y0: torch.Tensor, y1: torch.Tensor, atol: float, rtol: float) -> torch.Tensor:
    out = torch.empty((1,), dtype=torch.float32, device=e.device)
    work = torch.empty((1024,), dtype=torch.float64, device=e.device)
    _native.check(_L().s2s_ode_error_norm(_f32(e), _f32(y0), _f32(y1), float(atol), float(rtol), _f32(out),
                                          work.data_ptr(), e.numel(), _stream()), "ode_error_norm")
    return out


def axpy_(x: torch.Tensor, y: torch.Tensor, a: float) -> None:
    _native.check(_L().s2s_axpy(_f32(x), _f32(y), float(a), x.numel(), _stream()), "axpy")


# ... 985 lines not shown
```

stain2stain_amd/trainer.py:

```python
from __future__ import annotations

from typing import Dict, List, Optional, Tuple

import torch
import torch.distributed as dist

from . import engine, evaluation, ops
from .components import FlowUNet
from .ema import TrainerEMA
from .ddp import all_reduce_mean_scalar, broadcast_from_rank0
from .fused_step import CapturedStep, FlatParams


def _param_groups(net: FlowUNet) -> List[List[Tuple[str, str, torch.nn.Parameter]]]:
    dec, enc = net.flow_decoder, net.encoder
    dnamed = dict(dec.named_parameters())
    enamed = dict(enc.named_parameters())
    groups: List[List[Tuple[str, str, torch.nn.Parameter]]] = []

    def layer(owner, named, prefix):
        for idx in (("3.", "4."), ("0.", "1.")):
            groups.append([(owner, n, p) for n, p in named.items()
                           if any(n.startswith(prefix + i) for i in idx)])

    groups.append([("dec", n, p) for n, p in dnamed.items() if n.startswith("outc.")])
    for i in range(len(dec.ups) - 1, -1, -1):
        layer("dec", dnamed, f"ups.{i}.conv.double_conv.")
    groups.append([("dec", n, p) for n, p in dnamed.items() if n.startswith("time_")])
    for i in range(len(enc.downs) - 1, -1, -1):
        layer("enc", enamed, f"downs.{i}.maxpool_conv.1.double_conv.")
    layer("enc", enamed, "inc.double_conv.")
    groups = [g for g in groups if g] if getattr(dec, "time_mlp", None) is None else groups
    seen = sum(len(g) for g in groups)
    if seen != len(dnamed) + len(enamed) or any(not g for g in groups):
        raise RuntimeError("parameter grouping does not cover the network")
    return groups


class FusedAdamHandle(torch.optim.Optimizer):

    def __init__(self, trainer: "CFMTrainer", lr, betas, eps, weight_decay):
        self._trainer = trainer
        super().__init__([trainer.fp.p], dict(lr=lr, betas=tuple(betas), eps=eps, weight_decay=weight_decay))

    @torch.no_grad()
    def step(self, closure=None):
        loss = closure() if closure is not None else None
        self._trainer.optimizer_step()
        return loss

    def zero_grad(self, set_to_none: bool = False) -> None:
        pass

    def state_dict(self):
        return self._trainer.optimizer_state_dict()

    def load_state_dict(self, state_dict) -> None:
        self._trainer.load_optimizer_state_dict(state_dict)


class CFMTrainer:
    def __init__(self, net: FlowUNet, lr: float = 1e-4, weight_decay: float = 1e-5,
                 betas: Tuple[float, float] = (0.9, 0.999), eps: float = 1e-8, sigma: float = 0.0,
                 bucket_mb: float = 4.0, process_group=None, sync_loss: bool = True, max_bucket_mb: float = 16.0,
                 sharded_optimizer: bool = False, sync_batchnorm: bool = False, graph: bool = False,
                 ema_decay: Optional[float] = None, ema_buffers: bool = True):
        dev = next(net.parameters()).device
        if dev.type != "cuda":
            raise RuntimeError("stain2stain_amd: CFMTrainer needs the network on a GPU (HIP-only implementation)")
        self.net = net
        self.sigma = sigma
        self.pg = process_group
        self.sync_loss = sync_loss
        groups = [[(f"{owner}.{name}", p) for owner, name, p in g] for g in _param_groups(net)]
        self.fp = FlatParams(groups, bucket_mb, process_group, max_bucket_mb, sharded_optimizer)
        self.grads_enc = {k[len("enc."):]: v for k, v in self.fp.grads.items() if k.startswith("enc.")}
        self.grads_dec = {k[len("dec."):]: v for k, v in self.fp.grads.items() if k.startswith("dec.")}
        names = {id(p): name for g in groups for name, p in g}
        self._names = [names[id(p)] for p in net.parameters()]
        self.optimizer = FusedAdamHandle(self, lr, betas, eps, weight_decay)
        self.n_params = sum(p.numel() for g in groups for _, p in g)
        self._group = 0
        self._sync_bn = engine.SyncBNExchange(process_group) if sync_batchnorm and self.bucketer.enabled else None
        broadcast_from_rank0(list(net.buffers()), process_group)
        self._dtype = net.encoder.compute_dtype
        self.packer = engine.Conv3x3Packer(list(net.encoder._blocks) + list(net.flow_decoder.up_blocks), self._dtype)
        self._side = ops.side_stream_for(dev)
        self.overlap_wgrad = True
        self.fuse_tail = True
        self.graph = graph
        self._graph_step = CapturedStep()
        self._ema = None
        if ema_decay is not None:
            self.fp.enable_ema(ema_decay)
            self._ema = TrainerEMA(self.fp, [net], ema_buffers)
        self._eval_owner = object()
        self._generation = evaluation.GenerationEval()

    step_count = property(lambda self: self.fp.step_count)
    bucketer = property(lambda self: self.fp.bucketer)
    flat_p = property(lambda self: self.fp.p)
    flat_g = property(lambda self: self.fp.g)
    _captured = property(lambda self: self._graph_step.graph)

    @property
    def _hp(self):
        return self.optimizer.param_groups[0]

    lr = property(lambda self: self._hp["lr"], lambda self, v: self._hp.__setitem__("lr", v))
    wd = property(lambda self: self._hp["weight_decay"], lambda self, v: self._hp.__setitem__("weight_decay", v))
    betas = property(lambda self: self._hp["betas"], lambda self, v: self._hp.__setitem__("betas", tuple(v)))
    eps = property(lambda self: self._hp["eps"], lambda self, v: self._hp.__setitem__("eps", v))

    def forward_backward(self, x0: torch.Tensor, x1: torch.Tensor, t: Optional[torch.Tensor] = None,
                         want_v: bool = True):
        net = self.net
        enc, dec = net.encoder, net.flow_decoder
        dt = enc.compute_dtype
        B = x0.shape[0]
        x0, x1 = x0.float().contiguous(), x1.float().contiguous()
        if t is None:
            t = torch.rand(B, device=x0.device, dtype=torch.float32)
        t = t.float().contiguous()
        eps_noise = torch.randn_like(x0) if self.sigma != 0.0 else None
        xt, ut = ops.cfm_sample(x0, x1, t, self.sigma, eps_noise)
        with engine.sync_batchnorm(self._sync_bn):
            ectx = engine.encoder_forward(enc._blocks, xt, dt, True)
            temb = ops.time_embedding(t, net.time_embedding.dim)
            feats = ectx.feats
            dctx = engine.decoder_forward(dec, feats[-1], feats[:-1][::-1], temb, dt, True, with_head=False,
                                          fuse_tail=self.fuse_tail and not want_v)
        if dctx.lows[-1] is None:
            g_head = None
            loss, v = engine.decoder_tail_loss(dec, dctx, ut, self.grads_dec, want_v=want_v)
        else:
            loss, g_head, v = ops.head_loss_fused(dctx.lows[-1], dec.outc.weight.detach(),
                                                  dec.outc.bias.detach() if dec.outc.bias is not None else None, ut,
                                                  self.grads_dec["outc.weight"], self.grads_dec.get("outc.bias"),
                                                  want_v=want_v)
            dctx.v = v
        self.bucketer.start_step()
        self._group = 0
        with engine.side_scope(self._side if self.overlap_wgrad else None):
            dbott, dskips, _ = engine.decoder_backward(dec, dctx, None, self.grads_dec, g_head=g_head,
                                                       on_group_done=self._group_done)
            L = len(feats) - 1
            dfeats = [dskips[L - 1 - l] for l in range(L)] + [dbott]
            engine.encoder_backward(enc._blocks, ectx, dfeats, self.grads_enc, on_group_done=self._group_done)
        return loss, dctx.v

    def _group_done(self) -> None:
        self.bucketer.mark_ready_ordered(self._group, self._side if self.overlap_wgrad else None)
        self._group += 1

    def optimizer_step(self) -> None:
        self._enqueue_optimizer(None)
        self._after_step()

    def _after_step(self) -> None:
        engine.mutation_epoch[0] += 1
        if self._ema is not None:
            self._ema.after_step()

    def _enqueue_optimizer(self, hyper_dev: Optional[torch.Tensor]) -> None:
        engine.join_side(self._side)
        self.fp.adam(self.lr, self.betas, self.eps, self.wd, hyper_dev)
        if self._ema is not None:
            self._ema.update_buffers()
        self._repack()

    def _repack(self) -> None:
        self.packer.repack()

    def optimizer_state_dict(self) -> Dict:
        sd = self.fp.state_dict()
        state = {}
        if self.step_count > 0:
            for i, name in enumerate(self._names):
                state[i] = {"step": torch.tensor(float(self.step_count)),
                            "exp_avg": sd["exp_avg"][name], "exp_avg_sq": sd["exp_avg_sq"][name]}
        group = {"lr": self.lr, "betas": tuple(self.betas), "eps": self.eps, "weight_decay": self.wd,
                 "amsgrad": False, "maximize": False, "foreach": None, "capturable": False, "differentiable": False,
                 "fused": None, "params": list(range(len(self._names)))}
        return {"state": state, "param_groups": [group]}

    def load_optimizer_state_dict(self, sd: Dict) -> None:
        groups = sd["param_groups"]
        if len(groups) != 1 or len(groups[0]["params"]) != len(self._names):
            raise ValueError("optimizer state does not match this network (one group over net.parameters() expected)")
        if groups[0].get("amsgrad", False) or groups[0].get("maximize", False):
            raise ValueError("amsgrad / maximize Adam states are not supported")
        g = groups[0]
        self.lr, self.betas, self.eps, self.wd = g["lr"], tuple(g["betas"]), g["eps"], g["weight_decay"]
        steps = set()
        fp = self.fp
        fp.m.zero_()
        fp.v.zero_()
        for i, (p, name) in enumerate(zip(self.net.parameters(), self._names)):
            st = sd["state"].get(i, sd["state"].get(str(i)))
            if st is None:
                continue
            o, n = fp.slot[name]
            if tuple(st["exp_avg"].shape) != tuple(p.shape):
                raise ValueError(f"optimizer state {i}: shape {tuple(st['exp_avg'].shape)} != {tuple(p.shape)}")
            fp.m[o:o + n].copy_(st["exp_avg"].reshape(-1))
            fp.v[o:o + n].copy_(st["exp_avg_sq"].reshape(-1))
            steps.add(int(float(st["step"])))
        if len(steps) > 1:
            raise ValueError("per-parameter step counts differ; the flat Adam kernel keeps one")
        fp.step_count = steps.pop() if steps else 0

    def step(self, x0: torch.Tensor, x1: torch.Tensor, t: Optional[torch.Tensor] = None) -> torch.Tensor:
        with ops.workspace_owner(self):
            if self.graph and ops._PROFILE is None:
                if t is None:
                    t = torch.rand(x0.shape[0], device=x0.device, dtype=torch.float32)
                if self.sigma != 0.0:
                    raise NotImplementedError("graph=True with sigma != 0: the path noise is drawn inside forward_backward")
                loss = self._graph_step.run((tuple(x0.shape), x0.device, self.overlap_wgrad), (x0, x1, t),
                                            self._step_body, [self.fp], (self.lr, self.betas, self.eps, self.wd))
            else:
                loss = self._step_body(x0, x1, t, None)
            self._after_step()
            return loss

    def _step_body(self, x0, x1, t, hyper_dev) -> torch.Tensor:
        loss, _ = self.forward_backward(x0, x1, t, want_v=False)
        work = all_reduce_mean_scalar(loss, self.pg) if self.sync_loss else None
        self._enqueue_optimizer(hyper_dev)
        if work is not None:
            work.wait()
            loss = loss / dist.get_world_size(self.pg)
        return loss

    def _ema_on(self) -> TrainerEMA:
        if self._ema is None:
            raise RuntimeError("stain2stain_amd: this trainer keeps no EMA (construct it with ema_decay=...)")
        return self._ema

    def ema_model(self) -> FlowUNet:
        return self._ema_on().modules()[0]

    def ema_state_dict(self) -> Dict[str, torch.Tensor]:
        return self._ema_on().state_dict(self.ema_model().state_dict())

    def load_ema_state_dict(self, sd: Dict[str, torch.Tensor]) -> None:
        ema = self._ema_on()
        ema.load_state_dict(sd, ema.copies[0])

    def evaluate(self, x0: torch.Tensor, x1: torch.Tensor, t: Optional[torch.Tensor] = None,
                 accumulator: Optional[evaluation.EvalAccumulator] = None,
                 use_ema: bool = False) -> Dict[str, torch.Tensor]:
        net = self.ema_model() if use_ema else self.net
        with ops.workspace_owner(self._eval_owner), evaluation.eval_grad_mode():
            x0, x1 = x0.float().contiguous(), x1.float().contiguous()
            if t is None:
                t = torch.rand(x0.shape[0], device=x0.device, dtype=torch.float32)
            t = t.float().contiguous()
            eps_noise = torch.randn_like(x0) if self.sigma != 0.0 else None
            xt, ut = ops.cfm_sample(x0, x1, t, self.sigma, eps_noise)
            loss = evaluation.flow_loss(net.encoder, net.flow_decoder, net.time_embedding.dim, xt, t, ut)
        out = {"loss": loss}
        if accumulator is not None:
            accumulator.add(out, x0.shape[0])
        return out

    def evaluate_generation(self, x0: torch.Tensor, x1: torch.Tensor, num_steps: int = 50, method: str = "euler",
                            graph: bool = False, use_ema: bool = False,
                            accumulator: Optional[evaluation.EvalAccumulator] = None,
                            quantize: bool = True, stain: Optional[dict] = None) -> Dict[str, torch.Tensor]:
        net = self.ema_model() if use_ema else self.net
        with ops.workspace_owner(self._eval_owner), evaluation.eval_grad_mode():
            return evaluation.generation_values(self._generation, bool(use_ema), net.encoder, net.flow_decoder,
                                                net.time_embedding.dim, x0, x1, num_steps, method, graph, quantize,
                                                accumulator, stain)

    def close(self) -> None:
        self._generation.close()
        self._graph_step.close()
        ops.release_workspaces(self)
        ops.release_workspaces(self._eval_owner)

    def __del__(self):
        try:
            self.close()
        except Exception:
            pass
```

Before: 2340.

## Fuse stem BN-ReLU backward into stem weight-gradient kernel

```diff
diff --git a/include/stain2stain_hip.h b/include/stain2stain_hip.h
--- a/include/stain2stain_hip.h
+++ b/include/stain2stain_hip.h
@@ -49,6 +49,10 @@
 int s2s_stem_wgrad_blocks(int B, int H, int W);
 int s2s_stem_conv3x3_wgrad(int dtype, const void* dy, int lddy, const float* x_nchw, float* part, float* dw_oihw,
                            float* dbias, int accumulate, int B, int H, int W, int Cin, int Cout, void* stream);
+int s2s_stem_bn_bwd_wgrad(int dtype, const void* g1, int ldg1, const void* raw, int ldx, const float* scale,
+                          const float* shift, const float* mean, const float* invstd, const float* gamma,
+                          const float* bnwork, const float* x_nchw, float* part, float* dw_oihw, int accumulate, int B,
+                          int H, int W, int Cin, int Cout, void* stream);
 int s2s_head_conv1x1_fwd(int dtype, const void* x, int ldx, const float* w, const float* bias, float* y_nchw, int B,
                          int H, int W, int C, int Cout, void* stream);
 int s2s_head_wgrad_blocks(int B, int H, int W);
diff --git a/stain2stain_amd/csrc/conv_edge.hip b/stain2stain_amd/csrc/conv_edge.hip
--- a/stain2stain_amd/csrc/conv_edge.hip
+++ b/stain2stain_amd/csrc/conv_edge.hip
@@ -30,6 +30,69 @@
   if (NIMG == 3) {
     *reinterpret_cast<bf16x8*>(base + img_stride + off) = m;
     *reinterpret_cast<bf16x8*>(base + 2 * img_stride + off) = l;
+  }
+}
+
+constexpr int STEM_NPX = 256;
+constexpr int STEM_DY_IMG = 2 * STEM_NPX * 64;
+constexpr int STEM_P_IMG = STEM_NPX * 64;
+
+__device__ __forceinline__ void stem_tile_origin(int tile, int tilesY, int tilesX, int& n, int& y0, int& x0) {
+  const int tx = tile % tilesX; tile /= tilesX;
+  const int ty = tile % tilesY;
+  n = tile / tilesY;
+  y0 = ty * 16; x0 = tx * 16;
+}
+
+template <int NIMG>
+__device__ __forceinline__ void stem_im2col(const float* xl, char* ldsP, int tid, bool inside, int K, bool bias_col) {
+  const int py = tid >> 4, px = tid & 15;
+#pragma unroll
+  for (int c4 = 0; c4 < 4; ++c4) {
+    float v8[8];
+#pragma unroll
+    for (int k = 0; k < 8; ++k) {
+      const int kk = c4 * 8 + k;
+      float v = 0.f;
+      if (kk < K) {
+        const int ci = kk / 9, t = kk - ci * 9;
+        v = xl[ci * 324 + (py + t / 3) * 18 + px + t % 3];
+      } else if (kk == K && bias_col) {
+        v = inside ? 1.f : 0.f;
+      }
+      v8[k] = v;
+    }
+    split_store<NIMG>(ldsP, STEM_P_IMG, tid * 64 + c4 * 16, v8);
+  }
+}
+
+template <int NIMG>
+__device__ __forceinline__ void stem_tile_mfma(const char* A0, const char* B0, int whalf, f32x16& acc) {
+#pragma unroll
+  for (int ks = 0; ks < 8; ++ks) {
+    const int m0 = (whalf * 8 + ks) * 16;
+    const bf16x8 ah = tr_frag8(A0 + m0 * 64);
+    const bf16x8 bh = tr_frag8(B0 + m0 * 64);
+    if constexpr (NIMG == 3) {
+      const bf16x8 am = tr_frag8(A0 + STEM_DY_IMG + m0 * 64), al = tr_frag8(A0 + 2 * STEM_DY_IMG + m0 * 64);
+      const bf16x8 bm = tr_frag8(B0 + STEM_P_IMG + m0 * 64), bl = tr_frag8(B0 + 2 * STEM_P_IMG + m0 * 64);
+      acc = __builtin_amdgcn_mfma_f32_32x32x16_bf16(am, bm, acc, 0, 0, 0);
+      acc = __builtin_amdgcn_mfma_f32_32x32x16_bf16(al, bh, acc, 0, 0, 0);
+      acc = __builtin_amdgcn_mfma_f32_32x32x16_bf16(ah, bl, acc, 0, 0, 0);
+      acc = __builtin_amdgcn_mfma_f32_32x32x16_bf16(am, bh, acc, 0, 0, 0);
+      acc = __builtin_amdgcn_mfma_f32_32x32x16_bf16(ah, bm, acc, 0, 0, 0);
+    }
+    acc = __builtin_amdgcn_mfma_f32_32x32x16_bf16(ah, bh, acc, 0, 0, 0);
+  }
+}
+
+__device__ __forceinline__ void stem_store_slab(const f32x16& acc, float* part, int lane, int co0, int wco, int whalf, int Cout) {
+  const int kcol = lane & 31, h = lane >> 5;
+#pragma unroll
+  for (int j = 0; j < 16; ++j) {
+    const int co = co0 + wco * 32 + (j & 3) + 8 * (j >> 2) + 4 * h;
+    if (co < Cout)
+      part[((((long)blockIdx.z * gridDim.x + blockIdx.x) * 2 + whalf) * Cout + co) * 32 + kcol] = acc[j];
   }
 }
 
@@ -39,9 +102,7 @@
                                                          int B, int H, int W, int Cin, int Cout, int tilesY,
                                                          int tilesX) {
   constexpr int NIMG = sizeof(T) == 4 ? 3 : 1;
-  constexpr int NPX = 256;
-  constexpr int DY_IMG = 2 * NPX * 64;
-  constexpr int P_IMG = NPX * 64;
+  constexpr int NPX = STEM_NPX, DY_IMG = STEM_DY_IMG, P_IMG = STEM_P_IMG;
   extern __shared__ __attribute__((aligned(16))) char smem[];
   char* const ldsDY = smem;
   char* const ldsP = smem + NIMG * DY_IMG;
@@ -58,11 +119,8 @@
 #pragma unroll
   for (int j = 0; j < 16; ++j) acc[j] = 0.f;
   for (int tile = blockIdx.x; tile < ntiles; tile += gridDim.x) {
-    int bt = tile;
-    const int tx = bt % tilesX; bt /= tilesX;
-    const int ty = bt % tilesY;
-    const int n = bt / tilesY;
-    const int y0 = ty * 16, x0 = tx * 16;
+    int n, y0, x0;
+    stem_tile_origin(tile, tilesY, tilesX, n, y0, x0);
     __syncthreads();
     for (int i = tid; i < nc * 324; i += 256) {
       const int ci = i / 324, r = i - ci * 324, hy = r / 18, hx = r - hy * 18;
@@ -85,54 +143,119 @@
       split_store<NIMG>(ldsDY, DY_IMG, (pc >> 2) * (NPX * 64) + px * 64 + (pc & 3) * 16, v8);
     }
     __syncthreads();
-    {
-      const int py = tid >> 4, px = tid & 15;
-      const bool inside = (y0 + py < H) && (x0 + px < W);
-#pragma unroll
-      for (int c4 = 0; c4 < 4; ++c4) {
-        float v8[8];
-#pragma unroll
-        for (int k = 0; k < 8; ++k) {
-          const int kk = c4 * 8 + k;
-          float v = 0.f;
-          if (kk < K) {
-            const int ci = kk / 9, t = kk - ci * 9;
-            v = xl[ci * 324 + (py + t / 3) * 18 + px + t % 3];
-          } else if (kk == K && c0 == 0) {
-            v = inside ? 1.f : 0.f;
-          }
-          v8[k] = v;
-        }
-        split_store<NIMG>(ldsP, P_IMG, tid * 64 + c4 * 16, v8);
-      }
-    }
-    __syncthreads();
-    const char* A0 = ldsDY + wco * (NPX * 64) + frag_off;
-    const char* B0 = ldsP + frag_off;
-#pragma unroll
-    for (int ks = 0; ks < 8; ++ks) {
-      const int m0 = (whalf * 8 + ks) * 16;
-      const bf16x8 ah = tr_frag8(A0 + m0 * 64);
-      const bf16x8 bh = tr_frag8(B0 + m0 * 64);
-      if constexpr (NIMG == 3) {
-        const bf16x8 am = tr_frag8(A0 + DY_IMG + m0 * 64), al = tr_frag8(A0 + 2 * DY_IMG + m0 * 64);
-        const bf16x8 bm = tr_frag8(B0 + P_IMG + m0 * 64), bl = tr_frag8(B0 + 2 * P_IMG + m0 * 64);
-        acc = __builtin_amdgcn_mfma_f32_32x32x16_bf16(am, bm, acc, 0, 0, 0);
-        acc = __builtin_amdgcn_mfma_f32_32x32x16_bf16(al, bh, acc, 0, 0, 0);
-        acc = __builtin_amdgcn_mfma_f32_32x32x16_bf16(ah, bl, acc, 0, 0, 0);
-        acc = __builtin_amdgcn_mfma_f32_32x32x16_bf16(am, bh, acc, 0, 0, 0);
-        acc = __builtin_amdgcn_mfma_f32_32x32x16_bf16(ah, bm, acc, 0, 0, 0);
-      }
-      acc = __builtin_amdgcn_mfma_f32_32x32x16_bf16(ah, bh, acc, 0, 0, 0);
-    }
-  }
-  const int kcol = lane & 31, h = lane >> 5;
-#pragma unroll
-  for (int j = 0; j < 16; ++j) {
-    const int co = co0 + wco * 32 + (j & 3) + 8 * (j >> 2) + 4 * h;
-    if (co < Cout)
-      part[((((long)blockIdx.z * gridDim.x + blockIdx.x) * 2 + whalf) * Cout + co) * 32 + kcol] = acc[j];
-  }
+    stem_im2col<NIMG>(xl, ldsP, tid, (y0 + (tid >> 4) < H) && (x0 + (tid & 15) < W), K, c0 == 0);
+    __syncthreads();
+    stem_tile_mfma<NIMG>(ldsDY + wco * (NPX * 64) + frag_off, ldsP + frag_off, whalf, acc);
+  }
+  stem_store_slab(acc, part, lane, co0, wco, whalf, Cout);
+}
+
+template <typename T>
+struct __attribute__((aligned(16))) Raw8 {
+  T e[8];
+};
+
+struct StemBN {
+  const float *scale, *shift, *mean, *invstd, *gamma, *c1, *c2;
+};
+
+template <typename T>
+__device__ __forceinline__ float stem_draw(float g, float x, float scale, float shift, float mean, float invstd, float ga,
+                                           float c1, float c2) {
+#pragma clang fp contract(off)
+  const float dz = fmaf(x, scale, shift) > 0.f ? g : 0.f;
+  const float t = (x - mean) * invstd;
+  return (float)from_f32<T>(ga * fmaf(-t, c2, dz - c1));
+}
+
+template <typename T>
+__global__ __launch_bounds__(256) void stem_bn_bwd_wgrad_kernel(const T* __restrict__ g1, int ldg,
+                                                                const T* __restrict__ raw, int ldr, StemBN bn,
+                                                                const float* __restrict__ x, float* __restrict__ part,
+                                                                int B, int H, int W, int Cin, int Cout, int tilesY,
+                                                                int tilesX) {
+  constexpr int NIMG = sizeof(T) == 4 ? 3 : 1;
+  constexpr int NPX = STEM_NPX, DY_IMG = STEM_DY_IMG, P_IMG = STEM_P_IMG;
+  extern __shared__ __attribute__((aligned(16))) char smem[];
+  char* const ldsDY = smem;
+  char* const ldsP = smem + NIMG * DY_IMG;
+  float* const xl = reinterpret_cast<float*>(ldsP + NIMG * P_IMG);
+  const int tid = threadIdx.x, lane = tid & 63, wave = tid >> 6;
+  const int wco = wave & 1, whalf = wave >> 1;
+  const int co0 = blockIdx.y * 64;
+  const int c0 = blockIdx.z * 3;
+  const int nc = (Cin - c0) < 3 ? (Cin - c0) : 3, K = nc * 9;
+  const int g = lane >> 4, q = (lane & 15) >> 2, pq = lane & 3;
+  const int frag_off = ((g >> 1) * 8 + q) * 64 + ((g & 1) * 16 + pq * 4) * 2;
+  const int ntiles = B * tilesY * tilesX;
+  const int pc = tid & 7, co = co0 + pc * 8, spx = tid >> 3;
+  const bool cok = co < Cout;
+  const int cc = cok ? co : 0;
+  float sc[8], sh[8], mu[8], is[8], ga[8], k1[8], k2[8];
+#pragma unroll
+  for (int k = 0; k < 8; ++k) {
+    sc[k] = bn.scale[cc + k]; sh[k] = bn.shift[cc + k]; mu[k] = bn.mean[cc + k]; is[k] = bn.invstd[cc + k];
+    ga[k] = bn.gamma[cc + k] * is[k]; k1[k] = bn.c1[cc + k]; k2[k] = bn.c2[cc + k];
+  }
+  Raw8<T> rg[8], rx[8];
+  float hv[4];
+  auto load_tile = [&](int tile) {
+    int n, y0, x0;
+    stem_tile_origin(tile, tilesY, tilesX, n, y0, x0);
+#pragma unroll
+    for (int it = 0; it < 8; ++it) {
+      const int px = spx + it * 32;
+      const int gy = min(y0 + (px >> 4), H - 1), gx = min(x0 + (px & 15), W - 1);
+      const long p = ((long)n * H + gy) * W + gx;
+      rg[it] = *reinterpret_cast<const Raw8<T>*>(g1 + p * ldg + cc);
+      rx[it] = *reinterpret_cast<const Raw8<T>*>(raw + p * ldr + cc);
+    }
+#pragma unroll
+    for (int j = 0; j < 4; ++j) {
+      const int i = min(tid + j * 256, nc * 324 - 1);
+      const int ci = i / 324, r = i - ci * 324, hy = r / 18, hx = r - hy * 18;
+      const int gy = min(max(y0 - 1 + hy, 0), H - 1), gx = min(max(x0 - 1 + hx, 0), W - 1);
+      hv[j] = x[(((long)n * Cin + c0 + ci) * H + gy) * W + gx];
+    }
+  };
+  f32x16 acc;
+#pragma unroll
+  for (int j = 0; j < 16; ++j) acc[j] = 0.f;
+  if ((int)blockIdx.x < ntiles) load_tile(blockIdx.x);
+  for (int tile = blockIdx.x; tile < ntiles; tile += gridDim.x) {
+    int n, y0, x0;
+    stem_tile_origin(tile, tilesY, tilesX, n, y0, x0);
+    __syncthreads();
+#pragma unroll
+    for (int j = 0; j < 4; ++j) {
+      const int i = tid + j * 256;
+      if (i < nc * 324) {
+        const int r = i % 324, hy = r / 18, hx = r - hy * 18;
+        const int gy = y0 - 1 + hy, gx = x0 - 1 + hx;
+        xl[i] = (gy >= 0 && gy < H && gx >= 0 && gx < W) ? hv[j] : 0.f;
+      }
+    }
+#pragma unroll
+    for (int it = 0; it < 8; ++it) {
+      const int px = spx + it * 32;
+      const int gy = y0 + (px >> 4), gx = x0 + (px & 15);
+      float v8[8];
+#pragma unroll
+      for (int k = 0; k < 8; ++k) v8[k] = 0.f;
+      if (gy < H && gx < W && cok) {
+#pragma unroll
+        for (int k = 0; k < 8; ++k)
+          v8[k] = stem_draw<T>((float)rg[it].e[k], (float)rx[it].e[k], sc[k], sh[k], mu[k], is[k], ga[k], k1[k], k2[k]);
+      }
+      split_store<NIMG>(ldsDY, DY_IMG, (pc >> 2) * (NPX * 64) + px * 64 + (pc & 3) * 16, v8);
+    }
+    __syncthreads();
+    if (tile + (int)gridDim.x < ntiles) load_tile(tile + gridDim.x);
+    stem_im2col<NIMG>(xl, ldsP, tid, (y0 + (tid >> 4) < H) && (x0 + (tid & 15) < W), K, c0 == 0);
+    __syncthreads();
+    stem_tile_mfma<NIMG>(ldsDY + wco * (NPX * 64) + frag_off, ldsP + frag_off, whalf, acc);
+  }
+  stem_store_slab(acc, part, lane, co0, wco, whalf, Cout);
 }
 
 __global__ __launch_bounds__(1024) void stem_wgrad_reduce_kernel(const float* part, int nslab, int Cout, int Cin, float* dw, float* db,
@@ -843,6 +966,7 @@
 
 int s2s_internal_stem_fwd(int dtype, const float* x_nchw, const float* w_oihw, const float* bias, void* y, int ldy,
                           float* stat_part, int B, int H, int W, int Cin, int Cout, hipStream_t s);
+extern "C" int s2s_bn_bwd_blocks(int B, int H, int W, int C);
 
 extern "C" int s2s_stem_stat_blocks(int B, int H, int W) {
   if (B <= 0 || H <= 0 || W <= 0) return S2S_ERR_SHAPE;
@@ -887,6 +1011,38 @@
   } else return S2S_ERR_DTYPE;
   hipLaunchKernelGGL(stem_wgrad_reduce_kernel, dim3(Cout, cdiv(Cin, 3)), dim3(1024), 0, s, part, 2 * nb, Cout, Cin, dw_oihw, dbias,
                      accumulate);
+  S2S_LAUNCH_CHECK();
+  return S2S_OK;
+}
+
+extern "C" int s2s_stem_bn_bwd_wgrad(int dtype, const void* g1, int ldg1, const void* raw, int ldx, const float* scale,
+                                     const float* shift, const float* mean, const float* invstd, const float* gamma,
+                                     const float* bnwork, const float* x_nchw, float* part, float* dw_oihw,
+                                     int accumulate, int B, int H, int W, int Cin, int Cout, void* stream) {
+  if (!g1 || !raw || !scale || !shift || !mean || !invstd || !gamma || !bnwork || !x_nchw || !part || !dw_oihw)
+    return S2S_ERR_NULL;
+  if (B <= 0 || H <= 0 || W <= 0 || Cin <= 0 || Cin > 6 || Cout <= 0 || (Cout % 8) || (ldg1 % 8) || (ldx % 8))
+    return S2S_ERR_SHAPE;
+  const int nbn = s2s_bn_bwd_blocks(B, H, W, Cout);
+  if (nbn <= 0) return S2S_ERR_SHAPE;
+  const float* const c1 = bnwork + (long)4 * nbn * Cout;
+  const StemBN bn{scale, shift, mean, invstd, gamma, c1, c1 + Cout};
+  const int nb = s2s_stem_wgrad_blocks(B, H, W);
+  hipStream_t s = (hipStream_t)stream;
+  dim3 grid(nb, cdiv(Cout, 64), cdiv(Cin, 3));
+  if (dtype == S2S_BF16) {
+    const int lds = 1 * (STEM_DY_IMG + STEM_P_IMG) + 3 * 324 * 4;
+    hipLaunchKernelGGL(stem_bn_bwd_wgrad_kernel<bf16_t>, grid, dim3(256), lds, s, (const bf16_t*)g1, ldg1,
+                       (const bf16_t*)raw, ldx, bn, x_nchw, part, B, H, W, Cin, Cout, cdiv(H, 16), cdiv(W, 16));
+  } else if (dtype == S2S_F32) {
+    const int lds = 3 * (STEM_DY_IMG + STEM_P_IMG) + 3 * 324 * 4;
+    static unsigned long long attr_devs = 0;
+    if (int rc = s2s_allow_dyn_lds(reinterpret_cast<const void*>(stem_bn_bwd_wgrad_kernel<float>), lds, &attr_devs)) return rc;
+    hipLaunchKernelGGL(stem_bn_bwd_wgrad_kernel<float>, grid, dim3(256), lds, s, (const float*)g1, ldg1,
+                       (const float*)raw, ldx, bn, x_nchw, part, B, H, W, Cin, Cout, cdiv(H, 16), cdiv(W, 16));
+  } else return S2S_ERR_DTYPE;
+  hipLaunchKernelGGL(stem_wgrad_reduce_kernel, dim3(Cout, cdiv(Cin, 3)), dim3(1024), 0, s, part, 2 * nb, Cout, Cin, dw_oihw,
+                     (float*)nullptr, accumulate);
   S2S_LAUNCH_CHECK();
   return S2S_OK;
 }
@@ -1023,7 +1179,6 @@
                               const float* shift, const float* mean, const float* invstd, float* work, float* dgamma,
                               float* dbeta, float* zero_out, int accumulate, int B, int H, int W, int C, int Cout,
                               hipStream_t s);
-extern "C" int s2s_bn_bwd_blocks(int B, int H, int W, int C);
 
 namespace {
 inline bool tail_shape_ok(int B, int H, int W, int C, int Cout, int ldx) {
diff --git a/stain2stain_amd/csrc/norm_act.hip b/stain2stain_amd/csrc/norm_act.hip
--- a/stain2stain_amd/csrc/norm_act.hip
+++ b/stain2stain_amd/csrc/norm_act.hip
@@ -668,8 +668,8 @@
                                float* dgamma, float* dbeta, float* dbias_conv, int accumulate, void* dx, int lddx,
                                float* work, int B, int H, int W, int C, long count_total, int phases, void* stream) {
   if (phases < 1 || phases > 3 || count_total < (long)B * H * W) return S2S_ERR_SHAPE;
-  if ((!g1 && !gp) || !scale || !shift || !x || !mean || !invstd || !gamma || !dgamma || !dbeta || !dx || !work) return S2S_ERR_NULL;
-  if (B <= 0 || H <= 0 || W <= 0 || C <= 0 || (C % 8) || (ldx % 8) || (lddx % 8) ||
+  if ((!g1 && !gp) || !scale || !shift || !x || !mean || !invstd || !gamma || !dgamma || !dbeta || (!dx && (phases & 2)) || !work) return S2S_ERR_NULL;
+  if (B <= 0 || H <= 0 || W <= 0 || C <= 0 || (C % 8) || (ldx % 8) || (dx && (lddx % 8)) ||
       (g1 && (ldg1 % 8)) || (gp && (ldgp % 8)))
     return S2S_ERR_SHAPE;
   if ((long)B * ((H + 1) / 2) * ((W + 1) / 2) >= (1L << 31) - (1 << 20)) return S2S_ERR_SHAPE;
diff --git a/stain2stain_amd/engine.py b/stain2stain_amd/engine.py
--- a/stain2stain_amd/engine.py
+++ b/stain2stain_amd/engine.py
@@ -325,12 +325,19 @@
         raise RuntimeError(f"stain2stain_amd: no gradient buffer for parameter {name!r}") from e
 
 
-def _conv_bn_relu_bwd(cb: ConvBN, lc: LayerCtx, g1, gp, grads, accumulate: bool, need_dx: bool, stem: bool = False):
+def _conv_bn_relu_bwd(cb: ConvBN, lc: LayerCtx, g1, gp, grads, accumulate: bool, need_dx: bool, stem: bool = False,
+                      fuse_stem: bool = False):
     p = cb.prefix
     i_conv, i_bn = cb.idx
     dgamma = _g(grads, f"{p}.{i_bn}.weight")
     dbeta = _g(grads, f"{p}.{i_bn}.bias")
     dbias = _g(grads, f"{p}.{i_conv}.bias") if cb.conv.bias is not None else None
+    if stem and fuse_stem and gp is None and lc.sync is None:
+        gamma = cb.bn.weight.detach()
+        work = ops.bn_relu_bwd_sums(g1, lc.raw, lc.stats, gamma, dgamma, dbeta, dbias, accumulate)
+        dw = _g(grads, f"{p}.{i_conv}.weight")
+        run_on_side(lambda: ops.stem_bn_bwd_wgrad(g1, lc.raw, lc.stats, gamma, work, lc.x0, dw, accumulate), (g1, work))
+        return None
     draw = ops.bn_relu_bwd(g1, gp, lc.raw, lc.stats, cb.bn.weight.detach(), dgamma, dbeta, dbias, accumulate,
                            exchange=lc.sync, count_total=lc.count)
     dw = _g(grads, f"{p}.{i_conv}.weight")
@@ -394,7 +401,8 @@
 
 
 def encoder_backward(blocks: Sequence[Tuple[ConvBN, ConvBN]], ctx: EncCtx, dfeats: Sequence[Optional[torch.Tensor]],
-                     grads: Dict[str, torch.Tensor], accumulate: bool = False, on_group_done=None) -> None:
+                     grads: Dict[str, torch.Tensor], accumulate: bool = False, on_group_done=None,
+                     fuse_stem: bool = False) -> None:
     gpool = None
     nlev = len(blocks)
     for l in range(len(blocks) - 1, -1, -1):
@@ -406,7 +414,8 @@
         ga1 = _conv_bn_relu_bwd(c2, lc2, g1, gpool, grads, accumulate, need_dx=True)
         if on_group_done is not None:
             on_group_done()
-        gpool = _conv_bn_relu_bwd(c1, lc1, ga1, None, grads, accumulate, need_dx=(l > 0), stem=(l == 0))
+        fuse = {"fuse_stem": True} if fuse_stem and l == 0 else {}
+        gpool = _conv_bn_relu_bwd(c1, lc1, ga1, None, grads, accumulate, need_dx=(l > 0), stem=(l == 0), **fuse)
         if on_group_done is not None:
             on_group_done()
 
diff --git a/stain2stain_amd/multitask_trainer.py b/stain2stain_amd/multitask_trainer.py
--- a/stain2stain_amd/multitask_trainer.py
+++ b/stain2stain_amd/multitask_trainer.py
@@ -75,6 +75,7 @@
         self._side = ops.side_stream_for(dev)
         self.overlap_wgrad = True
         self.fuse_tail = True
+        self.fuse_stem = True
         self._group = 0
         self._eval_owner = object()
         self._generation = evaluation.GenerationEval()
@@ -92,7 +93,7 @@
         self._group += 1
 
     def forward_backward(self, source: torch.Tensor, target: torch.Tensor, mask: torch.Tensor,
-                         t: Optional[torch.Tensor] = None, want_outputs: bool = False):
+                         t: Optional[torch.Tensor] = None, want_outputs: bool = False, fuse_stem: bool = False):
         enc, fdec, sdec = self.encoder, self.flow_decoder, self.seg_decoder
         dt = self._dtype
         x0, x1 = source.float().contiguous(), target.float().contiguous()
@@ -135,9 +136,10 @@
             dbs, dss, _ = engine.decoder_backward(sdec, dctx_s, dz, self.grads_seg, on_group_done=self._group_done)
             dbf, dsf, _ = engine.decoder_backward(fdec, dctx_f, None, self.grads_flow, g_head=g_head,
                                                   on_group_done=self._group_done)
-            engine.encoder_backward(enc._blocks, ectx2, [dss[L - 1 - l] for l in range(L)] + [dbs], self.grads_enc)
+            engine.encoder_backward(enc._blocks, ectx2, [dss[L - 1 - l] for l in range(L)] + [dbs], self.grads_enc,
+                                    fuse_stem=fuse_stem)
             engine.encoder_backward(enc._blocks, ectx1, [dsf[L - 1 - l] for l in range(L)] + [dbf], self.grads_enc,
-                                    accumulate=True, on_group_done=self._group_done)
+                                    accumulate=True, on_group_done=self._group_done, fuse_stem=fuse_stem)
         second = "seg_ce" if self.num_classes is not None else "seg_bce"
         losses = {"total": total, "flow": flow, "seg": seg3[0], "seg_dice": seg3[1], second: seg3[2]}
         return losses, ({"v": v, "logits": logits} if want_outputs else None)
@@ -174,7 +176,7 @@
 
     def step(self, source: torch.Tensor, target: torch.Tensor, mask: torch.Tensor,
              t: Optional[torch.Tensor] = None) -> torch.Tensor:
-        losses, _ = self.forward_backward(source, target, mask, t)
+        losses, _ = self.forward_backward(source, target, mask, t, fuse_stem=self.fuse_stem)
         total = losses["total"]
         work = all_reduce_mean_scalar(total, self.pg) if self.sync_loss else None
         self.optimizer_step()
diff --git a/stain2stain_amd/ops.py b/stain2stain_amd/ops.py
--- a/stain2stain_amd/ops.py
+++ b/stain2stain_amd/ops.py
@@ -346,6 +346,24 @@
     _native.check(rc, "stem_conv3x3_wgrad")
 
 
+@_timed("stem_bn_bwd_wgrad")
+def stem_bn_bwd_wgrad(g1: torch.Tensor, raw: torch.Tensor, stats: torch.Tensor, gamma: torch.Tensor, work: torch.Tensor,
+                      x_nchw: torch.Tensor, dw: torch.Tensor, accumulate: bool = False) -> None:
+    B, H, W, cout = raw.shape
+    cin = x_nchw.shape[1]
+    px, ldx = _nhwc(raw)
+    pg, ldg = _nhwc(g1)
+    if g1.shape != raw.shape or g1.dtype != raw.dtype or tuple(x_nchw.shape) != (B, cin, H, W) \
+            or work.numel() != 4 * _L().s2s_bn_bwd_blocks(B, H, W, cout) * cout + 2 * cout:
+        raise RuntimeError("stain2stain_amd: stem_bn_bwd_wgrad operands do not belong together")
+    nb = _L().s2s_stem_wgrad_blocks(B, H, W)
+    part = torch.empty(((cin + 2) // 3, 2 * nb, cout, 32), dtype=torch.float32, device=raw.device)
+    rc = _L().s2s_stem_bn_bwd_wgrad(_dt(raw), pg, ldg, px, ldx, stats[2].data_ptr(), stats[3].data_ptr(),
+                                    stats[0].data_ptr(), stats[1].data_ptr(), _f32(gamma), _f32(work), _f32(x_nchw),
+                                    _f32(part), _f32(dw), int(accumulate), B, H, W, cin, cout, _stream())
+    _native.check(rc, "stem_bn_bwd_wgrad")
+
+
 @_timed("head_fwd")
 def head_fwd(x: torch.Tensor, w: torch.Tensor, bias: Optional[torch.Tensor]) -> torch.Tensor:
     B, H, W, C = x.shape
@@ -530,6 +548,22 @@
                               dx.data_ptr(), C, _f32(work), B, H, W, C, _stream())
     _native.check(rc, "bn_relu_bwd")
     return dx
+
+
+@_timed("bn_relu_bwd_sums")
+def bn_relu_bwd_sums(g1: torch.Tensor, x: torch.Tensor, stats: torch.Tensor, gamma: torch.Tensor, dgamma: torch.Tensor,
+                     dbeta: torch.Tensor, dbias_conv: Optional[torch.Tensor], accumulate: bool = False) -> torch.Tensor:
+    B, H, W, C = x.shape
+    px, ldx = _nhwc(x)
+    p1, ld1 = _nhwc(g1)
+    nb = _L().s2s_bn_bwd_blocks(B, H, W, C)
+    work = torch.empty((4 * nb * C + 2 * C,), dtype=torch.float32, device=x.device)
+    rc = _L().s2s_bn_relu_bwd_phase(_dt(x), p1, ld1, 0, 8, stats[2].data_ptr(), stats[3].data_ptr(), px, ldx,
+                                    stats[0].data_ptr(), stats[1].data_ptr(), _f32(gamma), _f32(dgamma), _f32(dbeta),
+                                    _f32(dbias_conv), int(accumulate), 0, 8, _f32(work), B, H, W, C, B * H * W, 1,
+                                    _stream())
+    _native.check(rc, "bn_relu_bwd_sums")
+    return work
 
 
 @_timed("upsample2x_fwd")
diff --git a/stain2stain_amd/trainer.py b/stain2stain_amd/trainer.py
--- a/stain2stain_amd/trainer.py
+++ b/stain2stain_amd/trainer.py
@@ -88,6 +88,7 @@
         self._side = ops.side_stream_for(dev)
         self.overlap_wgrad = True
         self.fuse_tail = True
+        self.fuse_stem = True
         self.graph = graph
         self._graph_step = CapturedStep()
         self._ema = None
@@ -113,7 +114,7 @@
     eps = property(lambda self: self._hp["eps"], lambda self, v: self._hp.__setitem__("eps", v))
 
     def forward_backward(self, x0: torch.Tensor, x1: torch.Tensor, t: Optional[torch.Tensor] = None,
-                         want_v: bool = True):
+                         want_v: bool = True, fuse_stem: bool = False):
         net = self.net
         enc, dec = net.encoder, net.flow_decoder
         dt = enc.compute_dtype
@@ -146,7 +147,8 @@
                                                        on_group_done=self._group_done)
             L = len(feats) - 1
             dfeats = [dskips[L - 1 - l] for l in range(L)] + [dbott]
-            engine.encoder_backward(enc._blocks, ectx, dfeats, self.grads_enc, on_group_done=self._group_done)
+            engine.encoder_backward(enc._blocks, ectx, dfeats, self.grads_enc, on_group_done=self._group_done,
+                                    fuse_stem=fuse_stem)
         return loss, dctx.v
 
     def _group_done(self) -> None:
@@ -225,7 +227,7 @@
             return loss
 
     def _step_body(self, x0, x1, t, hyper_dev) -> torch.Tensor:
-        loss, _ = self.forward_backward(x0, x1, t, want_v=False)
+        loss, _ = self.forward_backward(x0, x1, t, want_v=False, fuse_stem=self.fuse_stem)
         work = all_reduce_mean_scalar(loss, self.pg) if self.sync_loss else None
         self._enqueue_optimizer(hyper_dev)
         if work is not None:
```

Result: no change. 2359 (median of 6 runs) (+0.8%).
